# ai-forever/Kandinsky-2

Hardware: AMD Instinct MI355X
Metric: UNet denoise steps/sec @ 768x768 bs=1, 50 steps (higher is better)
Workload: dtype bf16; 1 GPU; Kandinsky-2.x text2img 768x768, decoder_steps=50, bs=1/GPU (CFG batch 2x4x96x96), 2.1-architecture UNet (1.23B) p_sampler step; parity pinned against the reference's modules; head=2.1, tile_configs_measured_in_this_process=0, images_per_gpu=1, parallelism=prompt-sharded x1, weights by one RCCL broadcast, world_size_observed=1, graph=True, chains=1, loop_graph=a 5-step loop replayed as ONE hipGraph (83 replay(s) = 415 timed steps)

## Files before the change

include/k22.h:

```cpp
#ifndef K22_H
#define K22_H
#include <stddef.h>
#include <stdint.h>
#ifdef __cplusplus
extern "C" {
#endif

#define K22_OK 0
#define K22_EINVAL (-1)
#define K22_EHIP (-2)
#define K22_ENOMEM (-3)

#define K22_BF16 0
#define K22_F32 1
#define K22_F16 2
#define K22_F16X3 3
#define K22_F16X2 4

int k22_version(void);
#define K22_BUILD_PACKED_FP32 1
#define K22_BUILD_DEBUG_VARIANTS 2
int k22_build_flags(void);
const char* k22_last_error(void);
int k22_set_option(const char* name, int value);
// ... 100 lines not shown
  int out_mode, res_f32, act, a_raw, want_stats;
  int SK0, SK1;
  int att_T, att_S, att_Tkp;
  int ldo, ldr;
  int has_frag;
  int algo, bm, bn, splitk, stages;
} K22IgemmProblem;
typedef struct K22IgemmOperands {
  const void *A0, *A1, *Wp, *bias, *residual;
  void *out, *partial;
  const void *S0, *S1, *Ws, *bias2;
  void *kall, *vtall;
  const void *Wfrag, *Wsfrag;
  float* stats;
  int stats_capacity_rows;
} K22IgemmOperands;
int k22_igemm_cfg_accepted(const K22IgemmProblem* pr);
int k22_igemm_cfg(const K22IgemmProblem* pr, const K22IgemmOperands* ops, int* rows_per_image, void* stream);
int k22_debug_conv_trace(const void* x_padded, const void* Wp, const float* bias, void* out, int B, int H, int W, int Cin, int Cout,
                         int Npad, unsigned long long* trace, void* stream);
int k22_conv3x3_gn(const void* x0, const void* x1, int C0, int C1, const float* gamma, const float* beta, const float* film, long film_ld,
                   float eps, int act, void* scratch, const void* Wp, const float* bias, const void* residual, void* out, void* partial,
                   int B, int H, int W, int Cout, int Npad, int splitk, int bm, int algo, int dtype, void* stream);
int k22_groupnorm(const void* x0, const void* x1, int C0, int C1, int B, int H, int W, const float* gamma,
                  const float* beta, const float* film, long film_ld, float eps, int act, int mode, int pad,
                  void* scratch, void* out, int dtype, void* stream);
size_t k22_groupnorm_scratch_bytes(int B, int C);
int k22_attention(const void* qkv, const void* ctxkv, void* kall, void* vtall, void* out, int B, int H, int T, int S,
                  int dtype, void* stream);
int k22_qkv_project(const void* x, const void* Wp, const float* bias, void* q_out, void* kall, void* vtall,
                    int B, int H, int T, int S, int K, int bm, int bn, int dtype, void* stream);
int k22_qkv_project_stream(const void* x, const void* Wp, const float* bias, void* q_out, void* kall, void* vtall, void* partial,
                           int B, int H, int T, int S, int K, int bm, int splitk, int dtype, void* stream);
int k22_linear_smallm(const float* x, const void* W, const float* bias, const float* add, float* out, int M, int N,
                      int K, int act_in, int act_out, int wdtype, void* stream);
int k22_conv3x3_direct(const float* x, const float* w, const float* bias, float* y, int B, int Cin, int Cout, int Hin, int Win,
                       int stride, int act, void* stream);

size_t k22_afrag_bytes(int M, int K);
int k22_afrag_pack(const void* A, long lda, void* out, int M, int K, int dtype, void* stream);
int k22_skinny_gemm(const void* Afrag, const void* Wfrag, const float* bias, void* out, float* partial, int M, int N, int Npad, int K,
                    int splitk, int epi, int act, int ldo, int mt, int nb, int dtype, void* stream);
int k22_finish_ln(const float* partial, int splitk, const float* bias, float* x, long ldx, const float* gain, const float* beta, void* yfrag,
                  int M, int N, float eps, int dtype, void* stream);
int k22_small_attention(const void* qkv, const float* qkv_partial, int nsplit, const float* qkv_bias, void* out, int out_frag, int B, int H, int T,
                        int causal, const float* key_valid, int kv_n, int dtype, void* stream);

typedef struct K22PriorConfig {
  int dtype;
  int text_ctx;
  int xf_width;
  int xf_layers;
  int xf_heads;
  int xf_final_ln;
  int clip_dim;
  int clip_xf_width;
} K22PriorConfig;
typedef struct K22Prior K22Prior;
int k22_prior_create(const K22PriorConfig* cfg, const K22Weight* weights, int n_weights, K22Prior** out);
void k22_prior_destroy(K22Prior* m);
int k22_prior_plan(K22Prior* m, int B, size_t* workspace_bytes);
int k22_prior_bind(K22Prior* m, void* workspace, size_t workspace_bytes);
int k22_prior_tuning_report(const K22Prior* m, char* buf, size_t cap);
int k22_prior_forward(K22Prior* m, const float* x, const float* timesteps, const float* text_emb, const float* text_enc,
                      const float* key_valid, float* out, void* stream);
int k22_prior_sampler_step(const float* x, const float* model_out, const float* noise, const float* scales, const float* table_row,
                           float clamp, float* x_out, int bs, int D, void* stream);
int k22_prior_ddim_step(const float* x, const float* model_out, const float* noise, const float* scales, const float* table_row,
                        float clamp, float* x_out, float* x0_out, int bs, int D, void* stream);
enum { K22_PRIOR_LOOP_ANCESTRAL = 0, K22_PRIOR_LOOP_DDIM = 1 };
int k22_prior_sample_loop(K22Prior* m, int kind, float* x, float* x_tmp, float* x0_out, const float* timesteps, const float* table,
                          const float* noise_seq, const float* scales, const float* text_emb, const float* text_enc,
                          const float* key_valid, float clamp, int n_steps, int use_graph, void* stream);

typedef struct K22MoVQConfig {
  int dtype;
  int ch;
  int n_levels;
  int ch_mult[8];
  int num_res_blocks;
  int attn_levels;
  int z_channels;
  int out_ch;
} K22MoVQConfig;
typedef struct K22MoVQ K22MoVQ;
int k22_movq_create(const K22MoVQConfig* cfg, const K22Weight* weights, int n_weights, K22MoVQ** out);
void k22_movq_destroy(K22MoVQ* m);
int k22_movq_plan(K22MoVQ* m, int B, int h, int w, size_t* workspace_bytes);
int k22_movq_bind(K22MoVQ* m, void* workspace, size_t workspace_bytes);
int k22_movq_decode(K22MoVQ* m, const float* z, float* out, unsigned char* out_u8, void* stream);
int k22_movq_plan_encoder(K22MoVQ* m, int B, int H, int W, size_t* workspace_bytes);
int k22_movq_encode(K22MoVQ* m, const float* image, float* latent, void* stream);
int k22_movq_num_ops(const K22MoVQ* m);

enum { K22_ENC_CLIP_TEXT = 0, K22_ENC_CLIP_VISION = 1, K22_ENC_XLMR = 2 };
typedef struct K22EncoderConfig {
  int dtype;
  int kind;
  int width;
  int layers;
  int heads;
  int n_ctx;
  int vocab;
  int out_dim;
  int image_size;
  int patch;
  int max_pos;
  int pad_id;
  float ln_eps;
  int mlp_dim;
  int hidden_act;
} K22EncoderConfig;
typedef struct K22Encoder K22Encoder;
int k22_encoder_create(const K22EncoderConfig* cfg, const K22Weight* weights, int n_weights, K22Encoder** out);
void k22_encoder_destroy(K22Encoder* m);
int k22_encoder_plan(K22Encoder* m, int B, size_t* workspace_bytes);
int k22_encoder_bind(K22Encoder* m, void* workspace, size_t workspace_bytes);
int k22_encoder_forward(K22Encoder* m, const int* tokens, const float* key_valid, const float* image, float* seq_out, float* pooled_out,
                        void* stream);

int k22_blend_noised(const float* x, const float* init, const float* noise, const float* mask, float sa, float sb, float* out,
                     int N, int C, int HW, int broadcast_first, void* stream);

int k22_spatialnorm_apply(const void* x, const float* coeff, const float* zq, const float* wy, const float* by, const float* wb, const float* bb,
                          void* out, int B, int H, int W, int C, int h0, int w0, int shift, int act, int pad, int dtype, void* stream);
int k22_upsample2_pad(const void* x, void* y, int B, int H, int W, int C, int dtype, void* stream);
int k22_pad_copy(const void* x, void* y, int B, int H, int W, int C, int dtype, void* stream);
int k22_subsample_odd(const void* x, void* y, int B, int H, int W, int C, int dtype, void* stream);
int k22_softmax_rows(void* x, long rows, int L, float scale, int dtype, void* stream);
int k22_movq_prepare(const float* z, const float* wpq, const float* bpq, float* zq, void* xin, int B, int h, int w, int Cpad, int dtype, void* stream);
int k22_movq_enc_prepare(const float* image, void* xin, int B, int H, int W, int Cpad, int dtype, void* stream);
int k22_movq_quant_conv(const float* h, const float* wq, const float* bq, float* out, int B, int HW, void* stream);
int k22_to_uint8_nhwc(const float* x, unsigned char* y, int B, int C, int H, int W, void* stream);
int k22_enc_layernorm(const float* x, long ldx, const float* gain, const float* beta, float* out_f32, long ld_out, void* out_t, int rows,
                      int D, float eps, int dtype, void* stream);
int k22_enc_embed(const int* tokens, const float* tok_emb, const float* pos_emb, const float* type_emb, float* x, int B, int n_ctx, int D,
                  int vocab, int xlmr, int pad_id, int max_pos, void* stream);
int k22_enc_gather_eot(const int* tokens, const float* x, float* out, int B, int n_ctx, int D, void* stream);
int k22_enc_masked_mean(const float* x, const float* mask, float* out, int B, int n_ctx, int D, void* stream);
int k22_enc_patchify(const float* image, void* out, int B, int S, int patch, int Kp, int dtype, void* stream);
int k22_enc_vision_assemble(const float* patch_out, const float* cls, const float* pos, float* x, int B, int P, int D, void* stream);
int k22_enc_mlp_act(const float* x, void* y, long n, int exact, int dtype, void* stream);
int k22_enc_attention_generic(const void* qkv, void* out, int B, int heads, int n, int hd, int dtype, void* stream);
int k22_prior_layernorm(const float* x, long ldx, const float* gain, const float* beta, void* y, int rows, int D, int to_f32, int dtype,
                        void* stream);
int k22_prior_finish_input(float* inp, const float* pos, const float* prd, int B, int n_ctx, int D, void* stream);
int k22_attention_masked(const void* qkv, const void* ctxkv, void* kall, void* vtall, void* out, int B, int H, int T, int S, int causal,
                         const float* key_valid, int kv_n, int out_x3, int dtype, void* stream);
int k22_gn_stats(const void* x0, const void* x1, int C0, int C1, int B, int HW, float* partial, int* nsplit_out, int dtype, void* stream);
int k22_gn_coeff(const float* st0, int rpi0, int C0, const float* st1, int rpi1, int C1, int B, int HW, const float* gamma, const float* beta,
                 const float* film, long film_ld, float eps, float* coeff, void* stream);
int k22_gn_apply(const void* x0, const void* x1, int C0, int C1, int B, int H, int W, const float* coeff, int act, int mode, int pad, void* out,
                 int dtype, void* stream);

#ifdef __cplusplus
}
#endif
#endif
```

kandinsky-2_amd/_lib.py:

```python
from __future__ import annotations

import ctypes as C
import os

_HERE = os.path.dirname(os.path.abspath(__file__))
LIB_PATH = os.environ.get("K22_LIB_PATH") or os.path.join(_HERE, "libk22hip.so")
TILE_TABLE_PATH = os.path.join(_HERE, "tiles_gfx950.txt")

K22_BF16, K22_F32, K22_F16, K22_F16X3, K22_F16X2 = 0, 1, 2, 3, 4
K22_LOOP_DDIM, K22_LOOP_PLMS = 0, 1
K22_PRIOR_LOOP_ANCESTRAL, K22_PRIOR_LOOP_DDIM = 0, 1
F16X3 = "f16x3"
F16X2 = "f16x2"
SPLIT_DTYPES = (F16X3, F16X2)
X3_WSCALE = 256.0


def dtype_code(backend_dtype) -> int:
    import torch
    try:
        return {torch.bfloat16: K22_BF16, torch.float32: K22_F32, torch.float16: K22_F16, F16X3: K22_F16X3, F16X2: K22_F16X2}[backend_dtype]
    except KeyError:
        raise ValueError('backend_dtype must be torch.bfloat16, torch.float16, torch.float32 "f16x3" or "f16x2"') from None
ACT_NONE, ACT_SILU, ACT_GELU = 0, 1, 2
OUT_ROWMAJOR, OUT_ROWMAJOR_F32, OUT_NCHW_F32, OUT_QKV = 0, 1, 2, 3


class K22UNetConfig(C.Structure):
    _fields_ = [
        ("dtype", C.c_int), ("in_channels", C.c_int), ("model_channels", C.c_int), ("out_channels", C.c_int),
        ("num_res_blocks", C.c_int), ("n_levels", C.c_int), ("channel_mult", C.c_int * 8),
        ("n_attention_ds", C.c_int), ("attention_ds", C.c_int * 8), ("num_head_channels", C.c_int),
        ("ctx_dim", C.c_int), ("ctx_len", C.c_int), ("n_image_embs", C.c_int), ("text_dim1", C.c_int),
        ("text_dim2", C.c_int), ("image_dim", C.c_int), ("head_type", C.c_int), ("hint_channels", C.c_int),
    ]


class K22IgemmProblem(C.Structure):
    _fields_ = [(n, C.c_int) for n in (
        "dtype", "taps", "M", "N", "Kc", "K0", "H", "W", "out_mode", "res_f32", "act", "a_raw", "want_stats", "SK0", "SK1",
        "att_T", "att_S", "att_Tkp", "ldo", "ldr", "has_frag", "algo", "bm", "bn", "splitk", "stages")]


class K22IgemmOperands(C.Structure):
    _fields_ = [(n, C.c_void_p) for n in (
        "A0", "A1", "Wp", "bias", "residual", "out", "partial", "S0", "S1", "Ws", "bias2", "kall", "vtall", "Wfrag", "Wsfrag",
        "stats")] + [("stats_capacity_rows", C.c_int)]


class K22MoVQConfig(C.Structure):
    _fields_ = [("dtype", C.c_int), ("ch", C.c_int), ("n_levels", C.c_int), ("ch_mult", C.c_int * 8),
                ("num_res_blocks", C.c_int), ("attn_levels", C.c_int), ("z_channels", C.c_int), ("out_ch", C.c_int)]


class K22PriorConfig(C.Structure):
    _fields_ = [("dtype", C.c_int), ("text_ctx", C.c_int), ("xf_width", C.c_int), ("xf_layers", C.c_int), ("xf_heads", C.c_int),
                ("xf_final_ln", C.c_int), ("clip_dim", C.c_int), ("clip_xf_width", C.c_int)]


class K22EncoderConfig(C.Structure):
    _fields_ = [("dtype", C.c_int), ("kind", C.c_int), ("width", C.c_int), ("layers", C.c_int), ("heads", C.c_int), ("n_ctx", C.c_int),
                ("vocab", C.c_int), ("out_dim", C.c_int), ("image_size", C.c_int), ("patch", C.c_int), ("max_pos", C.c_int),
                ("pad_id", C.c_int), ("ln_eps", C.c_float), ("mlp_dim", C.c_int), ("hidden_act", C.c_int)]


class K22Weight(C.Structure):
    _fields_ = [("name", C.c_char_p), ("ptr", C.c_void_p)]


_P, _I, _L, _F, _D, _Z = C.c_void_p, C.c_int, C.c_long, C.c_float, C.c_double, C.c_size_t

SIGNATURES = {
    "k22_version": (_I, []),
    "k22_build_flags": (_I, []),
    "k22_last_error": (C.c_char_p, []),
    "k22_set_option": (_I, [C.c_char_p, _I]),
    "k22_comm_broadcast_weights": (_I, [_P, _Z, _I, _P, _P]),
    "k22_tile_table_load": (_I, [C.c_char_p]),
    "k22_tile_table_save": (_I, [C.c_char_p]),
    "k22_tile_table_size": (_I, []),
    "k22_tile_table_measured": (_I, []),
    "k22_tile_table_clear": (None, []),
    "k22_unet_create": (_I, [C.POINTER(K22UNetConfig), C.POINTER(K22Weight), _I, C.POINTER(_P)]),
    "k22_unet_destroy": (None, [_P]),
    "k22_unet_plan": (_I, [_P, _I, _I, _I, C.POINTER(_Z)]),
    "k22_unet_bind": (_I, [_P, _P, _Z]),
    "k22_unet_set_condition": (_I, [_P, _P, _P, _P, _P]),
    "k22_unet_set_hint": (_I, [_P, _P, _P]),
    "k22_unet_forward": (_I, [_P, _P, _P, _P, _P, _P, _I, _P]),
    "k22_unet_sample_loop": (_I, [_P, _P, _P, _P, _P, _P, _P, _P, _P, _P, C.POINTER(_I), _I, _F, _F, _F, _I, _D, _P, _I, _P]),
    "k22_unet_ddim_loop": (_I, [_P, _I, _P, _P, _P, _P, _P, _P, _P, _P, _P, _I, _F, _I, _P]),
    "k22_unet_num_ops": (_I, [_P]),
    "k22_unet_set_autotune": (_I, [_P, _I]),
    "k22_unet_tuning_report": (_I, [_P, C.c_char_p, _Z]),
    "k22_unet_profile": (_I, [_P, _I, C.POINTER(_D), C.POINTER(_D), C.POINTER(_D), C.POINTER(_I), _P]),
    "k22_afrag_bytes": (_Z, [_I, _I]),
    "k22_afrag_pack": (_I, [_P, _L, _P, _I, _I, _I, _P]),
    "k22_skinny_gemm": (_I, [_P, _P, _P, _P, _P, _I, _I, _I, _I, _I, _I, _I, _I, _I, _I, _I, _P]),
    "k22_finish_ln": (_I, [_P, _I, _P, _P, _L, _P, _P, _P, _I, _I, _F, _I, _P]),
    "k22_small_attention": (_I, [_P, _P, _I, _P, _P, _I, _I, _I, _I, _I, _P, _I, _I, _P]),
    "k22_prior_create": (_I, [C.POINTER(K22PriorConfig), C.POINTER(K22Weight), _I, C.POINTER(_P)]),
    "k22_prior_destroy": (None, [_P]),
    "k22_prior_plan": (_I, [_P, _I, C.POINTER(_Z)]),
    "k22_prior_bind": (_I, [_P, _P, _Z]),
    "k22_prior_tuning_report": (_I, [_P, C.c_char_p, _Z]),
    "k22_prior_forward": (_I, [_P, _P, _P, _P, _P, _P, _P, _P]),
    "k22_prior_sampler_step": (_I, [_P, _P, _P, _P, _P, _F, _P, _I, _I, _P]),
    "k22_prior_ddim_step": (_I, [_P, _P, _P, _P, _P, _F, _P, _P, _I, _I, _P]),
    "k22_prior_sample_loop": (_I, [_P, _I, _P, _P, _P, _P, _P, _P, _P, _P, _P, _P, _F, _I, _I, _P]),
    "k22_encoder_create": (_I, [C.POINTER(K22EncoderConfig), C.POINTER(K22Weight), _I, C.POINTER(_P)]),
    "k22_encoder_destroy": (None, [_P]),
    "k22_encoder_plan": (_I, [_P, _I, C.POINTER(_Z)]),
    "k22_encoder_bind": (_I, [_P, _P, _Z]),
    "k22_encoder_forward": (_I, [_P, _P, _P, _P, _P, _P, _P]),
    "k22_movq_create": (_I, [C.POINTER(K22MoVQConfig), C.POINTER(K22Weight), _I, C.POINTER(_P)]),
    "k22_movq_destroy": (None, [_P]),
    "k22_movq_plan": (_I, [_P, _I, _I, _I, C.POINTER(_Z)]),
    "k22_movq_bind": (_I, [_P, _P, _Z]),
    "k22_movq_decode": (_I, [_P, _P, _P, _P, _P]),
    "k22_movq_plan_encoder": (_I, [_P, _I, _I, _I, C.POINTER(_Z)]),
    "k22_movq_encode": (_I, [_P, _P, _P, _P]),
    "k22_movq_num_ops": (_I, [_P]),
    "k22_ddim_step": (_I, [_P, _P, _P, _P, _F, _I, _P, _P, _I, _I, _P]),
    "k22_blend_noised": (_I, [_P, _P, _P, _P, _F, _F, _P, _I, _I, _I, _I, _P]),
    "k22_prepare_mask": (_I, [_P, _P, _I, _I, _I, _P]),
    "k22_plms_step": (_I, [_P, _P, _P, _P, _P, _I, _P, _F, _I, _P, _P, _P, _I, _I, _P]),
    "k22_sampler_scratch_bytes": (_Z, [_I, _I]),
    "k22_sampler_step": (_I, [_P, _P, _P, _P, _P, _P, _I, _F, _I, _F, _F, _I, _D, _P, _P, _P, _I, _I, _P]),
    "k22_gemm": (_I, [_P, _P, _P, _P, _P, _P, _P, _I, _I, _I, _I, _I, _L, _L, _I, _I, _I, _I, _I, _I, _I, _I, _P]),
    "k22_x3_pack": (_I, [_P, _P, _L, _F, _P]),
    "k22_conv3x3": (_I, [_P, _P, _P, _P, _P, _P, _I, _I, _I, _I, _I, _I, _I, _I, _I, _I, _I, _I, _P]),
    "k22_conv3x3_skip": (_I, [_P, _P, _P, _P, _P, _I, _I, _P, _P, _P, _P, _I, _I, _I, _I, _I, _I, _I, _I, _I, _P]),
    "k22_gemm_gnstats": (_I, [_P, _P, _P, _P, _P, _P, _I, _I, _I, _I, _I, _I, _I, _I, _P, _I, C.POINTER(_I), _I, _P]),
    "k22_conv3x3_gnstats": (_I, [_P, _P, _P, _P, _P, _P, _I, _I, _I, _I, _I, _I, _I, _I, _I, _P, _I, C.POINTER(_I), _I, _P]),
    "k22_igemm_cfg_accepted": (_I, [C.POINTER(K22IgemmProblem)]),
    "k22_igemm_cfg": (_I, [C.POINTER(K22IgemmProblem), C.POINTER(K22IgemmOperands), C.POINTER(_I), _P]),
    "k22_conv3x3_gn": (_I, [_P, _P, _I, _I, _P, _P, _P, _L, _F, _I, _P, _P, _P, _P, _P, _P, _I, _I, _I, _I, _I, _I, _I, _I, _I, _P]),
    "k22_debug_conv_trace": (_I, [_P, _P, _P, _P, _I, _I, _I, _I, _I, _I, _P, _P]),
    "k22_groupnorm": (_I, [_P, _P, _I, _I, _I, _I, _I, _P, _P, _P, _L, _F, _I, _I, _I, _P, _P, _I, _P]),
    "k22_groupnorm_scratch_bytes": (_Z, [_I, _I]),
    "k22_attention": (_I, [_P, _P, _P, _P, _P, _I, _I, _I, _I, _I, _P]),
    "k22_qkv_project": (_I, [_P, _P, _P, _P, _P, _P, _I, _I, _I, _I, _I, _I, _I, _I, _P]),
    "k22_qkv_project_stream": (_I, [_P, _P, _P, _P, _P, _P, _P, _I, _I, _I, _I, _I, _I, _I, _I, _P]),
    "k22_linear_smallm": (_I, [_P, _P, _P, _P, _P, _I, _I, _I, _I, _I, _I, _P]),
    "k22_conv3x3_direct": (_I, [_P, _P, _P, _P, _I, _I, _I, _I, _I, _I, _I, _P]),
    "k22_debug_counter": (_L, [C.c_char_p]),
    "k22_stream_frag_bytes": (C.c_size_t, [_I, _I, _I, _I]),
    "k22_stream_repack": (_I, [_P, _P, _I, _I, _I, _I, _P]),
    "k22_debug_set_stream_frag": (_I, [_P, _P]),
    "k22_debug_set_stream_scratch": (_I, [_P, C.c_size_t]),
    "k22_spatialnorm_apply": (_I, [_P, _P, _P, _P, _P, _P, _P, _P, _I, _I, _I, _I, _I, _I, _I, _I, _I, _I, _P]),
    "k22_upsample2_pad": (_I, [_P, _P, _I, _I, _I, _I, _I, _P]),
    "k22_pad_copy": (_I, [_P, _P, _I, _I, _I, _I, _I, _P]),
    "k22_subsample_odd": (_I, [_P, _P, _I, _I, _I, _I, _I, _P]),
    "k22_softmax_rows": (_I, [_P, _L, _I, _F, _I, _P]),
    "k22_movq_prepare": (_I, [_P, _P, _P, _P, _P, _I, _I, _I, _I, _I, _P]),
    "k22_movq_enc_prepare": (_I, [_P, _P, _I, _I, _I, _I, _I, _P]),
    "k22_movq_quant_conv": (_I, [_P, _P, _P, _P, _I, _I, _P]),
    "k22_to_uint8_nhwc": (_I, [_P, _P, _I, _I, _I, _I, _P]),
    "k22_enc_layernorm": (_I, [_P, _L, _P, _P, _P, _L, _P, _I, _I, _F, _I, _P]),
    "k22_enc_embed": (_I, [_P, _P, _P, _P, _P, _I, _I, _I, _I, _I, _I, _I, _P]),
    "k22_enc_gather_eot": (_I, [_P, _P, _P, _I, _I, _I, _P]),
    "k22_enc_masked_mean": (_I, [_P, _P, _P, _I, _I, _I, _P]),
    "k22_enc_patchify": (_I, [_P, _P, _I, _I, _I, _I, _I, _P]),
    "k22_enc_vision_assemble": (_I, [_P, _P, _P, _P, _I, _I, _I, _P]),
    "k22_enc_mlp_act": (_I, [_P, _P, _L, _I, _I, _P]),
    "k22_enc_attention_generic": (_I, [_P, _P, _I, _I, _I, _I, _I, _P]),
    "k22_prior_layernorm": (_I, [_P, _L, _P, _P, _P, _I, _I, _I, _I, _P]),
    "k22_prior_finish_input": (_I, [_P, _P, _P, _I, _I, _I, _P]),
    "k22_attention_masked": (_I, [_P, _P, _P, _P, _P, _I, _I, _I, _I, _I, _P, _I, _I, _I, _P]),
    "k22_gn_stats": (_I, [_P, _P, _I, _I, _I, _I, _P, C.POINTER(_I), _I, _P]),
    "k22_gn_coeff": (_I, [_P, _I, _I, _P, _I, _I, _I, _I, _P, _P, _P, _L, _F, _P, _P]),
    "k22_gn_apply": (_I, [_P, _P, _I, _I, _I, _I, _I, _P, _I, _I, _I, _P, _I, _P]),
}

_lib = None


def lib() -> C.CDLL:
    global _lib
    if _lib is None:
        if not os.path.exists(LIB_PATH):
            raise RuntimeError(
                f"{LIB_PATH} is missing: the HIP extension is the only compute path (no CPU fallback). "
                "Build it with `python -c 'import __graft_entry__ as g; g.build()'`.")
        l = C.CDLL(LIB_PATH)
        for name, (res, args) in SIGNATURES.items():
            fn = getattr(l, name)
            fn.restype = res
            fn.argtypes = args
        _lib = l
        tbl = os.environ.get("K22_TILE_TABLE", TILE_TABLE_PATH)
        if tbl != "0" and os.path.exists(tbl):
            if l.k22_tile_table_load(tbl.encode()) < 0:
                raise RuntimeError(f"k22: cannot read the tile table {tbl}")
    return _lib


def check(rc: int) -> None:
    if rc != 0:
        msg = lib().k22_last_error()
        raise RuntimeError(f"k22 error {rc}: {msg.decode() if msg else ''}")


def ptr(t) -> int:
    if t is None:
        return None
    assert t.is_contiguous(), "k22: tensors crossing the C ABI must be contiguous"
    return t.data_ptr()


def current_stream() -> int:
    import torch
    return torch.cuda.current_stream().cuda_stream
```

kandinsky-2_amd/csrc/capi.hip:

```cpp
#include "kernels.h"
#include "elementwise.h"
#include "../../include/k22.h"
#include "tuning.h"
#include "skinny.h"
#include <dlfcn.h>
#include <stdio.h>
#include <string.h>

static thread_local char g_err[512] = "";

int k22_set_error(int code, const char* msg) {
  snprintf(g_err, sizeof(g_err), "%s", msg ? msg : "");
  return code;
}
int k22_set_error_hip(hipError_t e, const char* file, int line) {
  snprintf(g_err, sizeof(g_err), "HIP error %d (%s) at %s:%d", (int)e, hipGetErrorString(e), file, line);
  return K22_EHIP;
}

extern "C" {

int k22_version(void) { return 100; }
int k22_build_flags(void) {
  int f = 0;
#ifndef K22_NOPK
  f |= K22_BUILD_PACKED_FP32;
#endif
#if defined(K22_DEBUG_VARIANTS) || defined(K22_STREAM_DEBUG) || defined(K22_SKINNY_DEBUG)
  f |= K22_BUILD_DEBUG_VARIANTS;
#endif
  return f;
}

int k22_set_option(const char* name, int value) {
  if (name && !strcmp(name, "igemm_stages")) { igemm_set_default_stages(value); return K22_OK; }
  if (name && !strcmp(name, "igemm_xcd_remap")) { igemm_set_xcd_remap(value); return K22_OK; }
  if (name && !strcmp(name, "conv_algo")) { igemm_set_conv_algo(value); return K22_OK; }
  if (name && !strcmp(name, "gemm_algo")) { igemm_set_gemm_algo(value); return K22_OK; }
  if (name && !strcmp(name, "att_pipe")) { attention_set_pipe(value); return K22_OK; }
  return k22_set_error(K22_EINVAL, "k22_set_option: unknown option");
}
const char* k22_last_error(void) { return g_err; }

#ifdef K22_STREAM_DEBUG
static unsigned long long* g_dbg_trace = nullptr;
extern "C" int k22_debug_set_stream_trace(unsigned long long* t) { g_dbg_trace = t; return K22_OK; }
#define K22_DBG_TRACE(p) (p).st_trace = g_dbg_trace
#else
#define K22_DBG_TRACE(p) (void)0
#endif
static const void* g_dbg_wfrag = nullptr;
static const void* g_dbg_wsfrag = nullptr;
static void* g_dbg_scratch = nullptr;
static size_t g_dbg_scratch_bytes = 0;
static int dbg_frag(IgemmParams& p, int dtype, hipStream_t st) {
  K22_DBG_TRACE(p);
  p.Wfrag = g_dbg_wfrag; p.Wsfrag = g_dbg_wsfrag;
  if (g_dbg_wfrag || !g_dbg_scratch || dtype == K22_F32 || (p.taps != 1 && p.taps != 9) || p.Kc % 64 || p.Npad % 64) return K22_OK;
  const size_t n1 = stream_frag_bytes(p.Npad, p.taps, p.Kc, dtype);
  const bool skip = p.S0 != nullptr && p.Ws != nullptr && (p.SK0 + p.SK1) % 64 == 0;
  const size_t n2 = skip ? stream_frag_bytes(p.Npad, 1, p.SK0 + p.SK1, dtype) : 0;
  if (n1 + n2 > g_dbg_scratch_bytes) return k22_set_error(K22_ENOMEM, "debug stream scratch too small");
  if (int rc = launch_stream_repack(p.Wp, g_dbg_scratch, p.Npad, p.taps, p.Kc, dtype, st)) return rc;
  p.Wfrag = g_dbg_scratch;
  if (skip) {
    void* w2 = static_cast<char*>(g_dbg_scratch) + n1;
    if (int rc = launch_stream_repack(p.Ws, w2, p.Npad, 1, p.SK0 + p.SK1, dtype, st)) return rc;
    p.Wsfrag = w2;
  }
  return K22_OK;
}
#define K22_DBG_FRAG(p) do { if (int rc_ = dbg_frag((p), dtype, reinterpret_cast<hipStream_t>(stream))) return rc_; } while (0)
int k22_debug_set_stream_frag(const void* wfrag, const void* wsfrag) { g_dbg_wfrag = wfrag; g_dbg_wsfrag = wsfrag; return K22_OK; }
int k22_debug_set_stream_scratch(void* scratch, size_t bytes) { g_dbg_scratch = scratch; g_dbg_scratch_bytes = scratch ? bytes : 0; return K22_OK; }
size_t k22_stream_frag_bytes(int Npad, int taps, int Kc, int dtype) { return stream_frag_bytes(Npad, taps, Kc, dtype); }
int k22_stream_repack(const void* W, void* out, int Npad, int taps, int Kc, int dtype, void* stream) {
  return launch_stream_repack(W, out, Npad, taps, Kc, dtype, reinterpret_cast<hipStream_t>(stream));
}

long k22_debug_counter(const char* name) {
  if (name && !strcmp(name, "stream_launches")) return stream_launch_count();
  if (name && !strcmp(name, "loop_captures")) return loop_capture_count();
  if (name && !strcmp(name, "loop_launches")) return loop_launch_count();
  return -1;
}

int k22_comm_broadcast_weights(void* arena, size_t bytes, int root, void* nccl_comm, void* stream) {
  if (!arena || !nccl_comm) return k22_set_error(K22_EINVAL, "k22_comm_broadcast_weights: null arena / communicator");
  typedef int (*bcast_fn)(const void*, void*, size_t, int , int, void*, hipStream_t);
  static bcast_fn fn = nullptr;
  if (!fn) {
    void* sym = dlsym(RTLD_DEFAULT, "ncclBroadcast");
    if (!sym) {
      void* h = dlopen("librccl.so.1", RTLD_NOW | RTLD_GLOBAL);
      if (!h) h = dlopen("librccl.so", RTLD_NOW | RTLD_GLOBAL);
      if (h) sym = dlsym(h, "ncclBroadcast");
    }
    if (!sym) return k22_set_error(K22_EINVAL, "k22_comm_broadcast_weights: RCCL (ncclBroadcast) is not loadable in this process");
    fn = reinterpret_cast<bcast_fn>(sym);
  }
  const size_t piece = (size_t)1 << 30;
  char* base = reinterpret_cast<char*>(arena);
  for (size_t off = 0; off < bytes; off += piece) {
    const size_t n = bytes - off < piece ? bytes - off : piece;
    const int rc = fn(base + off, base + off, n,  1, root, nccl_comm, reinterpret_cast<hipStream_t>(stream));
    if (rc != 0) { char msg[96]; snprintf(msg, sizeof msg, "k22_comm_broadcast_weights: ncclBroadcast returned %d", rc); return k22_set_error(K22_EHIP, msg); }
  }
  return K22_OK;
}

int k22_tile_table_load(const char* path) {
  if (!path) return k22_set_error(K22_EINVAL, "k22_tile_table_load: null path");
  const int n = tile_table_load_file(path);
  if (n < 0) return k22_set_error(K22_EINVAL, "k22_tile_table_load: cannot read the file");
  return n;
}
int k22_tile_table_save(const char* path) {
  if (!path) return k22_set_error(K22_EINVAL, "k22_tile_table_save: null path");
  const int n = tile_table_save_file(path);
  if (n < 0) return k22_set_error(K22_EINVAL, "k22_tile_table_save: cannot write the file");
  return n;
}
int k22_tile_table_size(void) {
  TileTable& tt = tile_table();
  std::lock_guard<std::mutex> lk(tt.mu);
  return (int)tt.m.size();
}
int k22_tile_table_measured(void) {
  TileTable& tt = tile_table();
  std::lock_guard<std::mutex> lk(tt.mu);
  return (int)tt.measured;
}
void k22_tile_table_clear(void) {
  TileTable& tt = tile_table();
  std::lock_guard<std::mutex> lk(tt.mu);
  tt.m.clear();
  tt.measured = 0;
}

int k22_gemm(const void* A0, const void* A1, const void* Wp, const float* bias, const void* residual, void* out,
             void* partial, int M, int N, int Npad, int K0, int K1, long lda0, long lda1, int ldo, int ldr,
             int out_f32, int act, int splitk, int bm, int bn, int dtype, void* stream) {
  IgemmParams p = igemm_gemm_problem(M, N, K0, K1, out_f32 ? IG_OUT_ROWMAJOR_F32 : IG_OUT_ROWMAJOR, act);
  p.A0 = A0; p.A1 = A1; p.Wp = Wp; p.bias = bias; p.residual = residual; p.out = out;
  p.partial = reinterpret_cast<float*>(partial);
  p.Npad = Npad; p.lda0 = lda0; p.lda1 = lda1; p.ldo = ldo; p.ldr = ldr;
  p.splitk = splitk; p.force_bm = bm; p.force_bn = bn;
  p.a_raw = k22_is_split(dtype) ? 1 : 0;
  if (p.splitk == 0) p.splitk = partial ? igemm_choose_splitk(p, dtype) : 1;
  K22_DBG_FRAG(p);
  return launch_igemm(p, dtype, reinterpret_cast<hipStream_t>(stream));
}

int k22_x3_pack(const float* src, void* dst, long n, float scale, void* stream) {
  if (!src || !dst || n < 0) return k22_set_error(K22_EINVAL, "x3_pack: null argument");
  return launch_x3_pack(src, dst, n, scale, reinterpret_cast<hipStream_t>(stream));
}

int k22_conv3x3(const void* x_padded, const void* Wp, const float* bias, const void* residual, void* out,
                void* partial, int B, int H, int W, int Cin, int Cout, int Npad, int out_mode, int act, int splitk,
                int bm, int bn, int dtype, void* stream) {
  IgemmParams p = igemm_conv3_problem(B, H, W, Cin, Cout, out_mode, act);
  p.A0 = x_padded; p.Wp = Wp; p.bias = bias; p.residual = residual; p.out = out;
  p.partial = reinterpret_cast<float*>(partial);
  p.Npad = Npad; p.splitk = splitk; p.force_bm = bm; p.force_bn = bn;
  if (p.splitk == 0) p.splitk = partial ? igemm_choose_splitk(p, dtype) : 1;
  K22_DBG_FRAG(p);
  return launch_igemm(p, dtype, reinterpret_cast<hipStream_t>(stream));
}

int k22_conv3x3_gnstats(const void* x_padded, const void* Wp, const float* bias, const void* residual, void* out,
                        void* partial, int B, int H, int W, int Cin, int Cout, int Npad, int splitk, int bm, int bn,
                        float* stats, int stats_capacity_rows, int* rows_per_image, int dtype, void* stream) {
  IgemmParams p = igemm_conv3_problem(B, H, W, Cin, Cout);
  p.A0 = x_padded; p.Wp = Wp; p.bias = bias; p.residual = residual; p.out = out;
  p.partial = reinterpret_cast<float*>(partial);
  p.Npad = Npad; p.splitk = splitk; p.force_bm = bm; p.force_bn = bn;
  if (p.splitk == 0) p.splitk = partial ? igemm_choose_splitk(p, dtype) : 1;
  const int rpi = igemm_stats_rows_per_image(p, dtype);
  if (rows_per_image) *rows_per_image = rpi;
  if (rpi <= 0) return k22_set_error(K22_EINVAL, "conv3x3_gnstats: this configuration cannot produce GroupNorm partial sums");
  if (rpi * B > stats_capacity_rows) return k22_set_error(K22_ENOMEM, "conv3x3_gnstats: stats buffer too small");
  p.stats = stats;
  K22_DBG_FRAG(p);
  return launch_igemm(p, dtype, reinterpret_cast<hipStream_t>(stream));
}

int k22_gemm_gnstats(const void* A, const void* Wp, const float* bias, const void* residual, void* out, void* partial,
                     int B, int H, int W, int N, int Npad, int K, int splitk, int bm, float* stats,
                     int stats_capacity_rows, int* rows_per_image, int dtype, void* stream) {
  IgemmParams p = igemm_gemm_problem(B * H * W, N, K, 0);
  p.A0 = A; p.Wp = Wp; p.bias = bias; p.residual = residual; p.out = out; p.partial = reinterpret_cast<float*>(partial);
  p.Npad = Npad; p.H = H; p.W = W;
  p.splitk = splitk > 0 ? splitk : 1;
  p.force_bm = bm; p.algo = (bm == 160 || bm == 288) ? IG_ALGO_STREAM : IG_ALGO_GEMM8;
  p.a_raw = k22_is_split(dtype) ? 1 : 0;
  const int rpi = igemm_stats_rows_per_image(p, dtype);
  if (rows_per_image) *rows_per_image = rpi;
  if (rpi <= 0) return k22_set_error(K22_EINVAL, "gemm_gnstats: this configuration cannot produce GroupNorm partial sums");
  if (rpi * B > stats_capacity_rows) return k22_set_error(K22_ENOMEM, "gemm_gnstats: stats buffer too small");
  p.stats = stats;
  K22_DBG_FRAG(p);
  return launch_igemm(p, dtype, reinterpret_cast<hipStream_t>(stream));
}

int k22_conv3x3_skip(const void* x_padded, const void* Wp, const float* bias, const void* skip0, const void* skip1,
                     int SK0, int SK1, const void* Ws, const float* bias_s, void* out, void* partial, int B, int H, int W,
                     int Cin, int Cout, int Npad, int splitk, int bm, int dtype, void* stream) {
  IgemmParams p = igemm_conv3_problem(B, H, W, Cin, Cout);
  p.A0 = x_padded; p.Wp = Wp; p.bias = bias; p.out = out; p.partial = reinterpret_cast<float*>(partial);
  p.Npad = Npad; p.splitk = splitk; p.force_bm = bm;
  p.S0 = skip0; p.S1 = skip1; p.SK0 = SK0; p.SK1 = SK1; p.Ws = Ws; p.bias2 = bias_s;
  if (p.splitk == 0) p.splitk = partial ? igemm_choose_splitk(p, dtype) : 1;
  K22_DBG_FRAG(p);
  return launch_igemm(p, dtype, reinterpret_cast<hipStream_t>(stream));
}

static int igemm_problem_tuned(const K22IgemmProblem& d, Tuned& t) {
  if (d.dtype < K22_BF16 || d.dtype > K22_F16X2) return k22_set_error(K22_EINVAL, "igemm_cfg: bad dtype");
  if ((d.taps != 1 && d.taps != 9) || d.M <= 0 || d.N <= 0 || d.Kc <= 0 || d.K0 <= 0 || d.K0 > d.Kc)
    return k22_set_error(K22_EINVAL, "igemm_cfg: bad problem (taps 1 / 9, M, N > 0, 0 < K0 <= Kc)");
  if (d.out_mode < IG_OUT_ROWMAJOR || d.out_mode > IG_OUT_QKV || d.SK0 < 0 || d.SK1 < 0 || (d.SK1 > 0 && d.SK0 == 0))
    return k22_set_error(K22_EINVAL, "igemm_cfg: bad output mode / skip widths");
  if (d.taps == 9 && (d.H <= 0 || d.W <= 0 || d.M % (d.H * d.W))) return k22_set_error(K22_EINVAL, "igemm_cfg: a convolution needs M = B * H * W");
  const void* mark = reinterpret_cast<const void*>(1);
  IgemmParams& p = t.p;
  if (d.taps == 9) {
    p = igemm_conv3_problem(d.M / (d.H * d.W), d.H, d.W, d.Kc, d.N, d.out_mode, d.act);
    p.K0 = d.K0;
  } else {
    p = igemm_gemm_problem(d.M, d.N, d.K0, d.Kc - d.K0, d.out_mode, d.act);
    p.H = d.H; p.W = d.W;
  }
  p.ldo = d.ldo > 0 ? d.ldo : (d.out_mode == IG_OUT_QKV ? d.N / 3 : d.N);
  p.ldr = d.ldr > 0 ? d.ldr : (d.res_f32 ? p.ldo : d.N);
  p.res_f32 = d.res_f32 ? 1 : 0; p.a_raw = d.a_raw ? 1 : 0;
// ... 163 lines not shown
  FinishLnParams q = {};
  q.partial = partial; q.splitk = splitk; q.bias = bias; q.x = x; q.ldx = ldx; q.g = gain; q.b = beta; q.yfrag = yfrag; q.M = M; q.N = N;
  q.MA = (M + 31) / 32; q.eps = eps;
  return launch_finish_ln(q, dtype, reinterpret_cast<hipStream_t>(stream));
}
int k22_small_attention(const void* qkv, const float* qkv_partial, int nsplit, const float* qkv_bias, void* out, int out_frag, int B, int H, int T,
                        int causal, const float* key_valid, int kv_n, int dtype, void* stream) {
  SmallAttnParams ap = {};
  ap.qkv = qkv; ap.part = qkv_partial; ap.nsplit = nsplit; ap.bias = qkv_bias; ap.ldq = 3 * H * 64; ap.out = out; ap.ldo = H * 64; ap.out_frag = out_frag; ap.MA = (B * T + 31) / 32;
  ap.B = B; ap.H = H; ap.T = T; ap.scale = 0.125f; ap.causal = causal; ap.key_valid = key_valid; ap.kv_ld = kv_n; ap.kv_n = kv_n;
  return launch_small_attention(ap, dtype, reinterpret_cast<hipStream_t>(stream));
}

int k22_linear_smallm(const float* x, const void* W, const float* bias, const float* add, float* out, int M, int N,
                      int K, int act_in, int act_out, int wdtype, void* stream) {
  LinearSmallParams lp = {};
  lp.x = x; lp.ldx = K; lp.W = W; lp.bias = bias; lp.add = add; lp.ld_add = N; lp.out = out; lp.ldo = N;
  lp.M = M; lp.N = N; lp.K = K; lp.act_in = act_in; lp.act_out = act_out;
  return launch_linear_smallm(lp, wdtype, reinterpret_cast<hipStream_t>(stream));
}

int k22_conv3x3_direct(const float* x, const float* w, const float* bias, float* y, int B, int Cin, int Cout, int Hin, int Win,
                       int stride, int act, void* stream) {
  if (!x || !w || !bias || !y) return k22_set_error(K22_EINVAL, "conv3x3_direct: null argument");
  if (B < 1 || Cin < 1 || Cout < 1 || Hin < 1 || Win < 1) return k22_set_error(K22_EINVAL, "conv3x3_direct: empty shape");
  if (act != K22_ACT_NONE && act != K22_ACT_SILU) return k22_set_error(K22_EINVAL, "conv3x3_direct: act must be 0 (none) or 1 (SiLU)");
  ConvDirectParams p = {};
  p.x = x; p.w = w; p.bias = bias; p.y = y;
  p.B = B; p.Cin = Cin; p.Cout = Cout; p.Hin = Hin; p.Win = Win; p.stride = stride; p.act = act;
  return launch_conv3x3_direct(p, reinterpret_cast<hipStream_t>(stream));
}

int k22_ddim_step(const float* x, const float* model_out, const float* noise, const float* table_row, float guidance, int use_cfg,
                  float* x_out, float* x0_out, int N, int HW, void* stream) {
  if (!x || !model_out || !table_row || !x_out) return k22_set_error(K22_EINVAL, "ddim_step: null argument");
  return launch_ddim_step(x, model_out, noise, table_row, guidance, use_cfg, x_out, x0_out, N, HW, reinterpret_cast<hipStream_t>(stream));
}

int k22_prepare_mask(const float* mask, float* out, int C, int H, int W, void* stream) {
  if (!mask || !out) return k22_set_error(K22_EINVAL, "prepare_mask: null argument");
  return launch_prepare_mask(mask, out, C, H, W, reinterpret_cast<hipStream_t>(stream));
}

int k22_plms_step(const float* x, const float* model_out, const float* eps_hist1, const float* eps_hist2, const float* eps_hist3, int order,
                  const float* table_row, float guidance, int use_cfg, float* x_out, float* eps_out, float* x0_out, int N, int HW, void* stream) {
  if (!x || !model_out || !table_row || !x_out) return k22_set_error(K22_EINVAL, "plms_step: null argument");
  return launch_plms_step(x, model_out, eps_hist1, eps_hist2, eps_hist3, order, table_row, guidance, use_cfg, x_out, eps_out, x0_out, N, HW,
                          reinterpret_cast<hipStream_t>(stream));
}

size_t k22_sampler_scratch_bytes(int N, int HW) { return (size_t)N * 4 * HW * sizeof(float) + 256; }

int k22_sampler_step(const float* x, const float* model_out, const float* noise, const float* init_img,
                     const float* mask, const float* table, int step_index, float guidance, int use_cfg,
                     float clamp_lo, float clamp_hi, int pct_index, double pct_gamma, void* scratch,
                     float* x_out, float* x0_out, int N, int HW, void* stream) {
  SamplerParams p = {};
  p.x = x; p.model_out = model_out; p.noise = noise; p.init_img = init_img; p.mask = mask; p.table = table;
  p.step = nullptr; p.step_host = step_index; p.guidance = guidance; p.clamp_lo = clamp_lo; p.clamp_hi = clamp_hi;
  p.use_cfg = use_cfg; p.n_lo = pct_index; p.gamma = pct_gamma;
  p.s_buf = reinterpret_cast<float*>(scratch);
  p.x0_buf = reinterpret_cast<float*>(scratch) + 64;
  p.x_out = x_out; p.x0_out = x0_out; p.N = N; p.HW = HW;
  if (pct_index >= 4 * HW) return k22_set_error(K22_EINVAL, "sampler: percentile index out of range");
  return launch_sampler_step(p, reinterpret_cast<hipStream_t>(stream));
}

static bool aux_dtype_ok(int dt) { return dt == K22_BF16 || dt == K22_F16 || dt == K22_F32; }

int k22_spatialnorm_apply(const void* x, const float* coeff, const float* zq, const float* wy, const float* by, const float* wb, const float* bb,
                          void* out, int B, int H, int W, int C, int h0, int w0, int shift, int act, int pad, int dtype, void* stream) {
  if (!x || !coeff || !zq || !wy || !by || !wb || !bb || !out || B < 1 || H < 1 || W < 1 || C < 1 || h0 < 1 || w0 < 1 || shift < 0 || shift > 12 || (H & ((1 << shift) - 1)) ||
      (pad != 0 && pad != 1) || (act != K22_ACT_NONE && act != K22_ACT_SILU) || !aux_dtype_ok(dtype))
    return k22_set_error(K22_EINVAL, "spatialnorm_apply: bad argument");
  SpatialNormParams p = {};
  p.x = x; p.coeff = coeff; p.zq = zq; p.wy = wy; p.by = by; p.wb = wb; p.bb = bb; p.out = out;
  p.B = B; p.H = H; p.W = W; p.C = C; p.h0 = h0; p.w0 = w0; p.shift = shift; p.act = act; p.pad = pad;
  return launch_spatialnorm_apply(p, dtype, reinterpret_cast<hipStream_t>(stream));
}
#define K22_AUX_NHWC(NAME_)                                                                                                     \
  int k22_##NAME_(const void* x, void* y, int B, int H, int W, int C, int dtype, void* stream) {                                \
    if (!x || !y || B < 1 || B > 65535 || H < 1 || W < 1 || C < 1 || !aux_dtype_ok(dtype)) return k22_set_error(K22_EINVAL, #NAME_ ": bad argument"); \
    return launch_##NAME_(x, y, B, H, W, C, dtype, reinterpret_cast<hipStream_t>(stream));                                      \
  }
K22_AUX_NHWC(upsample2_pad)
K22_AUX_NHWC(pad_copy)
K22_AUX_NHWC(subsample_odd)
#undef K22_AUX_NHWC
int k22_softmax_rows(void* x, long rows, int L, float scale, int dtype, void* stream) {
  if (!x || L < 1 || !aux_dtype_ok(dtype)) return k22_set_error(K22_EINVAL, "softmax_rows: bad argument");
  return launch_softmax_rows(x, rows, L, scale, dtype, reinterpret_cast<hipStream_t>(stream));
}
int k22_movq_prepare(const float* z, const float* wpq, const float* bpq, float* zq, void* xin, int B, int h, int w, int Cpad, int dtype, void* stream) {
  if (!z || !wpq || !bpq || !zq || !xin || B < 1 || h < 1 || w < 1 || Cpad < 4 || !aux_dtype_ok(dtype)) return k22_set_error(K22_EINVAL, "movq_prepare: bad argument");
  return launch_movq_prepare(z, wpq, bpq, zq, xin, B, h, w, Cpad, dtype, reinterpret_cast<hipStream_t>(stream));
}
int k22_movq_enc_prepare(const float* image, void* xin, int B, int H, int W, int Cpad, int dtype, void* stream) {
  if (!image || !xin || B < 1 || H < 1 || W < 1 || Cpad < 3 || !aux_dtype_ok(dtype)) return k22_set_error(K22_EINVAL, "movq_enc_prepare: bad argument");
  return launch_movq_enc_prepare(image, xin, B, H, W, Cpad, dtype, reinterpret_cast<hipStream_t>(stream));
}
int k22_movq_quant_conv(const float* h, const float* wq, const float* bq, float* out, int B, int HW, void* stream) {
  if (!h || !wq || !bq || !out || B < 1 || HW < 1) return k22_set_error(K22_EINVAL, "movq_quant_conv: bad argument");
  return launch_movq_quant_conv(h, wq, bq, out, B, HW, reinterpret_cast<hipStream_t>(stream));
}
int k22_to_uint8_nhwc(const float* x, unsigned char* y, int B, int C, int H, int W, void* stream) {
  if (!x || !y || B < 1 || C < 1 || H < 1 || W < 1) return k22_set_error(K22_EINVAL, "to_uint8_nhwc: bad argument");
  return launch_to_uint8_nhwc(x, y, B, C, H, W, reinterpret_cast<hipStream_t>(stream));
}
int k22_attention_masked(const void* qkv, const void* ctxkv, void* kall, void* vtall, void* out, int B, int H, int T, int S, int causal,
                         const float* key_valid, int kv_n, int out_x3, int dtype, void* stream) {
  if (!qkv || !kall || !vtall || !out || B < 1 || H < 1 || T < 1 || S < 0 || kv_n < 0 || (S > 0 && !ctxkv) || !(aux_dtype_ok(dtype) || k22_is_split(dtype)))
    return k22_set_error(K22_EINVAL, "attention_masked: bad argument");
  if (causal && S != 0) return k22_set_error(K22_EINVAL, "attention_masked: causal needs S == 0 (key index against query index)");
  if (kv_n > S + T) return k22_set_error(K22_EINVAL, "attention_masked: kv_n > S + T");
  if (out_x3 && !k22_is_split(dtype)) return k22_set_error(K22_EINVAL, "attention_masked: out_x3 needs a split dtype");
  return attention_seq(qkv, ctxkv, kall, vtall, out, B, H, T, S, causal, key_valid, kv_n, out_x3, dtype, reinterpret_cast<hipStream_t>(stream));
}

int k22_gn_stats(const void* x0, const void* x1, int C0, int C1, int B, int HW, float* partial, int* nsplit_out, int dtype, void* stream) {
  if (nsplit_out) *nsplit_out = 0;
  if (!x0 || !partial || C0 < 1 || C1 < 0 || (C1 > 0 && !x1) || B < 1 || B > 65535 || HW < 1 || !(aux_dtype_ok(dtype) || k22_is_split(dtype)))
    return k22_set_error(K22_EINVAL, "gn_stats: bad argument");
  GnStatsParams sp = {};
  sp.x0 = x0; sp.x1 = C1 > 0 ? x1 : nullptr; sp.C0 = C0; sp.C1 = C1; sp.HW = HW; sp.B = B; sp.groups = 32; sp.nsplit = gn_nsplit(B, HW); sp.partial = partial;
  if (nsplit_out) *nsplit_out = sp.nsplit;
  return launch_gn_stats(sp, k22_storage_dtype(dtype), reinterpret_cast<hipStream_t>(stream));
}
int k22_gn_coeff(const float* st0, int rpi0, int C0, const float* st1, int rpi1, int C1, int B, int HW, const float* gamma, const float* beta,
                 const float* film, long film_ld, float eps, float* coeff, void* stream) {
  if (!gamma || !beta || !coeff) return k22_set_error(K22_EINVAL, "gn_coeff: gamma, beta and coeff are required");
  if (!st0 || C0 < 1 || C1 < 0 || B < 1 || B > 65535 || HW < 1) return k22_set_error(K22_EINVAL, "gn_coeff: bad argument");
  if (rpi0 <= 0 || (C1 > 0 && rpi1 <= 0)) return k22_set_error(K22_EINVAL, "gn_coeff: rows per image of a used source must be positive");
  if (C1 > 0 && !st1) return k22_set_error(K22_EINVAL, "gn_coeff: second source without partial sums");
  const int C = C0 + C1;
  if (C % 32 != 0) return k22_set_error(K22_EINVAL, "gn_coeff: 32 groups need C % 32 == 0");
  if (film && film_ld < 2L * C) return k22_set_error(K22_EINVAL, "gn_coeff: film_ld < 2 C");
  GnCoeffParams cp = {};
  cp.src[0].st = st0; cp.src[0].rpi = rpi0; cp.src[0].C = C0;
  if (C1 > 0) { cp.src[1].st = st1; cp.src[1].rpi = rpi1; cp.src[1].C = C1; }
  cp.HW = HW; cp.C = C; cp.groups = 32; cp.eps = eps; cp.gamma = gamma; cp.beta = beta; cp.film = film; cp.film_ld = film_ld; cp.coeff = coeff;
  return launch_gn_coeff(cp, B, reinterpret_cast<hipStream_t>(stream));
}
int k22_gn_apply(const void* x0, const void* x1, int C0, int C1, int B, int H, int W, const float* coeff, int act, int mode, int pad, void* out,
                 int dtype, void* stream) {
  if (!x0 || !coeff || !out || C0 < 1 || C1 < 0 || (C1 > 0 && !x1) || B < 1 || H < 1 || W < 1 || mode < 0 || mode > 2 || (mode == 1 && (H < 2 || W < 2)) ||
      (pad != 0 && pad != 1) || (act != K22_ACT_NONE && act != K22_ACT_SILU) || !(aux_dtype_ok(dtype) || k22_is_split(dtype)))
    return k22_set_error(K22_EINVAL, "gn_apply: bad argument");
  GnApplyParams ap = {};
  ap.x0 = x0; ap.x1 = C1 > 0 ? x1 : nullptr; ap.C0 = C0; ap.C1 = C1; ap.B = B; ap.H = H; ap.W = W; ap.mode = mode; ap.pad = pad; ap.act = act;
  ap.coeff = coeff; ap.out = out; ap.out_x3 = k22_is_split(dtype) ? 1 : 0;
  return launch_gn_apply(ap, k22_storage_dtype(dtype), reinterpret_cast<hipStream_t>(stream));
}

}

__global__ __launch_bounds__(256) void lds_sentinel_kernel(int words, int spins, unsigned* rec) {
  extern __shared__ unsigned sent_lds[];
  for (int i = threadIdx.x; i < words; i += 256) sent_lds[i] = 0xA5000000u | (unsigned)i;
  __syncthreads();
  for (int s = 0; s < spins; ++s) {
    for (int i = threadIdx.x; i < words; i += 256) {
      const unsigned v = reinterpret_cast<volatile unsigned*>(sent_lds)[i];
      if (v != (0xA5000000u | (unsigned)i)) {
        const unsigned k = atomicAdd(rec, 1u);
        if (k < 255u) { rec[1 + 4 * k] = blockIdx.x; rec[2 + 4 * k] = 4u * i; rec[3 + 4 * k] = v; rec[4 + 4 * k] = (unsigned)s; }
        sent_lds[i] = 0xA5000000u | (unsigned)i;
      }
    }
    __builtin_amdgcn_s_sleep(8);
  }
}
extern "C" int k22_debug_lds_sentinel(int bytes, int workgroups, int spins, unsigned* rec, void* stream) {
  if (bytes <= 0 || bytes > 64 * 1024 || (bytes & 3) || !rec) return k22_set_error(K22_EINVAL, "lds_sentinel: bytes in 4..65536, multiple of 4");
  hipLaunchKernelGGL(lds_sentinel_kernel, dim3(workgroups), dim3(256), (size_t)bytes, reinterpret_cast<hipStream_t>(stream), bytes / 4, spins, rec);
  K22_CHECK_LAUNCH();
  return K22_OK;
}
```

kandinsky-2_amd/csrc/elementwise.h:

```cpp
#pragma once
#include "common.h"

struct GnStatsParams {
  const void* x0; const void* x1;
  int C0, C1, HW, B, groups, nsplit;
  float* partial;
};
struct GnSrc { const float* st; int rpi, C; };
struct GnCoeffParams {
  GnSrc src[2];
  int HW, C, groups; float eps;
  const float* gamma; const float* beta;
  const float* film; int64_t film_ld;
  float* coeff;
};
struct GnApplyParams {
  const void* x0; const void* x1; int C0, C1;
  int B, H, W;
  int mode;
  int pad;
  int act;
  const float* coeff;
  void* out;
  int out_x3;
};
struct ConvInParams {
  const float* x; const float* img; const float* mask;
  const float* w; const float* bias;
  void* out;
  int B, H, W, Cin, Cout;
  int img_premul;
};
struct ConvDirectParams {
  const float* x; const float* w; const float* bias; float* y;
  int B, Cin, Cout, Hin, Win, stride, act;
};
int launch_conv3x3_direct(const ConvDirectParams& p, hipStream_t s);
struct LinearSmallParams {
  const float* x; int64_t ldx;
  const void* W;
  const float* bias;
  const float* add; int64_t ld_add;
  int add_mod;
  float* out; int64_t ldo;
  int M, N, K, act_in, act_out;
  int rows_per_wave;
};
struct KvPackParams {
  const void* qkv; const void* ctxkv; void* kall; void* vtall;
  int B, H, T, S, Tkp;
};
struct AttentionParams {
  const void* q; int64_t ldq;
  const void* kall; const void* vtall;
  void* out; int64_t ldo;
  int B, H, T, Tk, Tkp;
  float scale;
  int causal;
  const float* key_valid;
  int kv_ld, kv_n;
  int out_x3;
};
struct SmallAttnParams {
  const void* qkv; int64_t ldq;
  const float* part; int nsplit; const float* bias;
  void* out; int64_t ldo;
  int out_frag, MA;
  int B, H, T;
  float scale;
  int causal;
  const float* key_valid; int kv_ld, kv_n;
};
struct SamplerParams {
  const float* x;
  const float* model_out;
  const float* noise;
  const float* init_img;
  const float* mask;
  const float* table;
  const int* step;
  int step_host;
  float guidance, clamp_lo, clamp_hi;
  int use_cfg;
  int n_lo; double gamma;
  float* x0_buf;
  float* s_buf;
  float* x_out;
  float* x0_out;
  int N, HW;
};

int launch_x3_pack(const float* in, void* out, int64_t n, float scale, hipStream_t s);
int gn_nsplit(int B, int HW);
int launch_gn_stats(const GnStatsParams& p, int dtype, hipStream_t s);
int launch_gn_coeff(const GnCoeffParams& p, int B, hipStream_t s);
inline int launch_gn_stats_coeff(const void* x0, const void* x1, int C0, int C1, int B, int HW, float eps, const float* gamma, const float* beta,
                                 const float* film, int64_t film_ld, float* partial, float* coeff, int dtype, hipStream_t s) {
  const int nsplit = gn_nsplit(B, HW), C = C0 + C1;
  GnStatsParams sp = {};
  sp.x0 = x0; sp.x1 = x1; sp.C0 = C0; sp.C1 = C1; sp.HW = HW; sp.B = B; sp.groups = 32; sp.nsplit = nsplit; sp.partial = partial;
  const int rc = launch_gn_stats(sp, dtype, s);
  if (rc) return rc;
  GnCoeffParams cp = {};
  cp.src[0].st = partial; cp.src[0].rpi = nsplit; cp.src[0].C = C;
  cp.HW = HW; cp.C = C; cp.groups = 32; cp.eps = eps; cp.gamma = gamma; cp.beta = beta; cp.film = film; cp.film_ld = film_ld; cp.coeff = coeff;
  return launch_gn_coeff(cp, B, s);
}
int launch_gn_apply(const GnApplyParams& p, int dtype, hipStream_t s);
int launch_resample(const void* x, void* y, int B, int H, int W, int C, int mode, int dtype, hipStream_t s);
int launch_conv_in(const ConvInParams& p, int dtype, hipStream_t s);
int launch_timestep_embedding(const float* t, const float* freqs, float* out, int B, int half, hipStream_t s);
int launch_linear_smallm(const LinearSmallParams& p, int wdtype, hipStream_t s);
int launch_layernorm_f32(const float* x, const float* g, const float* b, float* y, int rows, int D, float eps, hipStream_t s);
int launch_cast_rows(const float* x, void* y, int rows, int cols, int64_t ldx, int64_t ldy, int dtype, hipStream_t s);
int launch_kv_pack(const KvPackParams& p, int dtype, hipStream_t s);
int launch_attention(const AttentionParams& p, int dtype, hipStream_t s);
int launch_small_attention(const SmallAttnParams& p, int dtype, hipStream_t s);
int launch_sampler_step(const SamplerParams& p, hipStream_t s);
int launch_plms_step(const float* x, const float* model_out, const float* h1, const float* h2, const float* h3, int order, const float* tab,
                     float guidance, int use_cfg, float* x_out, float* e_store, float* x0_out, int N, int HW, hipStream_t s);
int launch_prepare_mask(const float* old_mask, float* out, int C, int H, int W, hipStream_t s);
int launch_ddim_step(const float* x, const float* model_out, const float* noise, const float* tab, float guidance, int use_cfg,
                     float* x_out, float* x0_out, int N, int HW, hipStream_t s);

struct SpatialNormParams {
  const void* x;
  const float* coeff;
  const float* zq;
  const float* wy; const float* by;
  const float* wb; const float* bb;
  void* out;
  int B, H, W, C, h0, w0, shift, act, pad;
};
int launch_spatialnorm_apply(const SpatialNormParams& p, int dtype, hipStream_t s);
int launch_upsample2_pad(const void* x, void* y, int B, int H, int W, int C, int dtype, hipStream_t s);
int launch_softmax_rows(void* x, int64_t rows, int L, float scale, int dtype, hipStream_t s);
int launch_movq_prepare(const float* z, const float* wpq, const float* bpq, float* zq, void* xin, int B, int h, int w,
                        int Cpad, int dtype, hipStream_t s);
int launch_movq_enc_prepare(const float* img, void* xin, int B, int H, int W, int Cpad, int dtype, hipStream_t s);
int launch_pad_copy(const void* x, void* y, int B, int H, int W, int C, int dtype, hipStream_t s);
int launch_subsample_odd(const void* x, void* y, int B, int H, int W, int C, int dtype, hipStream_t s);
int launch_movq_quant_conv(const float* h, const float* wq, const float* bq, float* out, int B, int HW, hipStream_t s);
int launch_to_uint8_nhwc(const float* x, unsigned char* y, int B, int C, int H, int W, hipStream_t s);
```

kandinsky-2_amd/csrc/elementwise.hip:

```cpp
#include "kernels.h"
#include "elementwise.h"

__device__ __forceinline__ void load4(const bf16_t* p, float* f) {
  const uint2 r = *reinterpret_cast<const uint2*>(p);
  f[0] = __uint_as_float(r.x << 16); f[1] = __uint_as_float(r.x & 0xffff0000u);
  f[2] = __uint_as_float(r.y << 16); f[3] = __uint_as_float(r.y & 0xffff0000u);
}
__device__ __forceinline__ void load4(const f16_t* p, float* f) {
  const uint2 r = *reinterpret_cast<const uint2*>(p);
  unpack2_f16(r.x, f[0], f[1]); unpack2_f16(r.y, f[2], f[3]);
}
__device__ __forceinline__ void load4(const float* p, float* f) {
  const float4 r = *reinterpret_cast<const float4*>(p);
  f[0] = r.x; f[1] = r.y; f[2] = r.z; f[3] = r.w;
}

template <typename T>
__global__ __launch_bounds__(256) void gn_stats_kernel(GnStatsParams p) {
  __shared__ float red[1024 * 2 * 2];
  const int tid = threadIdx.x, b = blockIdx.y, s = blockIdx.x;
  const int C = p.C0 + p.C1, VP = C / 4;
  const int per = (p.HW + p.nsplit - 1) / p.nsplit;
  const int pix0 = s * per, pix1 = min(p.HW, pix0 + per);
  const T* x0 = reinterpret_cast<const T*>(p.x0) + (int64_t)b * p.HW * p.C0;
  const T* x1 = p.x1 ? reinterpret_cast<const T*>(p.x1) + (int64_t)b * p.HW * p.C1 : nullptr;
  int PL, pl;
  if (VP >= 256) { PL = 1; pl = 0; } else { PL = 256 / VP; pl = tid / VP; }
  float sum[3][4], sq[3][4];
  int vj[3];
#pragma unroll
  for (int j = 0; j < 3; ++j) {
    int v = (VP >= 256) ? tid + 256 * j : ((j == 0 && pl < PL) ? tid - pl * VP : VP);
    vj[j] = v < VP ? v : -1;
#pragma unroll
    for (int k = 0; k < 4; ++k) { sum[j][k] = 0.f; sq[j][k] = 0.f; }
  }
#pragma unroll
  for (int j = 0; j < 3; ++j) {
    if (vj[j] >= 0) {
      const int c = vj[j] * 4;
      const T* src = c < p.C0 ? x0 + c : x1 + (c - p.C0);
      const int64_t ld = c < p.C0 ? p.C0 : p.C1;
      int pix = pix0 + pl;
      for (; pix + 7 * PL < pix1; pix += 8 * PL) {
        float f[8][4];
#pragma unroll
        for (int u = 0; u < 8; ++u) load4(src + (int64_t)(pix + u * PL) * ld, f[u]);
#pragma unroll
        for (int k = 0; k < 4; ++k) {
          sum[j][k] += ((f[0][k] + f[1][k]) + (f[2][k] + f[3][k])) + ((f[4][k] + f[5][k]) + (f[6][k] + f[7][k]));
          sq[j][k] += ((f[0][k] * f[0][k] + f[1][k] * f[1][k]) + (f[2][k] * f[2][k] + f[3][k] * f[3][k])) +
                      ((f[4][k] * f[4][k] + f[5][k] * f[5][k]) + (f[6][k] * f[6][k] + f[7][k] * f[7][k]));
        }
      }
      for (; pix < pix1; pix += PL) {
        float f[4];
        load4(src + (int64_t)pix * ld, f);
#pragma unroll
        for (int k = 0; k < 4; ++k) { sum[j][k] += f[k]; sq[j][k] += f[k] * f[k]; }
      }
    }
  }
  float* out = p.partial + ((int64_t)b * p.nsplit + s) * C * 2;
  if (PL == 1) {
#pragma unroll
    for (int j = 0; j < 3; ++j)
      if (vj[j] >= 0) {
        float* o = out + (int64_t)vj[j] * 8;
        *reinterpret_cast<float4*>(o) = make_float4(sum[j][0], sq[j][0], sum[j][1], sq[j][1]);
        *reinterpret_cast<float4*>(o + 4) = make_float4(sum[j][2], sq[j][2], sum[j][3], sq[j][3]);
      }
    return;
  }
  if (vj[0] >= 0) {
    float* o = red + ((int64_t)pl * C + vj[0] * 4) * 2;
    *reinterpret_cast<float4*>(o) = make_float4(sum[0][0], sq[0][0], sum[0][1], sq[0][1]);
    *reinterpret_cast<float4*>(o + 4) = make_float4(sum[0][2], sq[0][2], sum[0][3], sq[0][3]);
  }
  __syncthreads();
  for (int i = tid; i < C * 2; i += 256) {
    float a = 0.f;
    for (int q = 0; q < PL; ++q) a += red[(int64_t)q * C * 2 + i];
    out[i] = a;
  }
}

__global__ __launch_bounds__(256) void gn_coeff_kernel(GnCoeffParams p) {
  __shared__ double red[4][2];
  __shared__ float ms[2];
  const int tid = threadIdx.x, lane = tid & 63, wave = tid >> 6, g = blockIdx.x, b = blockIdx.y;
  const int cg = p.C / p.groups;
  float pg = 0.f, pb = 0.f, psc = 1.f, psh = 0.f;
  if (tid < cg) {
    const int c = g * cg + tid;
    pg = p.gamma[c]; pb = p.beta[c];
    if (p.film != nullptr) {
      psc = 1.f + p.film[(int64_t)b * p.film_ld + c];
      psh = p.film[(int64_t)b * p.film_ld + p.C + c];
    }
  }
  double s = 0.0, q = 0.0;
  int off = 0;
#pragma unroll
  for (int k = 0; k < 2; ++k) {
    const GnSrc sr = p.src[k];
    if (sr.C > 0) {
      const int c_lo = max(g * cg, off), c_hi = min((g + 1) * cg, off + sr.C);
      const int nc = c_hi - c_lo;
      if (nc > 0) {
        const float* base = sr.st + ((int64_t)b * sr.rpi * sr.C + (c_lo - off)) * 2;
        const int items = sr.rpi * nc;
        int i = tid;
        for (; i + 768 < items; i += 1024) {
          float2 v[4];
#pragma unroll
          for (int u = 0; u < 4; ++u) {
            const int ii = i + 256 * u, r = ii / nc, cc = ii - r * nc;
            v[u] = *reinterpret_cast<const float2*>(base + ((int64_t)r * sr.C + cc) * 2);
          }
          s += ((double)v[0].x + (double)v[1].x) + ((double)v[2].x + (double)v[3].x);
          q += ((double)v[0].y + (double)v[1].y) + ((double)v[2].y + (double)v[3].y);
        }
        for (; i < items; i += 256) {
          const int r = i / nc, cc = i - r * nc;
          const float2 v = *reinterpret_cast<const float2*>(base + ((int64_t)r * sr.C + cc) * 2);
          s += (double)v.x;
          q += (double)v.y;
        }
      }
    }
    off += sr.C;
  }
#pragma unroll
  for (int o = 32; o > 0; o >>= 1) {
    s += __shfl_xor(s, o, 64);
    q += __shfl_xor(q, o, 64);
  }
  if (lane == 0) { red[wave][0] = s; red[wave][1] = q; }
  __syncthreads();
  if (tid == 0) {
    const double st = (red[0][0] + red[1][0]) + (red[2][0] + red[3][0]);
    const double qt = (red[0][1] + red[1][1]) + (red[2][1] + red[3][1]);
    const double n = (double)p.HW * (double)cg;
    const double mean = st / n;
    double var = qt / n - mean * mean;
    if (var < 0.0) var = 0.0;
    ms[0] = (float)mean;
    ms[1] = (float)(1.0 / sqrt(var + (double)p.eps));
  }
  __syncthreads();
  const float mean_f = ms[0], rstd_f = ms[1];
  if (tid < cg) {
    const int c = g * cg + tid;
    float A = rstd_f * pg;
    float Bc = pb - mean_f * A;
    if (p.film != nullptr) {
      A *= psc;
      Bc = Bc * psc + psh;
    }
    *reinterpret_cast<float2*>(p.coeff + ((int64_t)b * p.C + c) * 2) = make_float2(A, Bc);
  }
}

template <typename T>
__global__ __launch_bounds__(256) void gn_apply_kernel(GnApplyParams p) {
  constexpr int EPV = Vec16<T>::N;
  const bool fast = p.out_x3 != 0;
  const int C = p.C0 + p.C1, CV = C / EPV;
  const int Ho = p.mode == 1 ? p.H / 2 : (p.mode == 2 ? p.H * 2 : p.H);
  const int Wo = p.mode == 1 ? p.W / 2 : (p.mode == 2 ? p.W * 2 : p.W);
  const int pad = p.pad, Hp = Ho + 2 * pad, Wp = Wo + 2 * pad;
  const int idx = blockIdx.x * 256 + threadIdx.x;
  if (idx >= Wp * CV) return;
  const int xp = idx / CV, cv = idx - xp * CV;
  const int xo = xp - pad, yo = (int)blockIdx.y - pad, b = blockIdx.z;
  T* out = reinterpret_cast<T*>(p.out) + (((int64_t)b * Hp + blockIdx.y) * Wp + xp) * C + cv * EPV;
  Vec16<T> o;
  if (xo < 0 || yo < 0 || xo >= Wo || yo >= Ho) {
#pragma unroll
    for (int k = 0; k < EPV / 2; ++k) o.set2(k, 0.f, 0.f);
  } else {
    const int c = cv * EPV;
    const T* src; int cs, ld;
    if (c < p.C0) { src = reinterpret_cast<const T*>(p.x0); cs = c; ld = p.C0; }
    else { src = reinterpret_cast<const T*>(p.x1); cs = c - p.C0; ld = p.C1; }
    float A[EPV], Bc[EPV];
    const float* cf = p.coeff + ((int64_t)b * C + c) * 2;
#pragma unroll
    for (int k = 0; k < EPV; k += 2) {
      const float4 q = *reinterpret_cast<const float4*>(cf + 2 * k);
      A[k] = q.x; Bc[k] = q.y; A[k + 1] = q.z; Bc[k + 1] = q.w;
    }
    float r[EPV];
    if (p.mode == 1) {
      Vec16<T> v[4];
#pragma unroll
      for (int dy = 0; dy < 2; ++dy)
#pragma unroll
        for (int dx = 0; dx < 2; ++dx)
          v[dy * 2 + dx].raw = *reinterpret_cast<const decltype(v[0].raw)*>(src + ((int64_t)(b * p.H + 2 * yo + dy) * p.W + 2 * xo + dx) * ld + cs);
#pragma unroll
      for (int k = 0; k < EPV; ++k) {
        float acc = 0.f;
#pragma unroll
        for (int q = 0; q < 4; ++q) acc += fast ? apply_act_sel<true>(v[q].get(k) * A[k] + Bc[k], p.act) : apply_act_sel<false>(v[q].get(k) * A[k] + Bc[k], p.act);
        r[k] = acc * 0.25f;
      }
    } else {
      const int yi = p.mode == 2 ? yo >> 1 : yo, xi = p.mode == 2 ? xo >> 1 : xo;
      Vec16<T> v;
      v.raw = *reinterpret_cast<const decltype(v.raw)*>(src + ((int64_t)(b * p.H + yi) * p.W + xi) * ld + cs);
#pragma unroll
      for (int k = 0; k < EPV; ++k) r[k] = fast ? apply_act_sel<true>(v.get(k) * A[k] + Bc[k], p.act) : apply_act_sel<false>(v.get(k) * A[k] + Bc[k], p.act);
    }
#pragma unroll
    for (int k = 0; k < EPV / 2; ++k) o.set2(k, r[2 * k], r[2 * k + 1]);
  }
  if constexpr (sizeof(T) == 4) {
    if (p.out_x3) { x3_store4(out, x3_split4(o.raw)); return; }
  }
  *reinterpret_cast<decltype(o.raw)*>(out) = o.raw;
}

template <typename T>
__global__ __launch_bounds__(256) void resample_kernel(const void* xin, void* yout, int B, int H, int W, int C, int mode) {
  constexpr int EPV = Vec16<T>::N;
  const int CV = C / EPV;
  const int Ho = mode == 1 ? H / 2 : H * 2, Wo = mode == 1 ? W / 2 : W * 2;
  const int64_t total = (int64_t)B * Ho * Wo * CV;
  const T* x = reinterpret_cast<const T*>(xin);
  T* y = reinterpret_cast<T*>(yout);
  for (int64_t i = (int64_t)blockIdx.x * 256 + threadIdx.x; i < total; i += (int64_t)gridDim.x * 256) {
    const int cv = (int)(i % CV);
    int64_t t = i / CV;
    const int xo = (int)(t % Wo); t /= Wo;
    const int yo = (int)(t % Ho);
    const int b = (int)(t / Ho);
    Vec16<T> o;
    if (mode == 1) {
      float r[EPV];
#pragma unroll
      for (int k = 0; k < EPV; ++k) r[k] = 0.f;
#pragma unroll
      for (int dy = 0; dy < 2; ++dy)
#pragma unroll
        for (int dx = 0; dx < 2; ++dx) {
          Vec16<T> v;
          v.raw = *reinterpret_cast<const decltype(v.raw)*>(x + ((int64_t)(b * H + 2 * yo + dy) * W + 2 * xo + dx) * C + cv * EPV);
#pragma unroll
          for (int k = 0; k < EPV; ++k) r[k] += v.get(k);
        }
#pragma unroll
      for (int k = 0; k < EPV / 2; ++k) o.set2(k, r[2 * k] * 0.25f, r[2 * k + 1] * 0.25f);
    } else {
      o.raw = *reinterpret_cast<const decltype(o.raw)*>(x + ((int64_t)(b * H + (yo >> 1)) * W + (xo >> 1)) * C + cv * EPV);
    }
    *reinterpret_cast<decltype(o.raw)*>(y + i * EPV) = o.raw;
  }
}

constexpr int CONV_IN_PT = 8;
template <typename T, int CIN>
__global__ __launch_bounds__(128) void conv_in_kernel(ConvInParams p) {
  constexpr int PT = CONV_IN_PT, PW = PT + 2;
  __shared__ float patch[CIN][3][PW];
  const int tid = threadIdx.x;
  const int xt = blockIdx.x, y = blockIdx.y, b = blockIdx.z;
  const int x0 = xt * PT;
  const int hw = p.H * p.W;
  for (int i = tid; i < CIN * 3 * PW; i += 128) {
    const int c = i / (3 * PW), r = (i / PW) % 3, xx = i % PW;
    const int yy = y + r - 1, xs = x0 + xx - 1;
    float v = 0.f;
    if (yy >= 0 && yy < p.H && xs >= 0 && xs < p.W) {
      const int64_t o = (int64_t)yy * p.W + xs;
      if (c < 4) v = p.x[((int64_t)b * 4 + c) * hw + o];
      else if (c < 8) v = p.img[((int64_t)b * 4 + (c - 4)) * hw + o] * (p.img_premul ? 1.f : p.mask[(int64_t)b * hw + o]);
      else v = p.mask[(int64_t)b * hw + o];
    }
    patch[c][r][xx] = v;
  }
  __syncthreads();
  T* out = reinterpret_cast<T*>(p.out);
  for (int n = tid; n < p.Cout; n += 128) {
    float w[CIN * 9];
#pragma unroll
    for (int k = 0; k < CIN * 9; ++k) w[k] = p.w[(int64_t)k * p.Cout + n];
    const float bias = p.bias[n];
    for (int px = 0; px < PT && x0 + px < p.W; ++px) {
      float acc = bias;
#pragma unroll
      for (int c = 0; c < CIN; ++c)
#pragma unroll
        for (int r = 0; r < 3; ++r)
#pragma unroll
          for (int q = 0; q < 3; ++q) acc += w[c * 9 + r * 3 + q] * patch[c][r][px + q];
      out[((int64_t)(b * p.H + y) * p.W + x0 + px) * p.Cout + n] = from_f32<T>(acc);
    }
  }
}

template <int OCB>
__global__ __launch_bounds__(256) void conv3x3_direct_kernel(ConvDirectParams p) {
  const int Ho = (p.Hin - 1) / p.stride + 1, Wo = (p.Win - 1) / p.stride + 1;
  const int pix = blockIdx.x * 256 + threadIdx.x;
  const int oc0 = blockIdx.y * OCB, b = blockIdx.z;
  if (pix >= Ho * Wo) return;
  const int yo = pix / Wo, xo = pix - yo * Wo;
  const int yi = yo * p.stride - 1, xi = xo * p.stride - 1;
  float acc[OCB];
#pragma unroll
  for (int o = 0; o < OCB; ++o) acc[o] = (oc0 + o < p.Cout) ? p.bias[oc0 + o] : 0.f;
  const int64_t plane = (int64_t)p.Hin * p.Win;
  for (int c = 0; c < p.Cin; ++c) {
    const float* xp = p.x + ((int64_t)b * p.Cin + c) * plane;
    float v[9];
#pragma unroll
    for (int r = 0; r < 3; ++r)
#pragma unroll
      for (int q = 0; q < 3; ++q) {
        const int yy = yi + r, xx = xi + q;
        v[r * 3 + q] = (yy >= 0 && yy < p.Hin && xx >= 0 && xx < p.Win) ? xp[(int64_t)yy * p.Win + xx] : 0.f;
      }
#pragma unroll
    for (int o = 0; o < OCB; ++o) {
      if (oc0 + o < p.Cout) {
        const float* wp = p.w + ((int64_t)(oc0 + o) * p.Cin + c) * 9;
#pragma unroll
        for (int k = 0; k < 9; ++k) acc[o] += wp[k] * v[k];
      }
    }
  }
#pragma unroll
  for (int o = 0; o < OCB; ++o)
    if (oc0 + o < p.Cout) p.y[(((int64_t)b * p.Cout + oc0 + o) * Ho + yo) * Wo + xo] = apply_act(acc[o], p.act);
}

__global__ void timestep_embedding_kernel(const float* t, const float* freqs, float* out, int B, int half) {
  const int i = blockIdx.x * blockDim.x + threadIdx.x;
  if (i >= B * half) return;
  const int b = i / half, k = i - b * half;
  const float a = t[b] * freqs[k];
  out[(int64_t)b * 2 * half + k] = cosf(a);
  out[(int64_t)b * 2 * half + half + k] = sinf(a);
}

template <typename TW, int MT>
__global__ __launch_bounds__(256) void linear_smallm_kernel(LinearSmallParams p) {
  constexpr int EPC = 16 / sizeof(TW);
  extern __shared__ __attribute__((aligned(16))) char smem_lin[];
  float* xs = reinterpret_cast<float*>(smem_lin);
  const int tid = threadIdx.x, lane = tid & 63, wave = tid >> 6;
  for (int i = tid; i < MT * p.K; i += 256) {
    const int m = i / p.K, k = i - m * p.K;
    float xv = m < p.M ? p.x[(int64_t)m * p.ldx + k] : 0.f;
    if (p.act_in == K22_ACT_SILU) xv = silu_f(xv);
    xs[i] = xv;
  }
  __syncthreads();
  const int per_wave = p.rows_per_wave;
  const int n_begin = (blockIdx.x * 4 + wave) * per_wave;
  for (int r = 0; r < per_wave; ++r) {
    const int n = n_begin + r;
    if (n >= p.N) return;
    const TW* w = reinterpret_cast<const TW*>(p.W) + (int64_t)n * p.K;
    float acc[MT];
#pragma unroll
    for (int m = 0; m < MT; ++m) acc[m] = 0.f;
    for (int k = lane * EPC; k < p.K; k += 64 * EPC) {
      Vec16<TW> wv;
      wv.raw = *reinterpret_cast<const decltype(wv.raw)*>(w + k);
#pragma unroll
      for (int m = 0; m < MT; ++m) {
        const float* xr = xs + m * p.K + k;
#pragma unroll
        for (int e = 0; e < EPC; e += 4) {
          const float4 xv = *reinterpret_cast<const float4*>(xr + e);
          acc[m] += xv.x * wv.get(e) + xv.y * wv.get(e + 1) + xv.z * wv.get(e + 2) + xv.w * wv.get(e + 3);
        }
      }
    }
#pragma unroll
    for (int m = 0; m < MT; ++m) {
      float v = wave_sum(acc[m]);
      if (lane == 0 && m < p.M) {
        if (p.bias) v += p.bias[n];
        v = apply_act(v, p.act_out);
        if (p.add) v += p.add[(int64_t)(p.add_mod > 0 ? m % p.add_mod : m) * p.ld_add + n];
        p.out[(int64_t)m * p.ldo + n] = v;
      }
    }
  }
}

__global__ __launch_bounds__(256) void layernorm_f32_kernel(const float* x, const float* g, const float* bta, float* y, int D, float eps) {
  __shared__ float red[8];
  const int row = blockIdx.x, tid = threadIdx.x;
  const float* xr = x + (int64_t)row * D;
  float s = 0.f;
  for (int i = tid; i < D; i += 256) s += xr[i];
  s = wave_sum(s);
  if ((tid & 63) == 0) red[tid >> 6] = s;
  __syncthreads();
  const float mean = (red[0] + red[1] + red[2] + red[3]) / D;
  float q = 0.f;
  for (int i = tid; i < D; i += 256) { const float d = xr[i] - mean; q += d * d; }
  q = wave_sum(q);
  if ((tid & 63) == 0) red[4 + (tid >> 6)] = q;
  __syncthreads();
  const float rstd = rsqrtf((red[4] + red[5] + red[6] + red[7]) / D + eps);
  for (int i = tid; i < D; i += 256) y[(int64_t)row * D + i] = (xr[i] - mean) * rstd * g[i] + bta[i];
}

template <typename T>
__global__ void cast_rows_kernel(const float* x, void* yout, int rows, int cols, int64_t ldx, int64_t ldy) {
  T* y = reinterpret_cast<T*>(yout);
  const int64_t total = (int64_t)rows * cols;
  for (int64_t i = (int64_t)blockIdx.x * blockDim.x + threadIdx.x; i < total; i += (int64_t)gridDim.x * blockDim.x) {
    const int r = (int)(i / cols), c = (int)(i - (int64_t)r * cols);
    y[r * ldy + c] = from_f32<T>(x[r * ldx + c]);
  }
}

template <typename T>
__global__ __launch_bounds__(256) void kv_pack_kernel(KvPackParams p) {
  __shared__ T vt[64][66];
  const int tid = threadIdx.x, jt = blockIdx.x, h = blockIdx.y, b = blockIdx.z;
  const int C = p.H * 64, Tk = p.S + p.T;
  const T* qkv = reinterpret_cast<const T*>(p.qkv);
  const T* ckv = reinterpret_cast<const T*>(p.ctxkv);
  T* Kall = reinterpret_cast<T*>(p.kall) + ((int64_t)(b * p.H + h) * p.Tkp) * 64;
  T* VTall = reinterpret_cast<T*>(p.vtall) + ((int64_t)(b * p.H + h) * 64) * p.Tkp;
  for (int i = tid; i < 64 * 64; i += 256) {
    const int jj = i >> 6, d = i & 63;
    const int j = jt * 64 + jj;
    T kv = from_f32<T>(0.f), vv = from_f32<T>(0.f);
    if (j < p.S) {
      const T* r = ckv + (int64_t)(b * p.S + j) * 2 * C + h * 64 + d;
      kv = r[0]; vv = r[C];
    } else if (j < Tk) {
      const T* r = qkv + (int64_t)(b * p.T + (j - p.S)) * 3 * C + C + h * 64 + d;
      kv = r[0]; vv = r[C];
    }
    Kall[(int64_t)j * 64 + d] = kv;
    vt[d][jj] = vv;
  }
  __syncthreads();
  for (int i = tid; i < 64 * 64; i += 256) {
    const int d = i >> 6, jj = i & 63;
    VTall[(int64_t)d * p.Tkp + jt * 64 + jj] = vt[d][jj];
  }
}

__global__ __launch_bounds__(256) void x3_pack_kernel(const float4* __restrict__ in, u32x4_t* __restrict__ out, int64_t n4, float scale) {
  for (int64_t i = (int64_t)blockIdx.x * 256 + threadIdx.x; i < n4; i += (int64_t)gridDim.x * 256) {
    const float4 v = in[i];
    x3_store4(out + i, x3_split4(v.x * scale, v.y * scale, v.z * scale, v.w * scale));
  }
}
int launch_x3_pack(const float* in, void* out, int64_t n, float scale, hipStream_t s) {
  if (n % 8 || (uintptr_t)in % 16 || (uintptr_t)out % 32) return k22_set_error(K22_EINVAL, "x3_pack: n % 8 == 0, 16-byte aligned input, 32-byte aligned output (groups of eight)");
  const int64_t n4 = n / 4;
  int nb = (int)((n4 + 255) / 256);
  if (nb > 4096) nb = 4096;
  if (nb < 1) return K22_OK;
  hipLaunchKernelGGL(x3_pack_kernel, dim3(nb), dim3(256), 0, s, reinterpret_cast<const float4*>(in), reinterpret_cast<u32x4_t*>(out), n4, scale);
  K22_CHECK_LAUNCH();
  return K22_OK;
}

static inline int grid_for(int64_t total, int threads, int cap) {
  int64_t nb = (total + threads - 1) / threads;
  if (nb > cap) nb = cap;
  if (nb < 1) nb = 1;
  return (int)nb;
}

int gn_nsplit(int B, int HW) {
  int ns = 512 / (B > 0 ? B : 1);
  if (ns > 128) ns = 128;
  while (ns > 1 && HW / ns < 32) ns >>= 1;
  return ns < 1 ? 1 : ns;
}

int launch_gn_stats(const GnStatsParams& p, int dtype, hipStream_t s) {
  const int C = p.C0 + p.C1;
  if (p.groups != 32 || C % 128 != 0 || p.C0 % 4 != 0) return k22_set_error(K22_EINVAL, "gn_stats: need 32 groups, C % 128 == 0");
  if (C / 4 > 768) return k22_set_error(K22_EINVAL, "gn_stats: C too large (max 3072)");
  if (C / 4 < 256 && (256 / (C / 4)) * C > 2048) return k22_set_error(K22_EINVAL, "gn_stats: internal LDS bound");
  dim3 grid(p.nsplit, p.B);
  if (dtype == K22_BF16) hipLaunchKernelGGL(gn_stats_kernel<bf16_t>, grid, dim3(256), 0, s, p);
  else if (dtype == K22_F16) hipLaunchKernelGGL(gn_stats_kernel<f16_t>, grid, dim3(256), 0, s, p);
  else hipLaunchKernelGGL(gn_stats_kernel<float>, grid, dim3(256), 0, s, p);
  K22_CHECK_LAUNCH();
  return K22_OK;
}
int launch_gn_coeff(const GnCoeffParams& p, int B, hipStream_t s) {
  if (p.C / p.groups > 256) return k22_set_error(K22_EINVAL, "gn_coeff: more than 256 channels per group");
  hipLaunchKernelGGL(gn_coeff_kernel, dim3(p.groups, B), dim3(256), 0, s, p);
  K22_CHECK_LAUNCH();
  return K22_OK;
}
int launch_gn_apply(const GnApplyParams& p, int dtype, hipStream_t s) {
  const int C = p.C0 + p.C1;
  const int epv = dtype == K22_F32 ? 4 : 8;
  if (C % epv || p.C0 % epv) return k22_set_error(K22_EINVAL, "gn_apply: channel alignment");
  if (p.out_x3 && dtype != K22_F32) return k22_set_error(K22_EINVAL, "gn_apply: x3-chunk output is an option of the fp32 launch");
  const int Ho = p.mode == 1 ? p.H / 2 : (p.mode == 2 ? p.H * 2 : p.H);
  const int Wo = p.mode == 1 ? p.W / 2 : (p.mode == 2 ? p.W * 2 : p.W);
  const int Hp = Ho + 2 * p.pad, Wp = Wo + 2 * p.pad;
  if (Hp > 65535 || p.B > 65535) return k22_set_error(K22_EINVAL, "gn_apply: tensor too large");
  dim3 grid((Wp * (C / epv) + 255) / 256, Hp, p.B);
  if (dtype == K22_BF16) hipLaunchKernelGGL(gn_apply_kernel<bf16_t>, grid, dim3(256), 0, s, p);
  else if (dtype == K22_F16) hipLaunchKernelGGL(gn_apply_kernel<f16_t>, grid, dim3(256), 0, s, p);
  else hipLaunchKernelGGL(gn_apply_kernel<float>, grid, dim3(256), 0, s, p);
  K22_CHECK_LAUNCH();
  return K22_OK;
}
int launch_resample(const void* x, void* y, int B, int H, int W, int C, int mode, int dtype, hipStream_t s) {
  const int epv = dtype == K22_F32 ? 4 : 8;
  const int Ho = mode == 1 ? H / 2 : H * 2, Wo = mode == 1 ? W / 2 : W * 2;
  const int nb = grid_for((int64_t)B * Ho * Wo * (C / epv), 256, 8192);
  if (dtype == K22_BF16) hipLaunchKernelGGL(resample_kernel<bf16_t>, dim3(nb), dim3(256), 0, s, x, y, B, H, W, C, mode);
  else if (dtype == K22_F16) hipLaunchKernelGGL(resample_kernel<f16_t>, dim3(nb), dim3(256), 0, s, x, y, B, H, W, C, mode);
  else hipLaunchKernelGGL(resample_kernel<float>, dim3(nb), dim3(256), 0, s, x, y, B, H, W, C, mode);
  K22_CHECK_LAUNCH();
  return K22_OK;
}
int launch_conv_in(const ConvInParams& p, int dtype, hipStream_t s) {
  dim3 grid((p.W + CONV_IN_PT - 1) / CONV_IN_PT, p.H, p.B);
  if (p.Cin == 4) {
    if (dtype == K22_BF16) hipLaunchKernelGGL((conv_in_kernel<bf16_t, 4>), grid, dim3(128), 0, s, p);
    else if (dtype == K22_F16) hipLaunchKernelGGL((conv_in_kernel<f16_t, 4>), grid, dim3(128), 0, s, p);
    else hipLaunchKernelGGL((conv_in_kernel<float, 4>), grid, dim3(128), 0, s, p);
  } else if (p.Cin == 9) {
    if (dtype == K22_BF16) hipLaunchKernelGGL((conv_in_kernel<bf16_t, 9>), grid, dim3(128), 0, s, p);
    else if (dtype == K22_F16) hipLaunchKernelGGL((conv_in_kernel<f16_t, 9>), grid, dim3(128), 0, s, p);
    else hipLaunchKernelGGL((conv_in_kernel<float, 9>), grid, dim3(128), 0, s, p);
  } else if (p.Cin == 8) {
    if (dtype == K22_BF16) hipLaunchKernelGGL((conv_in_kernel<bf16_t, 8>), grid, dim3(128), 0, s, p);
    else if (dtype == K22_F16) hipLaunchKernelGGL((conv_in_kernel<f16_t, 8>), grid, dim3(128), 0, s, p);
    else hipLaunchKernelGGL((conv_in_kernel<float, 8>), grid, dim3(128), 0, s, p);
  } else {
    return k22_set_error(K22_EINVAL, "conv_in: in_channels must be 4, 8 or 9");
  }
  K22_CHECK_LAUNCH();
  return K22_OK;
}
int launch_conv3x3_direct(const ConvDirectParams& p, hipStream_t s) {
  if (p.stride != 1 && p.stride != 2) return k22_set_error(K22_EINVAL, "conv3x3_direct: stride must be 1 or 2");
  const int Ho = (p.Hin - 1) / p.stride + 1, Wo = (p.Win - 1) / p.stride + 1;
  constexpr int OCB = 8;
  dim3 grid((Ho * Wo + 255) / 256, (p.Cout + OCB - 1) / OCB, p.B);
  hipLaunchKernelGGL((conv3x3_direct_kernel<OCB>), grid, dim3(256), 0, s, p);
  K22_CHECK_LAUNCH();
  return K22_OK;
}
int launch_timestep_embedding(const float* t, const float* freqs, float* out, int B, int half, hipStream_t s) {
  hipLaunchKernelGGL(timestep_embedding_kernel, dim3((B * half + 255) / 256), dim3(256), 0, s, t, freqs, out, B, half);
  K22_CHECK_LAUNCH();
  return K22_OK;
}
template <typename TW>
static void launch_linear_m(const LinearSmallParams& p, int Mt, dim3 grid, size_t smem, hipStream_t s) {
  switch (Mt) {
    case 1: hipLaunchKernelGGL((linear_smallm_kernel<TW, 1>), grid, dim3(256), smem, s, p); break;
    case 2: hipLaunchKernelGGL((linear_smallm_kernel<TW, 2>), grid, dim3(256), smem, s, p); break;
    case 4: hipLaunchKernelGGL((linear_smallm_kernel<TW, 4>), grid, dim3(256), smem, s, p); break;
    default: hipLaunchKernelGGL((linear_smallm_kernel<TW, 8>), grid, dim3(256), smem, s, p); break;
  }
}
int launch_linear_smallm(const LinearSmallParams& p0, int wdtype, hipStream_t s) {
  if (p0.M > 8 || p0.M < 1) return k22_set_error(K22_EINVAL, "linear_smallm: M must be in 1..8");
  const int epc = wdtype == K22_F32 ? 4 : 8;
  if (p0.K % epc) return k22_set_error(K22_EINVAL, "linear_smallm: K alignment");
  const int Mt = p0.M <= 2 ? p0.M : (p0.M <= 4 ? 4 : 8);
  const size_t smem = (size_t)Mt * p0.K * 4;
  if (smem > 64 * 1024) return k22_set_error(K22_EINVAL, "linear_smallm: M*K too large for the LDS stage");
  LinearSmallParams p = p0;
  int rpw = 1;
  while (rpw < 8 && (p.N + 8 * rpw - 1) / (8 * rpw) >= 1024) rpw *= 2;
  p.rows_per_wave = rpw;
  dim3 grid((p.N + 4 * rpw - 1) / (4 * rpw));
  if (wdtype == K22_BF16) launch_linear_m<bf16_t>(p, Mt, grid, smem, s);
  else if (wdtype == K22_F16) launch_linear_m<f16_t>(p, Mt, grid, smem, s);
  else launch_linear_m<float>(p, Mt, grid, smem, s);
  K22_CHECK_LAUNCH();
  return K22_OK;
}
int launch_layernorm_f32(const float* x, const float* g, const float* b, float* y, int rows, int D, float eps, hipStream_t s) {
  hipLaunchKernelGGL(layernorm_f32_kernel, dim3(rows), dim3(256), 0, s, x, g, b, y, D, eps);
  K22_CHECK_LAUNCH();
  return K22_OK;
}
int launch_cast_rows(const float* x, void* y, int rows, int cols, int64_t ldx, int64_t ldy, int dtype, hipStream_t s) {
  const int nb = grid_for((int64_t)rows * cols, 256, 4096);
  if (dtype == K22_BF16) hipLaunchKernelGGL(cast_rows_kernel<bf16_t>, dim3(nb), dim3(256), 0, s, x, y, rows, cols, ldx, ldy);
  else if (dtype == K22_F16) hipLaunchKernelGGL(cast_rows_kernel<f16_t>, dim3(nb), dim3(256), 0, s, x, y, rows, cols, ldx, ldy);
  else hipLaunchKernelGGL(cast_rows_kernel<float>, dim3(nb), dim3(256), 0, s, x, y, rows, cols, ldx, ldy);
  K22_CHECK_LAUNCH();
  return K22_OK;
}
int launch_kv_pack(const KvPackParams& p, int dtype, hipStream_t s) {
  if (p.Tkp % 64) return k22_set_error(K22_EINVAL, "kv_pack: Tkp % 64");
  dim3 grid(p.Tkp / 64, p.H, p.B);
  if (dtype == K22_BF16) hipLaunchKernelGGL(kv_pack_kernel<bf16_t>, grid, dim3(256), 0, s, p);
  else if (dtype == K22_F16) hipLaunchKernelGGL(kv_pack_kernel<f16_t>, grid, dim3(256), 0, s, p);
  else hipLaunchKernelGGL(kv_pack_kernel<float>, grid, dim3(256), 0, s, p);
  K22_CHECK_LAUNCH();
  return K22_OK;
}
```

kandinsky-2_amd/csrc/engine.hip:

```cpp
#include "kernels.h"
#include "elementwise.h"
#include "../../include/k22.h"
#include "tuning.h"
#include "plan.h"

#include <atomic>
#include <deque>
#include <functional>
#include <map>
#include <memory>
#include <string>
#include <tuple>
#include <unordered_map>
#include <vector>
#include <stdio.h>
#include <stdlib.h>
#include <string.h>

int launch_step_advance(int* step, int delta, hipStream_t s);

static std::atomic<long> g_loop_captures{0}, g_loop_launches{0};
long loop_capture_count() { return g_loop_captures.load(); }
long loop_launch_count() { return g_loop_launches.load(); }
void loop_count_capture() { g_loop_captures.fetch_add(1); }
void loop_count_launch() { g_loop_launches.fetch_add(1); }
enum : unsigned long long { K22_LOOP_KIND_P = 0, K22_LOOP_KIND_DDIM = 1, K22_LOOP_KIND_PLMS = 2 };

namespace {

enum OpKind { OP_CONV3 = 0, OP_GEMM = 1, OP_GN = 2, OP_ATTN = 3, OP_MISC = 4, OP_NKINDS = 5 };

struct Op {
  std::function<int(hipStream_t)> fn;
  int kind = OP_MISC;
  double flops = 0.0;
  double flops2 = 0.0;
  double bytes = 0.0;
  int kernels = 1;
  Op() {}
  template <typename F> Op(F f, int k = OP_MISC, double fl = 0.0, double by = 0.0, int nk = 1) : fn(f), kind(k), flops(fl), bytes(by), kernels(nk) {}
  int operator()(hipStream_t st) const { return fn(st); }
};
typedef std::vector<Op> OpList;

struct Act {
  Slot* s0 = nullptr; int C0 = 0;
  Slot* s1 = nullptr; int C1 = 0;
  int H = 0, W = 0;
  const Tuned* p0 = nullptr; Slot* st0 = nullptr;
  const Tuned* p1 = nullptr; Slot* st1 = nullptr;
  int C() const { return C0 + C1; }
};

}

struct K22UNet : GraphPlan {
  K22UNetConfig cfg;
  int sdt;

  int B = 0, H = 0, W = 0;
  OpList ops;
  OpList cond_ops;
  OpList hint_ops;
  bool hint_set = false;
  int fuse_skip = 1;
  int fuse_gn = 0;
  struct GnLink { const Tuned* consumer = nullptr; };
  std::deque<GnLink> gn_links;
  int stream_frag = 1;
  struct FragJob { const void* W; Slot* slot; int Npad, taps, Kc; };
  std::vector<FragJob> frag_jobs;
  bool frag_done = false;
  int repack_frags(hipStream_t st) {
    for (auto& j : frag_jobs) {
      int rc = launch_stream_repack(j.W, ptr(j.slot), j.Npad, j.taps, j.Kc, dtype, st);
      if (rc) return rc;
    }
    frag_done = true;
    return K22_OK;
  }
  bool cond_set = false;
  GraphCache loop;
  std::vector<unsigned long long> loop_key;

  Slot *s_xin, *s_img, *s_mask, *s_t, *s_out;
  Slot *s_temb, *s_e1, *s_emb, *s_film, *s_xfproj, *s_ctx;
  Slot *s_full, *s_pool, *s_imgemb, *s_tmpf, *s_tmpf2, *s_fullT;
  Slot *s_part, *s_coeff, *s_P1, *s_U1, *s_P2, *s_S, *s_N, *s_QKV, *s_KALL, *s_VT, *s_ATT, *s_splitk, *s_flush;
  Slot *s_U1st;
  Slot *s_ctxf = nullptr, *s_hint = nullptr, *s_hintin = nullptr, *s_hbuf[2] = {nullptr, nullptr};
  Slot* s_h[3];
  Slot* s_hst[3];
  std::vector<Slot*> s_ctxkv;
  int n_attn = 0;
  int64_t film_total = 0;
  float* film_all = nullptr;
  size_t film_all_bytes = 0;
  int hoist_time = 1;
  const float* film_cur = nullptr;
  const float* film_base() const { return film_cur ? film_cur : ptr<float>(s_film); }
  struct TimeW { const float* freqs; const float* w0; const float* b0; const float* w2; const float* b2; const void* we; const float* be; int mc, ted, dt; } tw = {};
  int time_rows(const float* t, float* temb, float* e1, float* emb, float* film, int rows, hipStream_t st) {
    int rc = launch_timestep_embedding(t, tw.freqs, temb, rows, tw.mc / 2, st);
    if (rc) return rc;
    LinearSmallParams lp = {};
    lp.x = temb; lp.ldx = tw.mc; lp.W = tw.w0; lp.bias = tw.b0; lp.out = e1; lp.ldo = tw.ted;
    lp.M = rows; lp.N = tw.ted; lp.K = tw.mc; lp.act_in = K22_ACT_NONE; lp.act_out = K22_ACT_SILU;
    rc = launch_linear_smallm(lp, K22_F32, st);
    if (rc) return rc;
    lp.x = e1; lp.ldx = tw.ted; lp.W = tw.w2; lp.bias = tw.b2; lp.add = ptr<float>(s_xfproj); lp.ld_add = tw.ted; lp.add_mod = B;
    lp.out = emb; lp.K = tw.ted; lp.act_out = K22_ACT_NONE;
    rc = launch_linear_smallm(lp, K22_F32, st);
    if (rc) return rc;
    LinearSmallParams le = {};
    le.x = emb; le.ldx = tw.ted; le.W = tw.we; le.bias = tw.be; le.out = film; le.ldo = film_total;
    le.M = rows; le.N = (int)film_total; le.K = tw.ted; le.act_in = K22_ACT_SILU; le.act_out = K22_ACT_NONE;
    return launch_linear_smallm(le, tw.dt, st);
  }

  float* model_out() { return ptr<float>(s_out); }
  int exec(hipStream_t st) { return run_ops(st); }
  int exec_eager(hipStream_t st) { return run_eager(st, [this](hipStream_t s) { return exec(s); }); }
  int prepare_run(hipStream_t st) {
    if (!frag_done) { int rc = repack_frags(st); if (rc) return rc; }
    return tune_once(s_flush, st);
  }

  ~K22UNet() {
    if (film_all) (void)hipFree(film_all);
  }

  struct LoopRows {
    bool hoist = false;
    float *film = nullptr, *temb = nullptr, *e1 = nullptr, *emb = nullptr;
  };
  int loop_begin(int n_calls, hipStream_t st, LoopRows* lr) {
    if (int rc = prepare_run(st)) return rc;
    lr->hoist = B <= 8 && hoist_time;
    if (!lr->hoist) return K22_OK;
    const int64_t rows_all = (int64_t)n_calls * B;
    const size_t need = (size_t)rows_all * (size_t)(film_total + tw.mc + 2 * tw.ted) * sizeof(float);
    if (need > film_all_bytes) {
      loop.drop();
      if (film_all) { (void)hipStreamSynchronize(st); (void)hipFree(film_all); film_all = nullptr; film_all_bytes = 0; }
      const hipError_t e = hipMalloc(reinterpret_cast<void**>(&film_all), need);
      if (e != hipSuccess) { film_all = nullptr; return k22_set_error_hip(e, __FILE__, __LINE__); }
      film_all_bytes = need;
    }
    lr->film = film_all;
    lr->temb = lr->film + rows_all * film_total;
    lr->e1 = lr->temb + rows_all * tw.mc;
    lr->emb = lr->e1 + rows_all * tw.ted;
    return K22_OK;
  }
  int loop_prologue(const LoopRows& lr, const float* timesteps, int n_calls, const float* inpaint_image, const float* inpaint_mask, hipStream_t s) {
    if (lr.hoist) {
      const int spl = 8 / B;
      for (int k0 = 0; k0 < n_calls; k0 += spl) {
        const int rows = (n_calls - k0 < spl ? n_calls - k0 : spl) * B;
        const int64_t r0 = (int64_t)k0 * B;
        const int rc = time_rows(timesteps + r0, lr.temb + r0 * tw.mc, lr.e1 + r0 * tw.ted, lr.emb + r0 * tw.ted, lr.film + r0 * film_total, rows, s);
        if (rc) return rc;
      }
    }
    if (cfg.in_channels == 9) {
      const size_t pb = (size_t)B, hw = (size_t)H * W;
      if (int rc = copy_d2d(ptr(s_img), inpaint_image, pb * 4 * hw * 4, s)) return rc;
      if (int rc = copy_d2d(ptr(s_mask), inpaint_mask, pb * hw * 4, s)) return rc;
    }
    return K22_OK;
  }
  int loop_model(const LoopRows& lr, const float* cur, const float* timesteps, int call, hipStream_t s) {
    const size_t half = (size_t)(B / 2) * 4 * H * W * sizeof(float);
    if (int rc = copy_d2d(ptr(s_xin), cur, half, s)) return rc;
    if (int rc = copy_d2d(ptr(s_xin) + half, cur, half, s)) return rc;
    if (lr.hoist) {
      film_cur = lr.film + (int64_t)call * B * film_total;
    } else {
      if (int rc = copy_d2d(ptr(s_t), timesteps + (size_t)call * B, (size_t)B * 4, s)) return rc;
    }
    return exec(s);
  }
  template <typename F> int loop_run(const std::vector<unsigned long long>& key, const float* timesteps, const float* inpaint_image,
                                     const float* inpaint_mask, int use_graph, hipStream_t st, F body) {
    auto run_loop = [&](hipStream_t s) -> int { const int rc = body(s); film_cur = nullptr; return rc; };
    if (!use_graph) {
      const int rc = run_loop(st);
      if (rc == K22_OK) loop_count_launch();
      return rc;
    }
    if (!loop || key != loop_key) {
      if (!warmed) {
        const size_t pb = (size_t)B, hw = (size_t)H * W;
        hipError_t e = hipMemsetAsync(ptr(s_xin), 0, pb * 4 * hw * 4, st);
        if (e != hipSuccess) return k22_set_error_hip(e, __FILE__, __LINE__);
        if (int rc = copy_d2d(ptr(s_t), timesteps, pb * 4, st)) return rc;
        if (cfg.in_channels == 9) {
          if (int rc = copy_d2d(ptr(s_img), inpaint_image, pb * 4 * hw * 4, st)) return rc;
          if (int rc = copy_d2d(ptr(s_mask), inpaint_mask, pb * hw * 4, st)) return rc;
        }
        if (int rc = exec_eager(st)) return rc;
        e = hipStreamSynchronize(st);
        if (e != hipSuccess) return k22_set_error_hip(e, __FILE__, __LINE__);
      }
      if (int rc = loop.capture(cap, run_loop)) return rc;
      loop_key = key;
      loop_count_capture();
    }
    const int rc = loop.launch(st);
    if (rc == K22_OK) loop_count_launch();
    return rc;
  }

  int run_ops_range(hipStream_t st, size_t lo, size_t hi) {
    for (size_t i = lo; i < hi && i < ops.size(); ++i) { int rc = ops[i](st); if (rc) return rc; }
    return K22_OK;
  }
  int run_ops(hipStream_t st) { return run_ops_range(st, 0, ops.size()); }

  void op_gn(OpList& L, const Act& in, const std::string& pfx, int64_t film_off,
             int act, int mode, int pad, Slot* dst, const GnLink* link = nullptr) {
    const int Bn = B, C = in.C(), HW = in.H * in.W;
    const int nsplit = gn_nsplit(Bn, HW);
    const bool fused = in.st0 != nullptr && (in.s1 == nullptr || in.st1 != nullptr);
    if (!fused) need(s_part, (size_t)Bn * nsplit * C * 2 * sizeof(float));
    need(s_coeff, (size_t)Bn * C * 2 * sizeof(float));
    const int Ho = mode == 1 ? in.H / 2 : (mode == 2 ? in.H * 2 : in.H);
    const int Wo = mode == 1 ? in.W / 2 : (mode == 2 ? in.W * 2 : in.W);
    need(dst, (size_t)Bn * (Ho + 2 * pad) * (Wo + 2 * pad) * C * esz);
    const float* gamma = Wf(pfx + ".weight");
    const float* beta = Wf(pfx + ".bias");
    const Act a = in;
    const int dt = sdt;
    const int x3 = k22_is_split(dtype) ? 1 : 0;
    const double gn_bytes = (double)Bn * HW * C * esz * (fused ? 1.0 : 2.0) + (double)Bn * (Ho + 2 * pad) * (Wo + 2 * pad) * C * esz;
    L.push_back(Op([=](hipStream_t st) {
      const void* x0 = ptr(a.s0);
      const void* x1 = a.s1 ? ptr(a.s1) : nullptr;
      GnCoeffParams cp = {};
      if (fused) {
        cp.src[0].st = ptr<float>(a.st0); cp.src[0].rpi = a.p0->rpi; cp.src[0].C = a.C0;
        if (a.s1) { cp.src[1].st = ptr<float>(a.st1); cp.src[1].rpi = a.p1->rpi; cp.src[1].C = a.C1; }
        if (cp.src[0].rpi <= 0 || (a.s1 && cp.src[1].rpi <= 0)) return k22_set_error(K22_EINVAL, "unet: producer delivered no GroupNorm partial sums");
      } else {
        GnStatsParams sp;
        sp.x0 = x0; sp.x1 = x1; sp.C0 = a.C0; sp.C1 = a.C1;
        sp.HW = HW; sp.B = Bn; sp.groups = 32; sp.nsplit = nsplit; sp.partial = ptr<float>(s_part);
        int rc = launch_gn_stats(sp, dt, st);
        if (rc) return rc;
        cp.src[0].st = ptr<float>(s_part); cp.src[0].rpi = nsplit; cp.src[0].C = C;
      }
      cp.HW = HW; cp.C = C; cp.groups = 32; cp.eps = 1e-5f;
      cp.gamma = gamma; cp.beta = beta;
      cp.film = film_off >= 0 ? film_base() + film_off : nullptr; cp.film_ld = film_total;
      cp.coeff = ptr<float>(s_coeff);
      GnApplyParams ap = {};
      ap.x0 = x0; ap.x1 = x1; ap.C0 = a.C0; ap.C1 = a.C1; ap.B = Bn; ap.H = a.H; ap.W = a.W;
      ap.mode = mode; ap.pad = pad; ap.act = act; ap.coeff = ptr<float>(s_coeff); ap.out = ptr(dst); ap.out_x3 = x3;
      int rc = launch_gn_coeff(cp, Bn, st);
      if (rc) return rc;
      if (link != nullptr && link->consumer != nullptr && conv3_algo_fuses_gn(link->consumer->cfg.algo)) return K22_OK;
      return launch_gn_apply(ap, dt, st);
    }, OP_GN, 0.0, gn_bytes, fused ? 2 : 3));
  }

  static void apply_cfg(IgemmParams& q, const Cfg& c) { tuned_apply_cfg(q, c); }
  int op_dt(const Tuned& t) const { return t.dt >= 0 ? t.dt : dtype; }
  void make_candidates(Tuned& t) { tuned_make_candidates(t, op_dt(t)); }
  void default_cfg(Tuned& t) { tuned_default_cfg(t, op_dt(t)); }
  void finish_cfg(Tuned& t) { tuned_finish_cfg(t, op_dt(t)); }
  size_t max_splitk_bytes(const Tuned& t) const { return tuned_max_splitk_bytes(t, op_dt(t), autotune != 0); }
  int max_rpi(const Tuned& t) const { return tuned_max_rpi(t, op_dt(t), autotune != 0); }

  int x2_plan = 0;
  enum ConvRole { CONV_IN = 0, CONV_OUT = 1, CONV_HEAD = 2 };
  int conv_dt(int role, int Hc) const {
    if (dtype != K22_F16X2) return dtype;
    if (role == CONV_HEAD) return K22_F16X3;
    if (Hc >= H) return (x2_plan >> role) & 1 ? K22_F16X2 : K22_F16X3;
    return K22_F16X2;
  }
  int gemm_dt(bool qkv) const { return dtype == K22_F16X2 ? (qkv ? K22_F16X2 : K22_F16X3) : dtype; }

  Tuned* op_conv(OpList& L, int role, Slot* src, int Hc, int Wc, int Cin, int Cout,
                 const std::string& pfx, const Act* residual, Slot* dst, int out_mode, Slot* stats = nullptr,
                 const Act* skip_in = nullptr, const std::string& skip_pfx = std::string(), const Act* gn_in = nullptr, int gn_act = K22_ACT_NONE) {
    tuned.emplace_back();
    Tuned* t = &tuned.back();
    t->dt = conv_dt(role, Hc);
    IgemmParams& p = t->p;
    p = igemm_conv3_problem(B, Hc, Wc, Cin, Cout, out_mode);
    p.Wp = W_(pfx + ".weight"); p.bias = Wf(pfx + ".bias");
    Act sk;
    if (skip_in) {
      sk = *skip_in;
      p.S0 = reinterpret_cast<const void*>(1); p.S1 = sk.s1 ? reinterpret_cast<const void*>(1) : nullptr;
      p.SK0 = sk.C0; p.SK1 = sk.C1;
      p.Ws = W_(skip_pfx + ".weight"); p.bias2 = Wf(skip_pfx + ".bias");
    }
    t->want_stats = stats != nullptr;
    Slot *wf = nullptr, *wsf = nullptr;
    if (stream_frag && k22_esz(dtype) == 2 && p.M <= 1152 && (stream_supported(p, dtype, 5) || stream_supported(p, dtype, 9))) {
      wf = new_slot();
      need(wf, stream_frag_bytes(p.Npad, 9, Cin, dtype));
      frag_jobs.push_back({p.Wp, wf, p.Npad, 9, Cin});
      p.Wfrag = reinterpret_cast<const void*>(1);
      if (skip_in) {
        wsf = new_slot();
        need(wsf, stream_frag_bytes(p.Npad, 1, p.SK0 + p.SK1, dtype));
        frag_jobs.push_back({p.Ws, wsf, p.Npad, 1, p.SK0 + p.SK1});
        p.Wsfrag = reinterpret_cast<const void*>(1);
      }
    }
    make_candidates(*t);
    default_cfg(*t);
    if (wf && t->cfg.algo != IG_ALGO_STREAM && (t->from_table || !autotune)) {
      wf->bytes = 0; wf = nullptr;
      if (wsf) { wsf->bytes = 0; wsf = nullptr; frag_jobs.pop_back(); }
      frag_jobs.pop_back();
      p.Wfrag = nullptr; p.Wsfrag = nullptr;
      make_candidates(*t);
      default_cfg(*t);
    }
    need(s_splitk, max_splitk_bytes(*t));
    if (t->want_stats) need(stats, (size_t)B * max_rpi(*t) * Cout * 2 * sizeof(float));
    need(dst, out_mode == IG_OUT_ROWMAJOR ? (size_t)p.M * Cout * esz : (size_t)p.M * Cout * sizeof(float));
    Slot* rs = residual ? residual->s0 : nullptr;
    const int dt = t->dt;
    const bool gnf = gn_in != nullptr && fuse_gn;
    Act ga;
    if (gnf) ga = *gn_in;
    t->run = [=](hipStream_t st) {
      IgemmParams q = t->p;
      apply_cfg(q, t->cfg);
      q.A0 = ptr(src); q.residual = rs ? ptr(rs) : nullptr; q.out = ptr(dst); q.partial = ptr<float>(s_splitk);
      if (gnf && conv3_algo_fuses_gn(t->cfg.algo)) {
        q.gn_coeff = ptr<float>(s_coeff); q.gn_x0 = ptr(ga.s0); q.gn_x1 = ga.s1 ? ptr(ga.s1) : nullptr; q.gn_C0 = ga.C0; q.gn_act = gn_act;
      }
      q.stats = t->want_stats ? ptr<float>(stats) : nullptr;
      if (q.S0) { q.S0 = ptr(sk.s0); q.S1 = sk.s1 ? ptr(sk.s1) : nullptr; }
      q.Wfrag = wf ? ptr(wf) : nullptr; q.Wsfrag = wsf ? ptr(wsf) : nullptr;
      return launch_igemm(q, dt, st);
    };
    const double fl = 2.0 * p.M * (double)p.N * 9.0 * p.Kc;
    L.push_back(Op([=](hipStream_t st) { return t->run(st); }, OP_CONV3, fl, 0.0, 1));
    if (skip_in) L.back().flops2 = 2.0 * p.M * (double)p.N * (p.SK0 + p.SK1);
    return t;
  }

  Tuned* op_gemm(OpList& L, const Act& in, int M, int N, const std::string& pfx,
                 const Act* residual, Slot* dst, int ldo = 0, int out_mode = IG_OUT_ROWMAJOR, Slot* stats = nullptr, bool a_raw = false) {
    tuned.emplace_back();
    Tuned* t = &tuned.back();
    t->dt = gemm_dt(out_mode == IG_OUT_QKV);
    IgemmParams& p = t->p;
    p = igemm_gemm_problem(M, N, in.C0, in.C1, out_mode);
    if (ldo) p.ldo = ldo;
    if (in.H > 0 && in.W > 0 && M % (in.H * in.W) == 0 && M / (in.H * in.W) == B) { p.H = in.H; p.W = in.W; }
    if (out_mode == IG_OUT_QKV) p.att_T = in.H * in.W;
    p.Wp = W_(pfx + ".weight"); p.bias = Wf(pfx + ".bias");
    p.a_raw = (a_raw && k22_is_split(dtype)) ? 1 : 0;
    t->want_stats = stats != nullptr && p.H > 0;
    make_candidates(*t);
    if (t->want_stats && t->cands.empty()) { t->want_stats = false; make_candidates(*t); }
    default_cfg(*t);
    need(s_splitk, max_splitk_bytes(*t));
    if (t->want_stats) need(stats, (size_t)B * max_rpi(*t) * N * 2 * sizeof(float));
    need(dst, (size_t)M * p.ldo * esz);
    const Act a = in;
    Slot* rs = residual ? residual->s0 : nullptr;
    const int dt = t->dt;
    t->run = [=](hipStream_t st) {
      IgemmParams q = t->p;
      apply_cfg(q, t->cfg);
      q.A0 = ptr(a.s0); q.A1 = a.s1 ? ptr(a.s1) : nullptr;
      q.residual = rs ? ptr(rs) : nullptr; q.out = ptr(dst); q.partial = ptr<float>(s_splitk);
      if (t->aux0) { q.kall = ptr(reinterpret_cast<Slot*>(t->aux0)); q.vtall = ptr(reinterpret_cast<Slot*>(t->aux1)); }
      q.stats = t->want_stats ? ptr<float>(stats) : nullptr;
      return launch_igemm(q, dt, st);
    };
    L.push_back(Op([=](hipStream_t st) { return t->run(st); }, OP_GEMM, 2.0 * p.M * (double)p.N * p.Kc, 0.0, 1));
    return t;
  }

  Act resblock(const std::string& pfx, const Act& in, int Cout, int updown, int64_t& film_cursor, Slot* dst, Slot* dst_stats) {
    const int Cin = in.C();
    const int Ho = updown == 1 ? in.H / 2 : (updown == 2 ? in.H * 2 : in.H);
    const int Wo = updown == 1 ? in.W / 2 : (updown == 2 ? in.W * 2 : in.W);
    GnLink* l1 = nullptr;
    if (fuse_gn && updown == 0) { gn_links.emplace_back(); l1 = &gn_links.back(); }
    op_gn(ops, in, pfx + ".in_layers.0", -1, K22_ACT_SILU, updown, 1, s_P1, l1);
    Tuned* t1 = op_conv(ops, CONV_IN, s_P1, Ho, Wo, Cin, Cout, pfx + ".in_layers.2", nullptr, s_U1, IG_OUT_ROWMAJOR, s_U1st, nullptr, std::string(),
                        l1 ? &in : nullptr, K22_ACT_SILU);
    if (l1) l1->consumer = t1;
    Act u1; u1.s0 = s_U1; u1.C0 = Cout; u1.H = Ho; u1.W = Wo;
    if (t1->want_stats) { u1.p0 = t1; u1.st0 = s_U1st; }
    const int64_t film_off = film_cursor;
    film_cursor += 2 * Cout;
    GnLink* l2 = nullptr;
    if (fuse_gn) { gn_links.emplace_back(); l2 = &gn_links.back(); }
    op_gn(ops, u1, pfx + ".out_layers.0", film_off, K22_ACT_SILU, 0, 1, s_P2, l2);
    Act skip;
    skip.H = Ho; skip.W = Wo; skip.C0 = Cout;
    if (updown) {
      if (Cin != Cout || in.s1) { if (err.empty()) err = "updown ResBlock with channel change is not supported"; }
      need(s_S, (size_t)B * Ho * Wo * Cin * esz);
      const Act a = in; const int Bn = B, dt = sdt;
      ops.push_back([=](hipStream_t st) { return launch_resample(ptr(a.s0), ptr(s_S), Bn, a.H, a.W, Cin, updown, dt, st); });
      skip.s0 = s_S;
    } else if (Cin != Cout) {
      IgemmParams probe = igemm_conv3_problem(B, Ho, Wo, Cout, Cout);
      probe.S0 = reinterpret_cast<const void*>(1); probe.S1 = in.s1 ? reinterpret_cast<const void*>(1) : nullptr;
      probe.SK0 = in.C0; probe.SK1 = in.C1; probe.Ws = reinterpret_cast<const void*>(1);
      if (fuse_skip && Cout >= 128 && (conv3_halo_supported(probe, dtype, 256) || conv3_halo_supported(probe, dtype, 128))) {
        Tuned* t2 = op_conv(ops, CONV_OUT, s_P2, Ho, Wo, Cout, Cout, pfx + ".out_layers.3", nullptr, dst, IG_OUT_ROWMAJOR, dst_stats,
                            &in, pfx + ".skip_connection", l2 ? &u1 : nullptr, K22_ACT_SILU);
        if (l2) l2->consumer = t2;
        Act out; out.s0 = dst; out.C0 = Cout; out.H = Ho; out.W = Wo;
        if (t2->want_stats) { out.p0 = t2; out.st0 = dst_stats; }
        return out;
      }
      op_gemm(ops, in, B * Ho * Wo, Cout, pfx + ".skip_connection", nullptr, s_S, 0, IG_OUT_ROWMAJOR, nullptr, true);
      skip.s0 = s_S;
    } else {
      if (in.s1) { if (err.empty()) err = "identity skip over a concat input"; }
      skip.s0 = in.s0;
    }
    Tuned* t2 = op_conv(ops, CONV_OUT, s_P2, Ho, Wo, Cout, Cout, pfx + ".out_layers.3", &skip, dst, IG_OUT_ROWMAJOR, dst_stats, nullptr, std::string(),
                        l2 ? &u1 : nullptr, K22_ACT_SILU);
    if (l2) l2->consumer = t2;
    Act out; out.s0 = dst; out.C0 = Cout; out.H = Ho; out.W = Wo;
    if (t2->want_stats) { out.p0 = t2; out.st0 = dst_stats; }
    return out;
  }

  Act attnblock(const std::string& pfx, const Act& in, Slot* dst, Slot* dst_stats = nullptr) {
    const int C = in.C0, T = in.H * in.W, Hh = C / 64, S = cfg.ctx_len;
    const int Tk = S + T, Tkp = (Tk + 63) / 64 * 64;
    n_attn++;
    op_gn(ops, in, pfx + ".norm", -1, K22_ACT_NONE, 0, 0, s_N);
    Act n; n.s0 = s_N; n.C0 = C; n.H = in.H; n.W = in.W;
    Slot* kall = new_slot((size_t)B * Hh * Tkp * 64 * esz);
    Slot* vtall = new_slot((size_t)B * Hh * Tkp * 64 * esz);
    Slot* ckv = new_slot((size_t)B * S * 2 * C * esz);
    s_ctxkv.push_back(ckv);
    const int Bn = B, dt = dtype, sd = sdt;
    {
      Act c; c.s0 = s_ctx; c.C0 = cfg.ctx_dim; c.H = 1; c.W = S;
      op_gemm(cond_ops, c, B * S, 2 * C, pfx + ".encoder_kv", nullptr, ckv, 0, IG_OUT_ROWMAJOR, nullptr, true);
      cond_ops.push_back(Op([=](hipStream_t st) {
        KvPackParams kp;
        kp.qkv = nullptr; kp.ctxkv = ptr(ckv); kp.kall = ptr(kall); kp.vtall = ptr(vtall);
        kp.B = Bn; kp.H = Hh; kp.T = 0; kp.S = S; kp.Tkp = Tkp;
        return launch_kv_pack(kp, sd, st);
      }));
    }
    need(s_QKV, (size_t)B * T * C * esz);
    {
      Tuned* t = op_gemm(ops, n, B * T, 3 * C, pfx + ".qkv", nullptr, s_QKV, C, IG_OUT_QKV);
      t->p.att_T = T; t->p.att_S = S; t->p.att_Tkp = Tkp;
      t->aux0 = kall; t->aux1 = vtall;
    }
    need(s_ATT, (size_t)B * T * C * esz);
    ops.push_back(Op([=](hipStream_t st) {
      AttentionParams ap = {};
      ap.q = ptr(s_QKV); ap.ldq = C; ap.kall = ptr(kall); ap.vtall = ptr(vtall); ap.out = ptr(s_ATT); ap.ldo = C;
      ap.B = Bn; ap.H = Hh; ap.T = T; ap.Tk = Tk; ap.Tkp = Tkp; ap.scale = 0.125f;
      ap.out_x3 = k22_is_split(dt) ? 1 : 0;
      return launch_attention(ap, dt, st);
    }, OP_ATTN, 4.0 * Bn * Hh * (double)T * Tk * 64.0, 0.0, 1));
    Act a; a.s0 = s_ATT; a.C0 = C; a.H = in.H; a.W = in.W;
    Tuned* tp = op_gemm(ops, a, B * T, C, pfx + ".proj_out", &in, dst, 0, IG_OUT_ROWMAJOR, dst_stats);
    Act out; out.s0 = dst; out.C0 = C; out.H = in.H; out.W = in.W;
    if (tp->want_stats) { out.p0 = tp; out.st0 = dst_stats; }
    return out;
  }

  bool has_attn(int ds) const {
    for (int i = 0; i < cfg.n_attention_ds; ++i) if (cfg.attention_ds[i] == ds) return true;
    return false;
  }

  int plan(int nB, int nH, int nW) {
    const int n_down = cfg.n_levels - 1;
    if (nB < 1 || nH < 1 || nW < 1) return k22_set_error(K22_EINVAL, "unet: B, H, W must be positive");
    if (nH % (1 << n_down) || nW % (1 << n_down)) return k22_set_error(K22_EINVAL, "unet: H, W must be divisible by 2^(levels-1)");
    if (nB > 8) return k22_set_error(K22_EINVAL, "unet: batch (2*bs) must be <= 8 per engine call");
    begin_plan();
    B = nB; H = nH; W = nW;
    gn_links.clear();
    ops.clear(); cond_ops.clear(); hint_ops.clear(); s_ctxkv.clear(); frag_jobs.clear(); frag_done = false; n_attn = 0;
    cond_set = false; hint_set = false;
    loop.drop();
    const int mc = cfg.model_channels, ted = 4 * mc;

    film_total = 0;
    {
      int ch = mc * cfg.channel_mult[0];
      for (int l = 0; l < cfg.n_levels; ++l) {
        for (int i = 0; i < cfg.num_res_blocks; ++i) { ch = mc * cfg.channel_mult[l]; film_total += 2 * ch; }
        if (l != cfg.n_levels - 1) film_total += 2 * ch;
      }
      film_total += 2 * 2 * ch;
      for (int l = cfg.n_levels - 1; l >= 0; --l)
        for (int i = 0; i <= cfg.num_res_blocks; ++i) {
          ch = mc * cfg.channel_mult[l];
          film_total += 2 * ch;
          if (l && i == cfg.num_res_blocks) film_total += 2 * ch;
        }
    }

    s_xin = new_slot((size_t)B * 4 * H * W * 4); s_img = new_slot((size_t)B * 4 * H * W * 4);
    s_mask = new_slot((size_t)B * H * W * 4); s_t = new_slot((size_t)B * 4 + 64);
    s_out = new_slot((size_t)B * cfg.out_channels * H * W * 4);
    s_temb = new_slot((size_t)B * mc * 4); s_e1 = new_slot((size_t)B * ted * 4); s_emb = new_slot((size_t)B * ted * 4);
    s_film = new_slot((size_t)B * film_total * 4); s_xfproj = new_slot((size_t)B * ted * 4);
    s_ctx = new_slot((size_t)B * cfg.ctx_len * cfg.ctx_dim * esz);
    const int ntext_p = cfg.ctx_len - cfg.n_image_embs;
    s_full = new_slot((size_t)B * (ntext_p > 0 ? ntext_p : 1) * cfg.text_dim1 * 4); s_pool = new_slot((size_t)B * cfg.text_dim2 * 4);
    s_imgemb = new_slot((size_t)B * cfg.image_dim * 4);
    s_tmpf = new_slot((size_t)B * cfg.n_image_embs * cfg.ctx_dim * 4 + (size_t)B * ted * 4);
    s_tmpf2 = new_slot((size_t)B * ted * 4);
    s_fullT = new_slot((size_t)B * (ntext_p > 0 ? ntext_p : 1) * cfg.text_dim1 * esz);
    s_ctxf = new_slot(cfg.head_type == 1 ? (size_t)B * cfg.ctx_len * cfg.ctx_dim * 4 : 0);
    if (cfg.hint_channels) {
      s_hint = new_slot((size_t)B * 4 * H * W * 4);
      s_hintin = new_slot((size_t)B * cfg.hint_channels * 64 * H * W * 4);
      for (int i = 0; i < 2; ++i) s_hbuf[i] = new_slot((size_t)B * 16 * 64 * H * W * 4);
    }
    s_part = new_slot(); s_coeff = new_slot(); s_P1 = new_slot(); s_U1 = new_slot(); s_P2 = new_slot(); s_S = new_slot();
    s_N = new_slot(); s_QKV = new_slot(); s_KALL = new_slot(); s_VT = new_slot(); s_ATT = new_slot();
    s_splitk = new_slot(256);
    s_U1st = new_slot();
    s_flush = new_slot(autotune ? ((size_t)320 << 20) : 0);
    for (int i = 0; i < 3; ++i) { s_h[i] = new_slot(); s_hst[i] = new_slot(); }
    int hrot = 0, hcur = 0;
    auto next_h = [&]() { hcur = hrot; hrot = (hrot + 1) % 3; return s_h[hcur]; };
    auto cur_hst = [&]() { return s_hst[hcur]; };

    if (cfg.head_type == 1) build_cond_ops_22(); else build_cond_ops();
    if (cfg.hint_channels) build_hint_ops();

    {
      tw.freqs = Wf("time_freqs");
      tw.w0 = Wf("time_embed.0.weight"); tw.b0 = Wf("time_embed.0.bias");
      tw.w2 = Wf("time_embed.2.weight"); tw.b2 = Wf("time_embed.2.bias");
      tw.we = W_("emb_layers.weight"); tw.be = Wf("emb_layers.bias");
      tw.mc = mc; tw.ted = ted; tw.dt = sdt;
      const int Bn = B;
      ops.push_back([=](hipStream_t st) {
        if (film_cur) return (int)K22_OK;
        return time_rows(ptr<float>(s_t), ptr<float>(s_temb), ptr<float>(s_e1), ptr<float>(s_emb), ptr<float>(s_film), Bn, st);
      });
    }

    int64_t film_cursor = 0;
    std::vector<Act> hs;
    int ch = mc * cfg.channel_mult[0];
    {
      Slot* d = new_slot((size_t)B * H * W * ch * esz);
      ConvInParams cp = {};
      cp.w = Wf("input_blocks.0.0.weight"); cp.bias = Wf("input_blocks.0.0.bias");
      cp.B = B; cp.H = H; cp.W = W; cp.Cin = cfg.in_channels; cp.Cout = ch;
      const int dt = sdt; const bool inpaint = cfg.in_channels == 9, hinted = cfg.in_channels == 8;
      const int premul = (hinted || cfg.head_type == 1) ? 1 : 0;
      ops.push_back([=](hipStream_t st) {
        ConvInParams q = cp;
        q.x = ptr<float>(s_xin); q.img = inpaint ? ptr<float>(s_img) : (hinted ? ptr<float>(s_hint) : nullptr);
        q.mask = inpaint ? ptr<float>(s_mask) : nullptr; q.img_premul = premul;
        q.out = ptr(d);
        return launch_conv_in(q, dt, st);
      });
      Act a; a.s0 = d; a.C0 = ch; a.H = H; a.W = W;
      hs.push_back(a);
    }
    Act h = hs.back();
    int ds = 1, blk = 1;
    for (int l = 0; l < cfg.n_levels; ++l) {
      for (int i = 0; i < cfg.num_res_blocks; ++i) {
        const int co = mc * cfg.channel_mult[l];
        const std::string pfx = "input_blocks." + std::to_string(blk);
        Slot* d = new_slot();
        if (has_attn(ds)) {
          Slot* rd = next_h();
          Act r = resblock(pfx + ".0", h, co, 0, film_cursor, rd, cur_hst());
          h = attnblock(pfx + ".1", r, d, new_slot());
        } else {
          h = resblock(pfx + ".0", h, co, 0, film_cursor, d, new_slot());
        }
        ch = co; hs.push_back(h); ++blk;
      }
      if (l != cfg.n_levels - 1) {
        const std::string pfx = "input_blocks." + std::to_string(blk);
        Slot* d = new_slot();
        h = resblock(pfx + ".0", h, ch, 1, film_cursor, d, new_slot());
        hs.push_back(h); ++blk; ds *= 2;
      }
    }
    {
      Slot* d0 = next_h(); Slot* st0 = cur_hst();
      Act r = resblock("middle_block.0", h, ch, 0, film_cursor, d0, st0);
      Slot* da = next_h(); Slot* sta = cur_hst();
      Act a = attnblock("middle_block.1", r, da, sta);
      Slot* d2 = next_h(); Slot* st2 = cur_hst();
      h = resblock("middle_block.2", a, ch, 0, film_cursor, d2, st2);
    }
    blk = 0;
    for (int l = cfg.n_levels - 1; l >= 0; --l) {
      for (int i = 0; i <= cfg.num_res_blocks; ++i) {
        const Act skip = hs.back(); hs.pop_back();
        Act cat; cat.s0 = h.s0; cat.C0 = h.C0; cat.s1 = skip.s0; cat.C1 = skip.C0; cat.H = h.H; cat.W = h.W;
        cat.p0 = h.p0; cat.st0 = h.st0; cat.p1 = skip.p0; cat.st1 = skip.st0;
        if (skip.H != h.H || skip.W != h.W) return k22_set_error(K22_EINVAL, "unet: skip shape mismatch");
        const int co = mc * cfg.channel_mult[l];
        const std::string pfx = "output_blocks." + std::to_string(blk);
        { Slot* d = next_h(); Slot* dst_st = cur_hst(); h = resblock(pfx + ".0", cat, co, 0, film_cursor, d, dst_st); }
        int sub = 1;
        if (has_attn(ds)) { Slot* da = next_h(); Slot* sta = cur_hst(); h = attnblock(pfx + "." + std::to_string(sub), h, da, sta); ++sub; }
        if (l && i == cfg.num_res_blocks) {
          { Slot* d = next_h(); Slot* dst_st = cur_hst(); h = resblock(pfx + "." + std::to_string(sub), h, co, 2, film_cursor, d, dst_st); }
          ds /= 2;
        }
        ch = co; ++blk;
      }
    }
    if (film_cursor != film_total) return k22_set_error(K22_EINVAL, "unet: internal FiLM width mismatch");
    op_gn(ops, h, "out.0", -1, K22_ACT_SILU, 0, 1, s_P1);
    op_conv(ops, CONV_HEAD, s_P1, H, W, ch, cfg.out_channels, "out.2", nullptr, s_out, IG_OUT_NCHW_F32);

    return finish_plan();
  }

  void build_cond_ops_22() {
    const int mc = cfg.model_channels, ted = 4 * mc, Bn = B, dt = sdt;
    const int cd = cfg.ctx_dim, S = cfg.ctx_len, di = cfg.image_dim;
    const float* w_cp = Wf("head22.ctx_proj.weight"); const float* b_cp = Wf("head22.ctx_proj.bias");
    const float* g_cn = Wf("head22.ctx_norm.weight"); const float* b_cn = Wf("head22.ctx_norm.bias");
    const float* w_ep = Wf("head22.emb_proj.weight"); const float* b_ep = Wf("head22.emb_proj.bias");
    const float* g_en = Wf("head22.emb_norm.weight"); const float* b_en = Wf("head22.emb_norm.bias");
    cond_ops.push_back([=](hipStream_t st) {
      float* proj = ptr<float>(s_tmpf);
      float* embp = ptr<float>(s_tmpf) + (size_t)Bn * S * cd;
      LinearSmallParams lp = {};
      lp.x = ptr<float>(s_imgemb); lp.ldx = di; lp.W = w_cp; lp.bias = b_cp; lp.out = proj; lp.ldo = S * cd;
      lp.M = Bn; lp.N = S * cd; lp.K = di;
      int rc = launch_linear_smallm(lp, K22_F32, st);
      if (rc) return rc;
      rc = launch_layernorm_f32(proj, g_cn, b_cn, ptr<float>(s_ctxf), Bn * S, cd, 1e-5f, st);
      if (rc) return rc;
      rc = launch_cast_rows(ptr<float>(s_ctxf), ptr(s_ctx), Bn * S, cd, cd, cd, dt, st);
      if (rc) return rc;
      lp.W = w_ep; lp.bias = b_ep; lp.out = embp; lp.ldo = ted; lp.N = ted;
      rc = launch_linear_smallm(lp, K22_F32, st);
      if (rc) return rc;
      return launch_layernorm_f32(embp, g_en, b_en, ptr<float>(s_xfproj), Bn, ted, 1e-5f, st);
    });
  }

  void build_hint_ops() {
    static const int chans[9] = {0, 16, 16, 32, 32, 96, 96, 256, 4};
    static const int strides[8] = {1, 1, 2, 1, 2, 1, 2, 1};
    int hin = 8 * H, win = 8 * W, cin = cfg.hint_channels;
    for (int k = 0; k < 8; ++k) {
      const float* w = Wf("hint." + std::to_string(k) + ".weight");
      const float* b = Wf("hint." + std::to_string(k) + ".bias");
      const int cout = chans[k + 1], stride = strides[k], Bn = B, ci = cin, hi = hin, wi = win;
      Slot* src = k == 0 ? s_hintin : s_hbuf[(k - 1) & 1];
      Slot* dst = k == 7 ? s_hint : s_hbuf[k & 1];
      hint_ops.push_back([=](hipStream_t st) {
        ConvDirectParams q = {};
        q.x = ptr<float>(src); q.w = w; q.bias = b; q.y = ptr<float>(dst);
        q.B = Bn; q.Cin = ci; q.Cout = cout; q.Hin = hi; q.Win = wi; q.stride = stride; q.act = k == 7 ? K22_ACT_NONE : K22_ACT_SILU;
        return launch_conv3x3_direct(q, st);
      });
      cin = cout;
      if (stride == 2) { hin = (hin - 1) / 2 + 1; win = (win - 1) / 2 + 1; }
    }
  }

  void build_cond_ops() {
    const int mc = cfg.model_channels, ted = 4 * mc, Bn = B, dt = sdt;
    const int nie = cfg.n_image_embs, cd = cfg.ctx_dim, S = cfg.ctx_len, ntext = S - nie;
    const float* w_cs = Wf("clip_to_seq.weight"); const float* b_cs = Wf("clip_to_seq.bias");
    const float* w_pn = Wf("proj_n.weight"); const float* b_pn = Wf("proj_n.bias");
    const float* g_ln = Wf("ln_model_n.weight"); const float* b_ln = Wf("ln_model_n.bias");
    const float* w_il = Wf("img_layer.weight"); const float* b_il = Wf("img_layer.bias");
    const int d1 = cfg.text_dim1, d2 = cfg.text_dim2, di = cfg.image_dim;
    cond_ops.push_back([=](hipStream_t st) {
      float* clipseq = ptr<float>(s_tmpf);
      float* proj = ptr<float>(s_tmpf) + (size_t)Bn * nie * cd;
      LinearSmallParams lp = {};
      lp.x = ptr<float>(s_imgemb); lp.ldx = di; lp.W = w_cs; lp.bias = b_cs; lp.out = clipseq; lp.ldo = nie * cd;
      lp.M = Bn; lp.N = nie * cd; lp.K = di;
      int rc = launch_linear_smallm(lp, K22_F32, st);
      if (rc) return rc;
      for (int b = 0; b < Bn; ++b) {
        rc = launch_cast_rows(clipseq + (size_t)b * nie * cd, ptr(s_ctx) + (size_t)b * S * cd * esz, nie, cd, cd, cd, dt, st);
        if (rc) return rc;
      }
      lp.x = ptr<float>(s_pool); lp.ldx = d2; lp.W = w_pn; lp.bias = b_pn; lp.out = proj; lp.ldo = ted; lp.N = ted; lp.K = d2;
      rc = launch_linear_smallm(lp, K22_F32, st);
      if (rc) return rc;
      rc = launch_layernorm_f32(proj, g_ln, b_ln, ptr<float>(s_tmpf2), Bn, ted, 1e-5f, st);
      if (rc) return rc;
      lp.x = ptr<float>(s_imgemb); lp.ldx = di; lp.W = w_il; lp.bias = b_il; lp.add = ptr<float>(s_tmpf2); lp.ld_add = ted;
      lp.out = ptr<float>(s_xfproj); lp.ldo = ted; lp.N = ted; lp.K = di;
      rc = launch_linear_smallm(lp, K22_F32, st);
      if (rc) return rc;
      return launch_cast_rows(ptr<float>(s_full), ptr(s_fullT), Bn * ntext, d1, d1, d1, dt, st);
    });
    {
      IgemmParams p = igemm_gemm_problem(ntext, cd, d1, 0);
      p.splitk = 1;
      p.a_raw = k22_is_split(dtype) ? 1 : 0;
      p.Wp = W_("to_model_dim_n.weight"); p.bias = Wf("to_model_dim_n.bias");
      const size_t es = esz;
      const int gdt = gemm_dt(false);
      cond_ops.push_back([=](hipStream_t st) {
        for (int b = 0; b < Bn; ++b) {
          IgemmParams q = p;
          q.A0 = ptr(s_fullT) + (size_t)b * ntext * d1 * es;
          q.out = ptr(s_ctx) + ((size_t)b * S + nie) * cd * es;
          int rc = launch_igemm(q, gdt, st);
          if (rc) return rc;
        }
        return K22_OK;
      });
    }
  }
};

extern "C" {

int k22_unet_create(const K22UNetConfig* cfg, const K22Weight* weights, int n_weights, K22UNet** out) {
  if (!cfg || !out) return k22_set_error(K22_EINVAL, "unet_create: null argument");
  if (!k22_dtype_ok(cfg->dtype) && !k22_is_split(cfg->dtype)) return k22_set_error(K22_EINVAL, "unet_create: dtype");
  if (cfg->num_head_channels != 64) return k22_set_error(K22_EINVAL, "unet_create: only num_head_channels == 64");
  if (cfg->model_channels % 128) return k22_set_error(K22_EINVAL, "unet_create: model_channels % 128");
  if (cfg->n_levels < 1 || cfg->n_levels > 8) return k22_set_error(K22_EINVAL, "unet_create: n_levels");
  if (cfg->in_channels != 4 && cfg->in_channels != 9 && cfg->in_channels != 8) return k22_set_error(K22_EINVAL, "unet_create: in_channels must be 4, 8 or 9");
  if (cfg->head_type != 0 && cfg->head_type != 1) return k22_set_error(K22_EINVAL, "unet_create: head_type must be 0 (2.1) or 1 (2.2)");
  if ((cfg->hint_channels != 0) != (cfg->in_channels == 8) || (cfg->hint_channels != 0 && cfg->hint_channels != 3))
    return k22_set_error(K22_EINVAL, "unet_create: hint_channels = 3 goes with in_channels = 8 (latent + hint latent), else 0");
  if (cfg->head_type == 1 && cfg->n_image_embs != cfg->ctx_len) return k22_set_error(K22_EINVAL, "unet_create: the 2.2 head has image tokens only (n_image_embs == ctx_len)");
  K22UNet* u = new K22UNet();
  u->cfg = *cfg; u->set_dtype(cfg->dtype); u->sdt = k22_storage_dtype(cfg->dtype);
  u->stream_frag = env_flag("K22_STREAM", 1);
  u->fuse_gn = env_flag("K22_FUSE_GN", 0);
  u->fuse_skip = env_flag("K22_FUSE_SKIP", 1);
  u->hoist_time = env_flag("K22_HOIST_TIME", 1);
  const char* xp = getenv("K22_X2_PLAN");
  u->x2_plan = xp ? (atoi(xp) & 3) : 0;
  u->set_weights(weights, n_weights);
  *out = u;
  return K22_OK;
}

void k22_unet_destroy(K22UNet* u) { delete u; }

int k22_unet_plan(K22UNet* u, int B, int H, int W, size_t* workspace_bytes) {
  if (!u || !workspace_bytes) return k22_set_error(K22_EINVAL, "unet_plan: null argument");
  int rc = u->plan(B, H, W);
  if (rc) return rc;
  *workspace_bytes = u->ws_bytes;
  return K22_OK;
}

int k22_unet_bind(K22UNet* u, void* workspace, size_t workspace_bytes) {
  if (!u) return k22_set_error(K22_EINVAL, "unet_bind: null argument");
  if (int rc = u->bind(workspace, workspace_bytes, "unet_bind")) return rc;
  u->cond_set = false; u->hint_set = false; u->frag_done = false;
  u->loop.drop();
  return K22_OK;
}

int k22_unet_set_condition(K22UNet* u, const float* full_emb, const float* pooled_emb, const float* image_emb, void* stream) {
  if (!u || !u->ws) return k22_set_error(K22_EINVAL, "unet_set_condition: bind a workspace first");
  hipStream_t st = reinterpret_cast<hipStream_t>(stream);
  const K22UNetConfig& c = u->cfg;
  const int ntext = c.ctx_len - c.n_image_embs;
  if (!image_emb) return k22_set_error(K22_EINVAL, "unet_set_condition: image_emb is required");
  if (c.head_type == 0 && (!full_emb || !pooled_emb)) return k22_set_error(K22_EINVAL, "unet_set_condition: the 2.1 head needs full_emb and pooled_emb");
  const size_t pb = (size_t)u->B;
  if (c.head_type == 0) {
    if (int rc = copy_d2d(u->ptr(u->s_full), full_emb, pb * ntext * c.text_dim1 * 4, st)) return rc;
    if (int rc = copy_d2d(u->ptr(u->s_pool), pooled_emb, pb * c.text_dim2 * 4, st)) return rc;
  }
  if (int rc = copy_d2d(u->ptr(u->s_imgemb), image_emb, pb * c.image_dim * 4, st)) return rc;
  for (auto& op : u->cond_ops) { int rc = op(st); if (rc) return rc; }
  u->cond_set = true;
  return K22_OK;
}

int k22_unet_set_hint(K22UNet* u, const float* hint, void* stream) {
  if (!u || !u->ws) return k22_set_error(K22_EINVAL, "unet_set_hint: bind a workspace first");
  if (!u->cfg.hint_channels) return k22_set_error(K22_EINVAL, "unet_set_hint: this UNet has no hint input (hint_channels == 0)");
  if (!hint) return k22_set_error(K22_EINVAL, "unet_set_hint: null hint");
  hipStream_t st = reinterpret_cast<hipStream_t>(stream);
  const size_t per = (size_t)u->B * u->cfg.hint_channels * 64 * u->H * u->W;
  if (int rc = copy_d2d(u->ptr(u->s_hintin), hint, per * 4, st)) return rc;
  for (auto& op : u->hint_ops) { int rc = op(st); if (rc) return rc; }
  u->hint_set = true;
  return K22_OK;
}

int k22_unet_forward(K22UNet* u, const float* x, const float* timesteps, const float* inpaint_image,
                     const float* inpaint_mask, float* out, int use_graph, void* stream) {
  if (!u || !u->ws) return k22_set_error(K22_EINVAL, "unet_forward: bind a workspace first");
  if (!u->cond_set) return k22_set_error(K22_EINVAL, "unet_forward: call k22_unet_set_condition first");
  if (u->cfg.in_channels == 9 && (!inpaint_image || !inpaint_mask)) return k22_set_error(K22_EINVAL, "unet_forward: inpainting UNet needs inpaint_image and inpaint_mask");
  if (u->cfg.hint_channels && !u->hint_set) return k22_set_error(K22_EINVAL, "unet_forward: call k22_unet_set_hint first");
  hipStream_t st = reinterpret_cast<hipStream_t>(stream);
  const size_t hw = (size_t)u->H * u->W;
  const size_t pb = (size_t)u->B;
  if (int rc = copy_d2d(u->ptr(u->s_xin), x, pb * 4 * hw * 4, st)) return rc;
  if (int rc = copy_d2d(u->ptr(u->s_t), timesteps, pb * 4, st)) return rc;
  if (u->cfg.in_channels == 9) {
    if (int rc = copy_d2d(u->ptr(u->s_img), inpaint_image, pb * 4 * hw * 4, st)) return rc;
    if (int rc = copy_d2d(u->ptr(u->s_mask), inpaint_mask, pb * hw * 4, st)) return rc;
  }
  { int rc = u->prepare_run(st); if (rc) return rc; }
  const int rc = use_graph ? u->replay(u->graph, st, [u](hipStream_t s) { return u->exec(s); }) : u->exec_eager(st);
  if (rc) return rc;
  return copy_d2d(out, u->ptr(u->s_out), pb * u->cfg.out_channels * hw * 4, st);
}

int k22_unet_sample_loop(K22UNet* u, float* x, float* x_tmp, const float* timesteps, const float* noise_seq, const float* init_img,
                         const float* mask, const float* inpaint_image, const float* inpaint_mask, const float* table,
                         const int* table_rows, int n_steps, float guidance, float clamp_lo, float clamp_hi, int pct_index,
                         double pct_gamma, void* scratch, int use_graph, void* stream) {
  if (!u || !u->ws) return k22_set_error(K22_EINVAL, "unet_sample_loop: bind a workspace first");
  if (!u->cond_set) return k22_set_error(K22_EINVAL, "unet_sample_loop: call k22_unet_set_condition first");
  if (!x || !x_tmp || !timesteps || !noise_seq || !table || !table_rows || !scratch || n_steps < 1)
    return k22_set_error(K22_EINVAL, "unet_sample_loop: null argument");
  if (u->B % 2) return k22_set_error(K22_EINVAL, "unet_sample_loop: the batch is the CFG batch [cond | uncond] (even)");
  if (u->cfg.out_channels != 8) return k22_set_error(K22_EINVAL, "unet_sample_loop: the UNet must predict eps and variance (8 channels)");
  if (u->cfg.in_channels == 9 && (!inpaint_image || !inpaint_mask)) return k22_set_error(K22_EINVAL, "unet_sample_loop: inpainting UNet needs inpaint_image and inpaint_mask");
  if (u->cfg.hint_channels && !u->hint_set) return k22_set_error(K22_EINVAL, "unet_sample_loop: call k22_unet_set_hint first");
  const int B = u->B, HW = u->H * u->W;
  if (pct_index >= 4 * HW) return k22_set_error(K22_EINVAL, "unet_sample_loop: percentile index out of range");
  hipStream_t st = reinterpret_cast<hipStream_t>(stream);
  K22UNet::LoopRows lr;
  if (int rc = u->loop_begin(n_steps, st, &lr)) return rc;
  auto body = [&](hipStream_t s) -> int {
    if (int rc = u->loop_prologue(lr, timesteps, n_steps, inpaint_image, inpaint_mask, s)) return rc;
    float* cur = x; float* nxt = x_tmp;
    for (int k = 0; k < n_steps; ++k) {
      int rc = u->loop_model(lr, cur, timesteps, k, s);
      if (rc) return rc;
      SamplerParams p = {};
      p.x = cur; p.model_out = u->model_out(); p.noise = noise_seq + (size_t)k * B * 4 * HW; p.init_img = init_img; p.mask = mask;
      p.table = table; p.step = nullptr; p.step_host = table_rows[k]; p.guidance = guidance; p.clamp_lo = clamp_lo; p.clamp_hi = clamp_hi;
      p.use_cfg = 1; p.n_lo = pct_index; p.gamma = pct_gamma;
      p.s_buf = reinterpret_cast<float*>(scratch); p.x0_buf = reinterpret_cast<float*>(scratch) + 64;
      p.x_out = nxt; p.x0_out = nullptr; p.N = B; p.HW = HW;
      rc = launch_sampler_step(p, s);
      if (rc) return rc;
      float* t_ = cur; cur = nxt; nxt = t_;
    }
    if (cur != x) return copy_d2d(x, cur, (size_t)B * 4 * HW * sizeof(float), s);
    return K22_OK;
  };
  std::vector<unsigned long long> key = {K22_LOOP_KIND_P, loop_key_ptr(x), loop_key_ptr(x_tmp), loop_key_ptr(timesteps), loop_key_ptr(noise_seq),
      loop_key_ptr(init_img), loop_key_ptr(mask), loop_key_ptr(inpaint_image), loop_key_ptr(inpaint_mask), loop_key_ptr(table), loop_key_ptr(scratch),
      (unsigned long long)n_steps, (unsigned long long)pct_index, (unsigned long long)(lr.hoist ? 1 : 0),
      loop_key_bits(guidance), loop_key_bits(clamp_lo), loop_key_bits(clamp_hi), loop_key_bits(pct_gamma)};
  for (int k = 0; k < n_steps; ++k) key.push_back((unsigned long long)table_rows[k]);
  return u->loop_run(key, timesteps, inpaint_image, inpaint_mask, use_graph, st, body);
}

int k22_unet_ddim_loop(K22UNet* u, int kind, float* x, float* x_tmp, float* x0_out, const float* timesteps, const float* table,
                       const float* noise_seq, const float* inpaint_image, const float* inpaint_mask, float* eps_hist, int n_steps,
                       float guidance, int use_graph, void* stream) {
  if (!u || !u->ws) return k22_set_error(K22_EINVAL, "unet_ddim_loop: bind a workspace first");
  if (kind != K22_LOOP_DDIM && kind != K22_LOOP_PLMS) return k22_set_error(K22_EINVAL, "unet_ddim_loop: kind must be K22_LOOP_DDIM or K22_LOOP_PLMS");
  if (!u->cond_set) return k22_set_error(K22_EINVAL, "unet_ddim_loop: call k22_unet_set_condition first");
  if (!x || !x_tmp || !timesteps || !table) return k22_set_error(K22_EINVAL, "unet_ddim_loop: null argument");
  if (n_steps < 1) return k22_set_error(K22_EINVAL, "unet_ddim_loop: n_steps must be >= 1");
  if (kind == K22_LOOP_PLMS && noise_seq) return k22_set_error(K22_EINVAL, "unet_ddim_loop: PLMS is eta = 0 (samplers.py:355-356): noise_seq must be NULL");
  if (kind == K22_LOOP_PLMS && !eps_hist) return k22_set_error(K22_EINVAL, "unet_ddim_loop: PLMS needs the eps-history workspace (4 x [B][4][HW] floats)");
  if (u->B % 2) return k22_set_error(K22_EINVAL, "unet_ddim_loop: the batch is the CFG batch [cond | uncond] (even)");
  if (u->cfg.out_channels != 8) return k22_set_error(K22_EINVAL, "unet_ddim_loop: the UNet must predict eps and variance (8 channels)");
  if (u->cfg.in_channels == 9 && (!inpaint_image || !inpaint_mask)) return k22_set_error(K22_EINVAL, "unet_ddim_loop: inpainting UNet needs inpaint_image and inpaint_mask");
  if (u->cfg.hint_channels && !u->hint_set) return k22_set_error(K22_EINVAL, "unet_ddim_loop: call k22_unet_set_hint first");
  const int B = u->B, HW = u->H * u->W;
  const int n_calls = kind == K22_LOOP_PLMS ? n_steps + 1 : n_steps;
  hipStream_t st = reinterpret_cast<hipStream_t>(stream);
  K22UNet::LoopRows lr;
  if (int rc = u->loop_begin(n_calls, st, &lr)) return rc;
  const size_t lat = (size_t)B * 4 * HW;
  auto body = [&](hipStream_t s) -> int {
    if (int rc = u->loop_prologue(lr, timesteps, n_calls, inpaint_image, inpaint_mask, s)) return rc;
    float* cur = x; float* nxt = x_tmp;
    float* old[3] = {nullptr, nullptr, nullptr};
    int n_old = 0, call = 0;
    for (int k = 0; k < n_steps; ++k) {
      const float* row = table + (size_t)k * 4;
      int rc = u->loop_model(lr, cur, timesteps, call++, s);
      if (rc) return rc;
      if (kind == K22_LOOP_DDIM) {
        rc = launch_ddim_step(cur, u->model_out(), noise_seq ? noise_seq + (size_t)k * lat : nullptr, row, guidance, 1, nxt, x0_out, B, HW, s);
        if (rc) return rc;
      } else {
        float* e_buf = nullptr;
        for (int j = 0; j < 4 && !e_buf; ++j) {
          float* c = eps_hist + (size_t)j * lat;
          if (c != old[0] && c != old[1] && c != old[2]) e_buf = c;
        }
        if (n_old == 0) {
          rc = launch_plms_step(cur, u->model_out(), nullptr, nullptr, nullptr, 0, row, guidance, 1, nxt, e_buf, nullptr, B, HW, s);
          if (rc) return rc;
          rc = u->loop_model(lr, nxt, timesteps, call++, s);
          if (rc) return rc;
          rc = launch_plms_step(cur, u->model_out(), e_buf, nullptr, nullptr, 4, row, guidance, 1, nxt, nullptr, x0_out, B, HW, s);
        } else {
          rc = launch_plms_step(cur, u->model_out(), old[0], old[1], old[2], n_old, row, guidance, 1, nxt, e_buf, x0_out, B, HW, s);
        }
        if (rc) return rc;
        old[2] = old[1]; old[1] = old[0]; old[0] = e_buf;
        if (n_old < 3) ++n_old;
      }
      float* t_ = cur; cur = nxt; nxt = t_;
    }
    if (cur != x) return copy_d2d(x, cur, lat * sizeof(float), s);
    return K22_OK;
  };
  const std::vector<unsigned long long> key = {kind == K22_LOOP_DDIM ? K22_LOOP_KIND_DDIM : K22_LOOP_KIND_PLMS, loop_key_ptr(x), loop_key_ptr(x_tmp),
      loop_key_ptr(x0_out), loop_key_ptr(timesteps), loop_key_ptr(table), loop_key_ptr(noise_seq), loop_key_ptr(inpaint_image), loop_key_ptr(inpaint_mask),
      loop_key_ptr(eps_hist), (unsigned long long)n_steps, (unsigned long long)(lr.hoist ? 1 : 0), loop_key_bits(guidance)};
  return u->loop_run(key, timesteps, inpaint_image, inpaint_mask, use_graph, st, body);
}

int k22_unet_num_ops(const K22UNet* u) {
  return u && u->planned ? (int)u->ops.size() : 0;
}

int k22_unet_set_autotune(K22UNet* u, int on) {
  if (!u) return k22_set_error(K22_EINVAL, "unet_set_autotune: null handle");
  if (u->planned && (on != 0) != (u->autotune != 0)) return k22_set_error(K22_EINVAL, "unet_set_autotune: call before k22_unet_plan");
  u->autotune = on ? 1 : 0;
  return K22_OK;
}

int k22_unet_tuning_report(const K22UNet* u, char* buf, size_t cap) {
  if (!u || !buf || cap == 0) return k22_set_error(K22_EINVAL, "unet_tuning_report: null argument");
  const std::string out = tuning_report_text(u->tuned);
  snprintf(buf, cap, "%s", out.c_str());
  return K22_OK;
}

int k22_unet_profile(K22UNet* u, int reps, double* ms, double* flops, double* bytes, int* launches, void* stream) {
  if (!u || !u->ws || !u->cond_set) return k22_set_error(K22_EINVAL, "unet_profile: run k22_unet_forward once first");
  if (reps < 1) reps = 1;
  hipStream_t st = reinterpret_cast<hipStream_t>(stream);
  for (int k = 0; k < OP_NKINDS; ++k) { ms[k] = 0.0; flops[k] = 0.0; bytes[k] = 0.0; launches[k] = 0; }
  int rc = K22_OK;
  {
    K22UNet* q = u;
    if (!q->frag_done) { int rc0 = q->repack_frags(st); if (rc0) return rc0; }
    const size_t n = q->ops.size();
    std::vector<hipEvent_t> ev(2 * n);
    for (auto& e : ev) { hipError_t r = hipEventCreate(&e); if (r != hipSuccess) return k22_set_error_hip(r, __FILE__, __LINE__); }
    for (size_t i = 0; i < n; ++i) {
      flops[q->ops[i].kind] += q->ops[i].flops + q->ops[i].flops2;
      bytes[q->ops[i].kind] += q->ops[i].bytes;
      launches[q->ops[i].kind] += q->ops[i].kernels;
    }
    for (int r = 0; r < reps && rc == K22_OK; ++r) {
      for (size_t i = 0; i < n; ++i) {
        (void)hipEventRecord(ev[2 * i], st);
        rc = q->ops[i](st);
        (void)hipEventRecord(ev[2 * i + 1], st);
        if (rc) break;
      }
      hipError_t e = hipStreamSynchronize(st);
      if (e != hipSuccess) { rc = k22_set_error_hip(e, __FILE__, __LINE__); break; }
      for (size_t i = 0; i < n; ++i) {
        float t = 0.f;
        (void)hipEventElapsedTime(&t, ev[2 * i], ev[2 * i + 1]);
        ms[q->ops[i].kind] += (double)t / reps;
      }
    }
    for (auto& e : ev) (void)hipEventDestroy(e);
  }
  return rc;
}

}
```

kandinsky-2_amd/csrc/kernels.h:

```cpp
#pragma once
#include "common.h"

#include <atomic>
#include <stdint.h>
#include <string.h>
#include <type_traits>

#define K22_OK 0
#define K22_EINVAL (-1)
#define K22_EHIP (-2)
#define K22_ENOMEM (-3)

struct LdsAttrGuard { std::atomic<unsigned long long> done{0}; };
inline int k22_ensure_lds_attr(LdsAttrGuard& g, const void* fn, int bytes, const char* file, int line) {
  int dev = 0;
  (void)hipGetDevice(&dev);
  const unsigned long long bit = 1ull << (dev & 63);
  if (g.done.load(std::memory_order_acquire) & bit) return K22_OK;
  const hipError_t e = hipFuncSetAttribute(fn, hipFuncAttributeMaxDynamicSharedMemorySize, bytes);
  if (e != hipSuccess) return k22_set_error_hip(e, file, line);
  g.done.fetch_or(bit, std::memory_order_release);
  return K22_OK;
}

enum IgemmOut { IG_OUT_ROWMAJOR = 0,
                IG_OUT_ROWMAJOR_F32 = 1,
                IG_OUT_NCHW_F32 = 2,
                IG_OUT_QKV = 3 };

struct IgemmParams {
  const void* A0;
  const void* A1;
  const void* Wp;
  const float* bias;
  const void* residual;
  void* out;
  float* partial;
  int M, N, Npad;
  int Kc;
  int K0;
  int taps;
  int H, W;
  long lda0, lda1;
  int ldo, ldr;
  int out_mode;
  int act;
  int splitk;
  int force_bm, force_bn;
  int stages = -1;
  int xcd_remap;
  int algo;
  const void* S0; const void* S1; const void* Ws; const float* bias2;
  int SK0, SK1;
  void* kall; void* vtall;
  int att_T, att_S, att_Tkp;
  unsigned long long* trace;
  int res_f32;
  float* stats;
  const void* Wfrag; const void* Wsfrag;
  int a_raw;
  const float* gn_coeff; const void* gn_x0; const void* gn_x1; int gn_C0, gn_act;
  unsigned long long* st_trace;
  int st_tm, st_rb, st_mtiles, st_buf;
};
static_assert(sizeof(IgemmParams) == 320 && std::is_trivially_copyable<IgemmParams>::value, "IgemmParams layout");

enum IgemmAlgo {
  IG_ALGO_AUTO = 0,
  IG_ALGO_GENERIC = 1,
  IG_ALGO_HALO = 2,
  IG_ALGO_HALO3 = 3,
  IG_ALGO_HALO_PIPE = 6,
  IG_ALGO_HALO_ASM = 7,
  IG_ALGO_DBG_NO_DMA = 8,
  IG_ALGO_DBG_NO_MFMA = 9,
  IG_ALGO_GEMM8 = 10,
  IG_ALGO_SPEC = 11,
  IG_ALGO_SPEC_PIPE = 12,
  IG_ALGO_DBG_SPEC_NO_DMA = 13,
  IG_ALGO_DBG_SPEC_NO_WAIT = 14,
  IG_ALGO_STREAM = 20
};
struct IgemmAlgoName { int algo; const char* name; };
constexpr IgemmAlgoName IGEMM_ALGO_NAMES[] = {{IG_ALGO_GENERIC, "gen"},   {IG_ALGO_HALO, "halo"},   {IG_ALGO_HALO3, "hal3"}, {IG_ALGO_HALO_PIPE, "hal6"},
                                              {IG_ALGO_HALO_ASM, "hal7"}, {IG_ALGO_GEMM8, "gem8"}, {IG_ALGO_SPEC, "spec"},  {IG_ALGO_SPEC_PIPE, "spcp"}};
inline const char* igemm_algo_name(int algo) {
  for (const IgemmAlgoName& a : IGEMM_ALGO_NAMES) if (a.algo == algo) return a.name;
  return "auto";
}
inline bool igemm_algo_is_halo(int a) { return a == IG_ALGO_HALO || a == IG_ALGO_HALO3 || (a >= IG_ALGO_HALO_PIPE && a <= IG_ALGO_DBG_NO_MFMA) || (a >= IG_ALGO_SPEC && a <= IG_ALGO_DBG_SPEC_NO_WAIT); }
inline bool igemm_algo_is_debug(int a) { return a == IG_ALGO_DBG_NO_DMA || a == IG_ALGO_DBG_NO_MFMA || a == IG_ALGO_DBG_SPEC_NO_DMA || a == IG_ALGO_DBG_SPEC_NO_WAIT; }

inline IgemmParams igemm_gemm_problem(int M, int N, int K0, int K1, int out_mode = IG_OUT_ROWMAJOR, int act = 0) {
  IgemmParams p = {};
  p.M = M; p.N = N; p.Npad = (N + 63) / 64 * 64; p.Kc = K0 + K1; p.K0 = K0; p.taps = 1;
  p.lda0 = K0; p.lda1 = K1; p.ldo = N; p.ldr = N; p.out_mode = out_mode; p.act = act;
  return p;
}
inline IgemmParams igemm_conv3_problem(int B, int H, int W, int Cin, int Cout, int out_mode = IG_OUT_ROWMAJOR, int act = 0) {
  IgemmParams p = {};
  p.M = B * H * W; p.N = Cout; p.Npad = (Cout + 63) / 64 * 64; p.Kc = Cin; p.K0 = Cin; p.taps = 9; p.H = H; p.W = W;
  p.ldo = Cout; p.ldr = Cout; p.out_mode = out_mode; p.act = act;
  return p;
}

enum IgemmFamily { IG_FAM_GENERIC, IG_FAM_HALO, IG_FAM_HALO3, IG_FAM_SPEC, IG_FAM_GEMM8, IG_FAM_GEMM8_SPEC, IG_FAM_STREAM };
enum IgemmFinish { IG_FINISH_NONE, IG_FINISH_FLAT, IG_FINISH_ROWS };
struct IgemmLaunch {
  int family;
  int algo;
  int bm, bn;
  int splitk;
  int depth;
  int pipe;
  int dbg;
  int a_raw;
  int xcd_remap;
  int finish;
  int stats_rows_per_image;
  unsigned grid, block;
  size_t lds;
};
struct IgemmOptions { int conv_algo = 0, gemm_algo = 0, stages = -1, xcd_remap = 1; };
int igemm_resolve(const IgemmParams& p, int dtype, IgemmLaunch* L);

template <typename K>
inline int launch_lds_kernel(K kernel, LdsAttrGuard& guard, unsigned grid, unsigned block, size_t smem, int attr_bytes, hipStream_t stream, const IgemmParams& params) {
  if (int rc = k22_ensure_lds_attr(guard, reinterpret_cast<const void*>(kernel), attr_bytes, __FILE__, __LINE__)) return rc;
  hipLaunchKernelGGL(kernel, dim3(grid), dim3(block), smem, stream, params);
  K22_CHECK_LAUNCH();
  return K22_OK;
}

struct IgemmStatsInfo { int rows_per_image; };
int igemm_stats_rows_per_image(const IgemmParams& p, int dtype);

int launch_igemm(const IgemmParams& p, int dtype, hipStream_t stream);

bool conv3_halo_supported(const IgemmParams& p, int dtype, int bm);
inline bool conv3_algo_fuses_gn(int algo) { return algo == IG_ALGO_SPEC || algo == IG_ALGO_SPEC_PIPE; }
int conv3_halo_tiles_per_image(const IgemmParams& p, int bm);
int conv3_halo_ring(const IgemmParams& p, int bm);
size_t conv3_halo_lds_bytes(const IgemmParams& p, int bm, int depth);
int launch_conv3_halo(const IgemmParams& p, int dtype, const IgemmLaunch& L, hipStream_t stream);
int launch_conv3_halo_spec(const IgemmParams& p, int dtype, const IgemmLaunch& L, hipStream_t stream);
int launch_conv3_halo_trace(const IgemmParams& p, int dtype, hipStream_t stream);
bool gemm8_supported(const IgemmParams& p, int dtype, int bm);
bool gemm8_spec_supported(int dtype);
int gemm8_tiles_per_image(const IgemmParams& p, int bm);
size_t gemm8_lds_bytes(int bm, int depth);
int launch_gemm8(const IgemmParams& p, int dtype, const IgemmLaunch& L, hipStream_t stream);
bool stream_supported(const IgemmParams& p, int dtype, int mb);
int stream_mtiles(const IgemmParams& p, int mb);
size_t stream_lds_bytes(const IgemmParams& p, int mb);
int launch_stream(const IgemmParams& p, int dtype, const IgemmLaunch& L, hipStream_t stream);
long stream_launch_count();
long loop_capture_count();
long loop_launch_count();
void loop_count_capture();
void loop_count_launch();
inline unsigned long long loop_key_ptr(const void* p) { return (unsigned long long)(uintptr_t)p; }
inline unsigned long long loop_key_bits(double v) { unsigned long long b; memcpy(&b, &v, 8); return b; }
size_t stream_frag_bytes(int Npad, int taps, int Kc, int dtype);
int launch_stream_repack(const void* W, void* out, int Npad, int taps, int Kc, int dtype, hipStream_t stream);
void igemm_set_gemm_algo(int v);
void igemm_set_conv_algo(int v);
void igemm_set_default_stages(int v);
void igemm_set_xcd_remap(int v);
void attention_set_pipe(int v);
int igemm_choose_splitk(const IgemmParams& p, int dtype);
```

Before: 147.9 steps/s.

## Fuse stem GN stats, resample into GN apply, add MFMA head conv, in-place loop

The stem conv_in kernel now emits GroupNorm partial sums, so the first GN no longer needs its own stats pass. It also reads the latent with a batch modulo, avoiding a CFG duplication copy. For up/down ResBlocks, gn_apply also writes the raw resampled skip tensor, replacing a separate resample launch. A dedicated MFMA kernel handles the low-Cout output head conv, and the sampler loop can run in place to skip copies. Each piece is behind an env flag that defaults on, so the change adds several new code paths to validate.

```diff
diff --git a/include/k22.h b/include/k22.h
--- a/include/k22.h
+++ b/include/k22.h
@@ -276,6 +276,12 @@
                  const float* film, long film_ld, float eps, float* coeff, void* stream);
 int k22_gn_apply(const void* x0, const void* x1, int C0, int C1, int B, int H, int W, const float* coeff, int act, int mode, int pad, void* out,
                  int dtype, void* stream);
+int k22_conv_in(const float* x, const float* img, const float* mask, const float* w, const float* bias, void* out, float* stats, int* rpi,
+                int B, int H, int W, int Cin, int Cout, int x_bmod, int img_premul, int dtype, void* stream);
+int k22_gn_apply_raw(const void* x0, int C0, int B, int H, int W, const float* coeff, int act, int mode, int pad, void* out, void* raw_out,
+                     int dtype, void* stream);
+int k22_resample(const void* x, void* y, int B, int H, int W, int C, int mode, int dtype, void* stream);
+int k22_conv_head(const void* x_padded, const void* Wp, const float* bias, float* out, int B, int H, int W, int Cin, int Cout, int dtype, void* stream);
 
 #ifdef __cplusplus
 }
diff --git a/kandinsky-2_amd/_lib.py b/kandinsky-2_amd/_lib.py
--- a/kandinsky-2_amd/_lib.py
+++ b/kandinsky-2_amd/_lib.py
@@ -172,6 +172,10 @@
     "k22_gn_stats": (_I, [_P, _P, _I, _I, _I, _I, _P, C.POINTER(_I), _I, _P]),
     "k22_gn_coeff": (_I, [_P, _I, _I, _P, _I, _I, _I, _I, _P, _P, _P, _L, _F, _P, _P]),
     "k22_gn_apply": (_I, [_P, _P, _I, _I, _I, _I, _I, _P, _I, _I, _I, _P, _I, _P]),
+    "k22_conv_in": (_I, [_P, _P, _P, _P, _P, _P, _P, C.POINTER(_I), _I, _I, _I, _I, _I, _I, _I, _I, _P]),
+    "k22_gn_apply_raw": (_I, [_P, _I, _I, _I, _I, _P, _I, _I, _I, _P, _P, _I, _P]),
+    "k22_resample": (_I, [_P, _P, _I, _I, _I, _I, _I, _I, _P]),
+    "k22_conv_head": (_I, [_P, _P, _P, _P, _I, _I, _I, _I, _I, _I, _P]),
 }
 
 _lib = None
diff --git a/kandinsky-2_amd/csrc/capi.hip b/kandinsky-2_amd/csrc/capi.hip
--- a/kandinsky-2_amd/csrc/capi.hip
+++ b/kandinsky-2_amd/csrc/capi.hip
@@ -82,6 +82,9 @@
   if (name && !strcmp(name, "stream_launches")) return stream_launch_count();
   if (name && !strcmp(name, "loop_captures")) return loop_capture_count();
   if (name && !strcmp(name, "loop_launches")) return loop_launch_count();
+  if (name && !strcmp(name, "gn_stats_launches")) return gn_stats_launch_count();
+  if (name && !strcmp(name, "resample_launches")) return resample_launch_count();
+  if (name && !strcmp(name, "loop_copies")) return loop_copy_count();
   return -1;
 }
 
@@ -551,6 +554,46 @@
   return launch_gn_apply(ap, k22_storage_dtype(dtype), reinterpret_cast<hipStream_t>(stream));
 }
 
+int k22_conv_in(const float* x, const float* img, const float* mask, const float* w, const float* bias, void* out, float* stats, int* rpi,
+                int B, int H, int W, int Cin, int Cout, int x_bmod, int img_premul, int dtype, void* stream) {
+  if (rpi) *rpi = 0;
+  if (!x || !w || !bias || !out || B < 1 || B > 65535 || H < 1 || H > 65535 || W < 1 || Cout < 1 || !(aux_dtype_ok(dtype) || k22_is_split(dtype)))
+    return k22_set_error(K22_EINVAL, "conv_in: bad argument");
+  if (Cin != 4 && Cin != 8 && Cin != 9) return k22_set_error(K22_EINVAL, "conv_in: in_channels must be 4, 8 or 9");
+  if (x_bmod < 1 || x_bmod > B) return k22_set_error(K22_EINVAL, "conv_in: x_bmod must be in 1..B");
+  if (Cin >= 8 && !img) return k22_set_error(K22_EINVAL, "conv_in: 8 / 9 input channels need img");
+  if (Cin == 9 && !mask) return k22_set_error(K22_EINVAL, "conv_in: 9 input channels need mask");
+  if (Cin == 8 && !img_premul) return k22_set_error(K22_EINVAL, "conv_in: 8 input channels take img as it is (img_premul)");
+  ConvInParams p = {};
+  p.x = x; p.img = Cin >= 8 ? img : nullptr; p.mask = Cin == 9 ? mask : nullptr; p.w = w; p.bias = bias; p.out = out;
+  p.B = B; p.H = H; p.W = W; p.Cin = Cin; p.Cout = Cout; p.img_premul = img_premul ? 1 : 0; p.x_bmod = x_bmod; p.stats = stats;
+  if (rpi) *rpi = conv_in_rpi(H, W);
+  return launch_conv_in(p, k22_storage_dtype(dtype), reinterpret_cast<hipStream_t>(stream));
+}
+int k22_gn_apply_raw(const void* x0, int C0, int B, int H, int W, const float* coeff, int act, int mode, int pad, void* out, void* raw_out,
+                     int dtype, void* stream) {
+  if (!x0 || !coeff || !out || !raw_out || C0 < 1 || B < 1 || H < 1 || W < 1 || (mode != 1 && mode != 2) || (mode == 1 && (H < 2 || W < 2)) ||
+      (pad != 0 && pad != 1) || (act != K22_ACT_NONE && act != K22_ACT_SILU) || !(aux_dtype_ok(dtype) || k22_is_split(dtype)))
+    return k22_set_error(K22_EINVAL, "gn_apply_raw: bad argument (mode 1 or 2 of a single tensor, raw_out required)");
+  GnApplyParams ap = {};
+  ap.x0 = x0; ap.C0 = C0; ap.B = B; ap.H = H; ap.W = W; ap.mode = mode; ap.pad = pad; ap.act = act;
+  ap.coeff = coeff; ap.out = out; ap.out_x3 = k22_is_split(dtype) ? 1 : 0; ap.raw_out = raw_out;
+  return launch_gn_apply(ap, k22_storage_dtype(dtype), reinterpret_cast<hipStream_t>(stream));
+}
+int k22_conv_head(const void* x_padded, const void* Wp, const float* bias, float* out, int B, int H, int W, int Cin, int Cout, int dtype, void* stream) {
+  if (!x_padded || !Wp || !bias || !out) return k22_set_error(K22_EINVAL, "conv_head: null argument");
+  ConvHeadParams p = {};
+  p.x = x_padded; p.Wp = Wp; p.bias = bias; p.out = out; p.B = B; p.H = H; p.W = W; p.Cin = Cin; p.Cout = Cout;
+  return launch_conv_head(p, dtype, reinterpret_cast<hipStream_t>(stream));
+}
+int k22_resample(const void* x, void* y, int B, int H, int W, int C, int mode, int dtype, void* stream) {
+  const int sd = k22_storage_dtype(dtype);
+  if (!x || !y || B < 1 || H < 1 || W < 1 || C < 1 || (mode != 1 && mode != 2) || (mode == 1 && (H < 2 || W < 2)) || !(aux_dtype_ok(dtype) || k22_is_split(dtype)) ||
+      C % (sd == K22_F32 ? 4 : 8))
+    return k22_set_error(K22_EINVAL, "resample: bad argument (mode 1 or 2, C a multiple of the 16-byte vector)");
+  return launch_resample(x, y, B, H, W, C, mode, sd, reinterpret_cast<hipStream_t>(stream));
+}
+
 }
 
 __global__ __launch_bounds__(256) void lds_sentinel_kernel(int words, int spins, unsigned* rec) {
diff --git a/kandinsky-2_amd/csrc/conv_head.hip b/kandinsky-2_amd/csrc/conv_head.hip
--- /dev/null
+++ b/kandinsky-2_amd/csrc/conv_head.hip
@@ -0,0 +1,131 @@
+#include "kernels.h"
+#include "elementwise.h"
+
+namespace {
+
+template <typename T> __device__ __forceinline__ f32x4_t head_mma(u32x4_t a, u32x4_t b, f32x4_t c);
+template <> __device__ __forceinline__ f32x4_t head_mma<bf16_t>(u32x4_t a, u32x4_t b, f32x4_t c) {
+  return __builtin_amdgcn_mfma_f32_16x16x32_bf16(__builtin_bit_cast(bf16x8_t, a), __builtin_bit_cast(bf16x8_t, b), c, 0, 0, 0);
+}
+template <> __device__ __forceinline__ f32x4_t head_mma<f16_t>(u32x4_t a, u32x4_t b, f32x4_t c) {
+  return __builtin_amdgcn_mfma_f32_16x16x32_f16(__builtin_bit_cast(f16x8_t, a), __builtin_bit_cast(f16x8_t, b), c, 0, 0, 0);
+}
+
+constexpr int HEAD_BM = 48;
+constexpr int HEAD_NW = 8;
+constexpr int HEAD_LDN = 17;
+
+template <typename T, bool VEC>
+__global__ __launch_bounds__(HEAD_NW * 64) void conv_head_kernel(ConvHeadParams p) {
+  constexpr int MT = HEAD_BM / 16;
+  __shared__ float red[HEAD_NW][HEAD_BM][HEAD_LDN];
+  const int tid = threadIdx.x, lane = tid & 63, wave = tid >> 6;
+  const int row = lane & 15, kq = lane >> 4;
+  const int HW = p.H * p.W, M = p.B * HW;
+  const int m0 = blockIdx.x * HEAD_BM;
+  const int Wp2 = p.W + 2;
+  const T* x = reinterpret_cast<const T*>(p.x);
+  const T* abase[MT];
+#pragma unroll
+  for (int i = 0; i < MT; ++i) {
+    const int m = min(m0 + 16 * i + row, M - 1);
+    const int b = m / HW, rem = m - b * HW, y = rem / p.W, xx = rem - y * p.W;
+    abase[i] = x + (((int64_t)b * (p.H + 2) + y) * Wp2 + xx) * p.Cin + 8 * kq;
+  }
+  const bool nvalid = row < p.Cout;
+  const T* wbase = reinterpret_cast<const T*>(p.Wp) + (int64_t)(nvalid ? row : 0) * 9 * p.Cin + 8 * kq;
+  f32x4_t acc[MT];
+#pragma unroll
+  for (int i = 0; i < MT; ++i) acc[i] = f32x4_t{0.f, 0.f, 0.f, 0.f};
+  const int spt = p.Cin / 32, KS = 9 * spt;
+  struct Frags { u32x4_t a[2][MT], b[2]; };
+  auto fetch = [&](int ks, Frags& f) {
+#pragma unroll
+    for (int h = 0; h < 2; ++h) {
+      const int k = ks + h * HEAD_NW;
+      if (k < KS) {
+        const int tap = k / spt, c0 = (k - tap * spt) * 32;
+        const int r = tap / 3, q = tap - 3 * r;
+        const int64_t aoff = ((int64_t)r * Wp2 + q) * p.Cin + c0;
+        f.b[h] = *reinterpret_cast<const u32x4_t*>(wbase + (int64_t)k * 32);
+#pragma unroll
+        for (int i = 0; i < MT; ++i) f.a[h][i] = *reinterpret_cast<const u32x4_t*>(abase[i] + aoff);
+      } else {
+        f.b[h] = u32x4_t{0u, 0u, 0u, 0u};
+#pragma unroll
+        for (int i = 0; i < MT; ++i) f.a[h][i] = u32x4_t{0u, 0u, 0u, 0u};
+      }
+      if (!nvalid) f.b[h] = u32x4_t{0u, 0u, 0u, 0u};
+    }
+  };
+  auto multiply = [&](const Frags& f) {
+#pragma unroll
+    for (int h = 0; h < 2; ++h)
+#pragma unroll
+      for (int i = 0; i < MT; ++i) acc[i] = head_mma<T>(f.a[h][i], f.b[h], acc[i]);
+  };
+  Frags f0, f1;
+  fetch(wave, f0);
+  for (int ks = wave; ks < KS; ks += 4 * HEAD_NW) {
+    fetch(ks + 2 * HEAD_NW, f1);
+    multiply(f0);
+    fetch(ks + 4 * HEAD_NW, f0);
+    multiply(f1);
+  }
+#pragma unroll
+  for (int i = 0; i < MT; ++i)
+#pragma unroll
+    for (int g = 0; g < 4; ++g) red[wave][16 * i + 4 * kq + g][row] = acc[i][g];
+  __syncthreads();
+  if constexpr (VEC) {
+    if (tid < (HEAD_BM / 4) * p.Cout) {
+      const int n = tid / (HEAD_BM / 4), px = (tid - n * (HEAD_BM / 4)) * 4, m = m0 + px;
+      if (m < M) {
+        const float bias = p.bias[n];
+        float v[4];
+#pragma unroll
+        for (int j = 0; j < 4; ++j) {
+          float s = red[0][px + j][n];
+#pragma unroll
+          for (int w = 1; w < HEAD_NW; ++w) s += red[w][px + j][n];
+          v[j] = s + bias;
+        }
+        const int b = m / HW, rem = m - b * HW;
+        *reinterpret_cast<float4*>(p.out + ((int64_t)b * p.Cout + n) * HW + rem) = make_float4(v[0], v[1], v[2], v[3]);
+      }
+    }
+  } else {
+    for (int idx = tid; idx < HEAD_BM * p.Cout; idx += HEAD_NW * 64) {
+      const int n = idx / HEAD_BM, px = idx - n * HEAD_BM, m = m0 + px;
+      if (m >= M) continue;
+      float s = red[0][px][n];
+#pragma unroll
+      for (int w = 1; w < HEAD_NW; ++w) s += red[w][px][n];
+      const int b = m / HW, rem = m - b * HW;
+      p.out[((int64_t)b * p.Cout + n) * HW + rem] = s + p.bias[n];
+    }
+  }
+}
+
+}
+
+bool conv_head_supported(int B, int H, int W, int Cin, int Cout, int dtype) {
+  return (dtype == K22_BF16 || dtype == K22_F16) && B >= 1 && H >= 1 && W >= 1 && Cout >= 1 && Cout <= 16 && Cin >= 32 && Cin % 32 == 0 &&
+         (int64_t)B * H * W <= 0x7fffffff - HEAD_BM && (int64_t)B * (H + 2) * (W + 2) * Cin <= ((int64_t)1 << 40);
+}
+
+int launch_conv_head(const ConvHeadParams& p, int dtype, hipStream_t s) {
+  if (!conv_head_supported(p.B, p.H, p.W, p.Cin, p.Cout, dtype)) return k22_set_error(K22_EINVAL, "conv_head: 16-bit operands, Cout <= 16, Cin % 32 == 0");
+  const int M = p.B * p.H * p.W;
+  const dim3 grid((M + HEAD_BM - 1) / HEAD_BM), block(HEAD_NW * 64);
+  const bool vec = p.W % 4 == 0 && (reinterpret_cast<uintptr_t>(p.out) & 15) == 0;
+  if (dtype == K22_BF16) {
+    if (vec) hipLaunchKernelGGL((conv_head_kernel<bf16_t, true>), grid, block, 0, s, p);
+    else hipLaunchKernelGGL((conv_head_kernel<bf16_t, false>), grid, block, 0, s, p);
+  } else {
+    if (vec) hipLaunchKernelGGL((conv_head_kernel<f16_t, true>), grid, block, 0, s, p);
+    else hipLaunchKernelGGL((conv_head_kernel<f16_t, false>), grid, block, 0, s, p);
+  }
+  K22_CHECK_LAUNCH();
+  return K22_OK;
+}
diff --git a/kandinsky-2_amd/csrc/elementwise.h b/kandinsky-2_amd/csrc/elementwise.h
--- a/kandinsky-2_amd/csrc/elementwise.h
+++ b/kandinsky-2_amd/csrc/elementwise.h
@@ -23,6 +23,7 @@
   const float* coeff;
   void* out;
   int out_x3;
+  void* raw_out;
 };
 struct ConvInParams {
   const float* x; const float* img; const float* mask;
@@ -30,7 +31,19 @@
   void* out;
   int B, H, W, Cin, Cout;
   int img_premul;
+  int x_bmod;
+  float* stats;
 };
+int conv_in_rpi(int H, int W);
+struct ConvHeadParams {
+  const void* x;
+  const void* Wp;
+  const float* bias;
+  float* out;
+  int B, H, W, Cin, Cout;
+};
+bool conv_head_supported(int B, int H, int W, int Cin, int Cout, int dtype);
+int launch_conv_head(const ConvHeadParams& p, int dtype, hipStream_t s);
 struct ConvDirectParams {
   const float* x; const float* w; const float* bias; float* y;
   int B, Cin, Cout, Hin, Win, stride, act;
@@ -108,6 +121,8 @@
 }
 int launch_gn_apply(const GnApplyParams& p, int dtype, hipStream_t s);
 int launch_resample(const void* x, void* y, int B, int H, int W, int C, int mode, int dtype, hipStream_t s);
+long gn_stats_launch_count();
+long resample_launch_count();
 int launch_conv_in(const ConvInParams& p, int dtype, hipStream_t s);
 int launch_timestep_embedding(const float* t, const float* freqs, float* out, int B, int half, hipStream_t s);
 int launch_linear_smallm(const LinearSmallParams& p, int wdtype, hipStream_t s);
diff --git a/kandinsky-2_amd/csrc/elementwise.hip b/kandinsky-2_amd/csrc/elementwise.hip
--- a/kandinsky-2_amd/csrc/elementwise.hip
+++ b/kandinsky-2_amd/csrc/elementwise.hip
@@ -1,5 +1,7 @@
 #include "kernels.h"
 #include "elementwise.h"
+#include "conv3_common.h"
+#include <atomic>
 
 __device__ __forceinline__ void load4(const bf16_t* p, float* f) {
   const uint2 r = *reinterpret_cast<const uint2*>(p);
@@ -162,7 +164,7 @@
   }
 }
 
-template <typename T>
+template <typename T, bool RAW>
 __global__ __launch_bounds__(256) void gn_apply_kernel(GnApplyParams p) {
   constexpr int EPV = Vec16<T>::N;
   const bool fast = p.out_x3 != 0;
@@ -206,10 +208,24 @@
         for (int q = 0; q < 4; ++q) acc += fast ? apply_act_sel<true>(v[q].get(k) * A[k] + Bc[k], p.act) : apply_act_sel<false>(v[q].get(k) * A[k] + Bc[k], p.act);
         r[k] = acc * 0.25f;
       }
+      if constexpr (RAW) {
+        float s[EPV];
+#pragma unroll
+        for (int k = 0; k < EPV; ++k) s[k] = 0.f;
+#pragma unroll
+        for (int q = 0; q < 4; ++q)
+#pragma unroll
+          for (int k = 0; k < EPV; ++k) s[k] += v[q].get(k);
+        Vec16<T> ro;
+#pragma unroll
+        for (int k = 0; k < EPV / 2; ++k) ro.set2(k, s[2 * k] * 0.25f, s[2 * k + 1] * 0.25f);
+        *reinterpret_cast<decltype(ro.raw)*>(reinterpret_cast<T*>(p.raw_out) + (((int64_t)b * Ho + yo) * Wo + xo) * C + c) = ro.raw;
+      }
     } else {
       const int yi = p.mode == 2 ? yo >> 1 : yo, xi = p.mode == 2 ? xo >> 1 : xo;
       Vec16<T> v;
       v.raw = *reinterpret_cast<const decltype(v.raw)*>(src + ((int64_t)(b * p.H + yi) * p.W + xi) * ld + cs);
+      if constexpr (RAW) *reinterpret_cast<decltype(v.raw)*>(reinterpret_cast<T*>(p.raw_out) + (((int64_t)b * Ho + yo) * Wo + xo) * C + c) = v.raw;
 #pragma unroll
       for (int k = 0; k < EPV; ++k) r[k] = fast ? apply_act_sel<true>(v.get(k) * A[k] + Bc[k], p.act) : apply_act_sel<false>(v.get(k) * A[k] + Bc[k], p.act);
     }
@@ -259,13 +275,19 @@
   }
 }
 
-constexpr int CONV_IN_PT = 8;
+#ifndef K22_CONV_IN_PT
+#define K22_CONV_IN_PT 32
+#endif
+constexpr int CONV_IN_PT = K22_CONV_IN_PT;
+int conv_in_rpi(int H, int W) { return H * ((W + CONV_IN_PT - 1) / CONV_IN_PT); }
 template <typename T, int CIN>
 __global__ __launch_bounds__(128) void conv_in_kernel(ConvInParams p) {
   constexpr int PT = CONV_IN_PT, PW = PT + 2;
   __shared__ float patch[CIN][3][PW];
   const int tid = threadIdx.x;
-  const int xt = blockIdx.x, y = blockIdx.y, b = blockIdx.z;
+  const int nch = (p.Cout + 127) / 128;
+  const int xt = blockIdx.x / nch, n = (blockIdx.x - xt * nch) * 128 + tid, y = blockIdx.y, b = blockIdx.z;
+  const int bx = b % p.x_bmod;
   const int x0 = xt * PT;
   const int hw = p.H * p.W;
   for (int i = tid; i < CIN * 3 * PW; i += 128) {
@@ -274,29 +296,42 @@
     float v = 0.f;
     if (yy >= 0 && yy < p.H && xs >= 0 && xs < p.W) {
       const int64_t o = (int64_t)yy * p.W + xs;
-      if (c < 4) v = p.x[((int64_t)b * 4 + c) * hw + o];
+      if (c < 4) v = p.x[((int64_t)bx * 4 + c) * hw + o];
       else if (c < 8) v = p.img[((int64_t)b * 4 + (c - 4)) * hw + o] * (p.img_premul ? 1.f : p.mask[(int64_t)b * hw + o]);
       else v = p.mask[(int64_t)b * hw + o];
     }
     patch[c][r][xx] = v;
   }
   __syncthreads();
-  T* out = reinterpret_cast<T*>(p.out);
-  for (int n = tid; n < p.Cout; n += 128) {
-    float w[CIN * 9];
-#pragma unroll
-    for (int k = 0; k < CIN * 9; ++k) w[k] = p.w[(int64_t)k * p.Cout + n];
-    const float bias = p.bias[n];
-    for (int px = 0; px < PT && x0 + px < p.W; ++px) {
+  if (n >= p.Cout) return;
+  T* out = reinterpret_cast<T*>(p.out) + ((int64_t)(b * p.H + y) * p.W + x0) * p.Cout + n;
+  float w[CIN * 9];
+#pragma unroll
+  for (int k = 0; k < CIN * 9; ++k) w[k] = p.w[(int64_t)k * p.Cout + n];
+  const float bias = p.bias[n];
+  const int npx = min(PT, p.W - x0);
+  float s = 0.f, q = 0.f;
+  for (int px0 = 0; px0 < npx; px0 += 8) {
+    float ts = 0.f, tq = 0.f;
+    const int pe = min(px0 + 8, npx);
+    for (int px = px0; px < pe; ++px) {
       float acc = bias;
 #pragma unroll
       for (int c = 0; c < CIN; ++c)
 #pragma unroll
         for (int r = 0; r < 3; ++r)
 #pragma unroll
-          for (int q = 0; q < 3; ++q) acc += w[c * 9 + r * 3 + q] * patch[c][r][px + q];
-      out[((int64_t)(b * p.H + y) * p.W + x0 + px) * p.Cout + n] = from_f32<T>(acc);
-    }
+          for (int t = 0; t < 3; ++t) acc += w[c * 9 + r * 3 + t] * patch[c][r][px + t];
+      out[(int64_t)px * p.Cout] = from_f32<T>(acc);
+      const float v = stored<T>(acc);
+      ts += v; tq += v * v;
+    }
+    s += ts; q += tq;
+  }
+  if (p.stats != nullptr) {
+    const int tiles = (p.W + PT - 1) / PT;
+    const int64_t row = ((int64_t)b * p.H + y) * tiles + xt;
+    *reinterpret_cast<float2*>(p.stats + (row * p.Cout + n) * 2) = make_float2(s, q);
   }
 }
 
@@ -483,6 +518,10 @@
   return ns < 1 ? 1 : ns;
 }
 
+static std::atomic<long> g_gn_stats_launches{0}, g_resample_launches{0};
+long gn_stats_launch_count() { return g_gn_stats_launches.load(); }
+long resample_launch_count() { return g_resample_launches.load(); }
+
 int launch_gn_stats(const GnStatsParams& p, int dtype, hipStream_t s) {
   const int C = p.C0 + p.C1;
   if (p.groups != 32 || C % 128 != 0 || p.C0 % 4 != 0) return k22_set_error(K22_EINVAL, "gn_stats: need 32 groups, C % 128 == 0");
@@ -493,6 +532,7 @@
   else if (dtype == K22_F16) hipLaunchKernelGGL(gn_stats_kernel<f16_t>, grid, dim3(256), 0, s, p);
   else hipLaunchKernelGGL(gn_stats_kernel<float>, grid, dim3(256), 0, s, p);
   K22_CHECK_LAUNCH();
+  g_gn_stats_launches.fetch_add(1, std::memory_order_relaxed);
   return K22_OK;
 }
 int launch_gn_coeff(const GnCoeffParams& p, int B, hipStream_t s) {
@@ -511,9 +551,17 @@
   const int Hp = Ho + 2 * p.pad, Wp = Wo + 2 * p.pad;
   if (Hp > 65535 || p.B > 65535) return k22_set_error(K22_EINVAL, "gn_apply: tensor too large");
   dim3 grid((Wp * (C / epv) + 255) / 256, Hp, p.B);
-  if (dtype == K22_BF16) hipLaunchKernelGGL(gn_apply_kernel<bf16_t>, grid, dim3(256), 0, s, p);
-  else if (dtype == K22_F16) hipLaunchKernelGGL(gn_apply_kernel<f16_t>, grid, dim3(256), 0, s, p);
-  else hipLaunchKernelGGL(gn_apply_kernel<float>, grid, dim3(256), 0, s, p);
+  if (p.raw_out) {
+    if ((p.mode != 1 && p.mode != 2) || p.C1 != 0 || p.x1) return k22_set_error(K22_EINVAL, "gn_apply: raw_out needs mode 1 or 2 of a single tensor");
+    if (dtype == K22_BF16) hipLaunchKernelGGL((gn_apply_kernel<bf16_t, true>), grid, dim3(256), 0, s, p);
+    else if (dtype == K22_F16) hipLaunchKernelGGL((gn_apply_kernel<f16_t, true>), grid, dim3(256), 0, s, p);
+    else hipLaunchKernelGGL((gn_apply_kernel<float, true>), grid, dim3(256), 0, s, p);
+    K22_CHECK_LAUNCH();
+    return K22_OK;
+  }
+  if (dtype == K22_BF16) hipLaunchKernelGGL((gn_apply_kernel<bf16_t, false>), grid, dim3(256), 0, s, p);
+  else if (dtype == K22_F16) hipLaunchKernelGGL((gn_apply_kernel<f16_t, false>), grid, dim3(256), 0, s, p);
+  else hipLaunchKernelGGL((gn_apply_kernel<float, false>), grid, dim3(256), 0, s, p);
   K22_CHECK_LAUNCH();
   return K22_OK;
 }
@@ -525,10 +573,14 @@
   else if (dtype == K22_F16) hipLaunchKernelGGL(resample_kernel<f16_t>, dim3(nb), dim3(256), 0, s, x, y, B, H, W, C, mode);
   else hipLaunchKernelGGL(resample_kernel<float>, dim3(nb), dim3(256), 0, s, x, y, B, H, W, C, mode);
   K22_CHECK_LAUNCH();
+  g_resample_launches.fetch_add(1, std::memory_order_relaxed);
   return K22_OK;
 }
 int launch_conv_in(const ConvInParams& p, int dtype, hipStream_t s) {
-  dim3 grid((p.W + CONV_IN_PT - 1) / CONV_IN_PT, p.H, p.B);
+  if (p.x_bmod < 1 || p.x_bmod > p.B || p.Cout < 1) return k22_set_error(K22_EINVAL, "conv_in: x_bmod must be in 1..B");
+  const int64_t gx = (int64_t)((p.W + CONV_IN_PT - 1) / CONV_IN_PT) * ((p.Cout + 127) / 128);
+  if (gx > 0x7fffffff || p.H > 65535 || p.B > 65535) return k22_set_error(K22_EINVAL, "conv_in: tensor too large");
+  dim3 grid((unsigned)gx, p.H, p.B);
   if (p.Cin == 4) {
     if (dtype == K22_BF16) hipLaunchKernelGGL((conv_in_kernel<bf16_t, 4>), grid, dim3(128), 0, s, p);
     else if (dtype == K22_F16) hipLaunchKernelGGL((conv_in_kernel<f16_t, 4>), grid, dim3(128), 0, s, p);
diff --git a/kandinsky-2_amd/csrc/engine.hip b/kandinsky-2_amd/csrc/engine.hip
--- a/kandinsky-2_amd/csrc/engine.hip
+++ b/kandinsky-2_amd/csrc/engine.hip
@@ -22,6 +22,8 @@
 static std::atomic<long> g_loop_captures{0}, g_loop_launches{0};
 long loop_capture_count() { return g_loop_captures.load(); }
 long loop_launch_count() { return g_loop_launches.load(); }
+static std::atomic<long> g_loop_copies{0};
+long loop_copy_count() { return g_loop_copies.load(); }
 void loop_count_capture() { g_loop_captures.fetch_add(1); }
 void loop_count_launch() { g_loop_launches.fetch_add(1); }
 enum : unsigned long long { K22_LOOP_KIND_P = 0, K22_LOOP_KIND_DDIM = 1, K22_LOOP_KIND_PLMS = 2 };
@@ -47,8 +49,10 @@
   Slot* s0 = nullptr; int C0 = 0;
   Slot* s1 = nullptr; int C1 = 0;
   int H = 0, W = 0;
-  const Tuned* p0 = nullptr; Slot* st0 = nullptr;
-  const Tuned* p1 = nullptr; Slot* st1 = nullptr;
+  const Tuned* p0 = nullptr; Slot* st0 = nullptr; int r0 = 0;
+  const Tuned* p1 = nullptr; Slot* st1 = nullptr; int r1 = 0;
+  int rpi0() const { return p0 ? p0->rpi : r0; }
+  int rpi1() const { return p1 ? p1->rpi : r1; }
   int C() const { return C0 + C1; }
 };
 
@@ -64,6 +68,11 @@
   OpList hint_ops;
   bool hint_set = false;
   int fuse_skip = 1;
+  int stem_stats = 1;
+  int loop_inplace = 1;
+  int fuse_resample = 1;
+  int head_conv = 1;
+  const float* xin_cur = nullptr;
   int fuse_gn = 0;
   struct GnLink { const Tuned* consumer = nullptr; };
   std::deque<GnLink> gn_links;
@@ -170,16 +179,26 @@
     }
     return K22_OK;
   }
+  static int loop_copy(void* dst, const void* src, size_t bytes, hipStream_t s) {
+    g_loop_copies.fetch_add(1);
+    return copy_d2d(dst, src, bytes, s);
+  }
   int loop_model(const LoopRows& lr, const float* cur, const float* timesteps, int call, hipStream_t s) {
-    const size_t half = (size_t)(B / 2) * 4 * H * W * sizeof(float);
-    if (int rc = copy_d2d(ptr(s_xin), cur, half, s)) return rc;
-    if (int rc = copy_d2d(ptr(s_xin) + half, cur, half, s)) return rc;
+    if (loop_inplace) {
+      xin_cur = cur;
+    } else {
+      const size_t half = (size_t)(B / 2) * 4 * H * W * sizeof(float);
+      if (int rc = loop_copy(ptr(s_xin), cur, half, s)) return rc;
+      if (int rc = loop_copy(ptr(s_xin) + half, cur, half, s)) return rc;
+    }
     if (lr.hoist) {
       film_cur = lr.film + (int64_t)call * B * film_total;
     } else {
       if (int rc = copy_d2d(ptr(s_t), timesteps + (size_t)call * B, (size_t)B * 4, s)) return rc;
     }
-    return exec(s);
+    const int rc = exec(s);
+    xin_cur = nullptr;
+    return rc;
   }
   template <typename F> int loop_run(const std::vector<unsigned long long>& key, const float* timesteps, const float* inpaint_image,
                                      const float* inpaint_mask, int use_graph, hipStream_t st, F body) {
@@ -219,7 +238,7 @@
   int run_ops(hipStream_t st) { return run_ops_range(st, 0, ops.size()); }
 
   void op_gn(OpList& L, const Act& in, const std::string& pfx, int64_t film_off,
-             int act, int mode, int pad, Slot* dst, const GnLink* link = nullptr) {
+             int act, int mode, int pad, Slot* dst, const GnLink* link = nullptr, Slot* raw_dst = nullptr) {
     const int Bn = B, C = in.C(), HW = in.H * in.W;
     const int nsplit = gn_nsplit(Bn, HW);
     const bool fused = in.st0 != nullptr && (in.s1 == nullptr || in.st1 != nullptr);
@@ -233,14 +252,15 @@
     const Act a = in;
     const int dt = sdt;
     const int x3 = k22_is_split(dtype) ? 1 : 0;
-    const double gn_bytes = (double)Bn * HW * C * esz * (fused ? 1.0 : 2.0) + (double)Bn * (Ho + 2 * pad) * (Wo + 2 * pad) * C * esz;
+    const double gn_bytes = (double)Bn * HW * C * esz * (fused ? 1.0 : 2.0) + (double)Bn * (Ho + 2 * pad) * (Wo + 2 * pad) * C * esz +
+                            (raw_dst ? (double)Bn * Ho * Wo * C * esz : 0.0);
     L.push_back(Op([=](hipStream_t st) {
       const void* x0 = ptr(a.s0);
       const void* x1 = a.s1 ? ptr(a.s1) : nullptr;
       GnCoeffParams cp = {};
       if (fused) {
-        cp.src[0].st = ptr<float>(a.st0); cp.src[0].rpi = a.p0->rpi; cp.src[0].C = a.C0;
-        if (a.s1) { cp.src[1].st = ptr<float>(a.st1); cp.src[1].rpi = a.p1->rpi; cp.src[1].C = a.C1; }
+        cp.src[0].st = ptr<float>(a.st0); cp.src[0].rpi = a.rpi0(); cp.src[0].C = a.C0;
+        if (a.s1) { cp.src[1].st = ptr<float>(a.st1); cp.src[1].rpi = a.rpi1(); cp.src[1].C = a.C1; }
         if (cp.src[0].rpi <= 0 || (a.s1 && cp.src[1].rpi <= 0)) return k22_set_error(K22_EINVAL, "unet: producer delivered no GroupNorm partial sums");
       } else {
         GnStatsParams sp;
@@ -257,6 +277,7 @@
       GnApplyParams ap = {};
       ap.x0 = x0; ap.x1 = x1; ap.C0 = a.C0; ap.C1 = a.C1; ap.B = Bn; ap.H = a.H; ap.W = a.W;
       ap.mode = mode; ap.pad = pad; ap.act = act; ap.coeff = ptr<float>(s_coeff); ap.out = ptr(dst); ap.out_x3 = x3;
+      ap.raw_out = raw_dst ? ptr(raw_dst) : nullptr;
       int rc = launch_gn_coeff(cp, Bn, st);
       if (rc) return rc;
       if (link != nullptr && link->consumer != nullptr && conv3_algo_fuses_gn(link->consumer->cfg.algo)) return K22_OK;
@@ -389,7 +410,9 @@
     const int Wo = updown == 1 ? in.W / 2 : (updown == 2 ? in.W * 2 : in.W);
     GnLink* l1 = nullptr;
     if (fuse_gn && updown == 0) { gn_links.emplace_back(); l1 = &gn_links.back(); }
-    op_gn(ops, in, pfx + ".in_layers.0", -1, K22_ACT_SILU, updown, 1, s_P1, l1);
+    const bool raw_skip = updown != 0 && fuse_resample && in.s1 == nullptr;
+    if (raw_skip) need(s_S, (size_t)B * Ho * Wo * Cin * esz);
+    op_gn(ops, in, pfx + ".in_layers.0", -1, K22_ACT_SILU, updown, 1, s_P1, l1, raw_skip ? s_S : nullptr);
     Tuned* t1 = op_conv(ops, CONV_IN, s_P1, Ho, Wo, Cin, Cout, pfx + ".in_layers.2", nullptr, s_U1, IG_OUT_ROWMAJOR, s_U1st, nullptr, std::string(),
                         l1 ? &in : nullptr, K22_ACT_SILU);
     if (l1) l1->consumer = t1;
@@ -405,8 +428,10 @@
     if (updown) {
       if (Cin != Cout || in.s1) { if (err.empty()) err = "updown ResBlock with channel change is not supported"; }
       need(s_S, (size_t)B * Ho * Wo * Cin * esz);
-      const Act a = in; const int Bn = B, dt = sdt;
-      ops.push_back([=](hipStream_t st) { return launch_resample(ptr(a.s0), ptr(s_S), Bn, a.H, a.W, Cin, updown, dt, st); });
+      if (!raw_skip) {
+        const Act a = in; const int Bn = B, dt = sdt;
+        ops.push_back([=](hipStream_t st) { return launch_resample(ptr(a.s0), ptr(s_S), Bn, a.H, a.W, Cin, updown, dt, st); });
+      }
       skip.s0 = s_S;
     } else if (Cin != Cout) {
       IgemmParams probe = igemm_conv3_problem(B, Ho, Wo, Cout, Cout);
@@ -564,14 +589,19 @@
       cp.B = B; cp.H = H; cp.W = W; cp.Cin = cfg.in_channels; cp.Cout = ch;
       const int dt = sdt; const bool inpaint = cfg.in_channels == 9, hinted = cfg.in_channels == 8;
       const int premul = (hinted || cfg.head_type == 1) ? 1 : 0;
+      Slot* sst = stem_stats ? new_slot((size_t)B * conv_in_rpi(H, W) * ch * 2 * sizeof(float)) : nullptr;
+      const int Bn = B;
       ops.push_back([=](hipStream_t st) {
         ConvInParams q = cp;
-        q.x = ptr<float>(s_xin); q.img = inpaint ? ptr<float>(s_img) : (hinted ? ptr<float>(s_hint) : nullptr);
+        q.x = xin_cur ? xin_cur : ptr<float>(s_xin); q.x_bmod = xin_cur ? Bn / 2 : Bn;
+        q.stats = sst ? ptr<float>(sst) : nullptr;
+        q.img = inpaint ? ptr<float>(s_img) : (hinted ? ptr<float>(s_hint) : nullptr);
         q.mask = inpaint ? ptr<float>(s_mask) : nullptr; q.img_premul = premul;
         q.out = ptr(d);
         return launch_conv_in(q, dt, st);
       });
       Act a; a.s0 = d; a.C0 = ch; a.H = H; a.W = W;
+      if (sst) { a.st0 = sst; a.r0 = conv_in_rpi(H, W); }
       hs.push_back(a);
     }
     Act h = hs.back();
@@ -611,6 +641,7 @@
         const Act skip = hs.back(); hs.pop_back();
         Act cat; cat.s0 = h.s0; cat.C0 = h.C0; cat.s1 = skip.s0; cat.C1 = skip.C0; cat.H = h.H; cat.W = h.W;
         cat.p0 = h.p0; cat.st0 = h.st0; cat.p1 = skip.p0; cat.st1 = skip.st0;
+        cat.r0 = h.r0; cat.r1 = skip.r0;
         if (skip.H != h.H || skip.W != h.W) return k22_set_error(K22_EINVAL, "unet: skip shape mismatch");
         const int co = mc * cfg.channel_mult[l];
         const std::string pfx = "output_blocks." + std::to_string(blk);
@@ -626,7 +657,19 @@
     }
     if (film_cursor != film_total) return k22_set_error(K22_EINVAL, "unet: internal FiLM width mismatch");
     op_gn(ops, h, "out.0", -1, K22_ACT_SILU, 0, 1, s_P1);
-    op_conv(ops, CONV_HEAD, s_P1, H, W, ch, cfg.out_channels, "out.2", nullptr, s_out, IG_OUT_NCHW_F32);
+    if (head_conv && conv_head_supported(B, H, W, ch, cfg.out_channels, conv_dt(CONV_HEAD, H))) {
+      ConvHeadParams hp = {};
+      hp.Wp = W_("out.2.weight"); hp.bias = Wf("out.2.bias");
+      hp.B = B; hp.H = H; hp.W = W; hp.Cin = ch; hp.Cout = cfg.out_channels;
+      const int dt = dtype;
+      ops.push_back(Op([=](hipStream_t st) {
+        ConvHeadParams q = hp;
+        q.x = ptr(s_P1); q.out = ptr<float>(s_out);
+        return launch_conv_head(q, dt, st);
+      }, OP_CONV3, 2.0 * B * H * W * (double)cfg.out_channels * 9.0 * ch, 0.0, 1));
+    } else {
+      op_conv(ops, CONV_HEAD, s_P1, H, W, ch, cfg.out_channels, "out.2", nullptr, s_out, IG_OUT_NCHW_F32);
+    }
 
     return finish_plan();
   }
@@ -748,6 +791,10 @@
   u->stream_frag = env_flag("K22_STREAM", 1);
   u->fuse_gn = env_flag("K22_FUSE_GN", 0);
   u->fuse_skip = env_flag("K22_FUSE_SKIP", 1);
+  u->stem_stats = env_flag("K22_STEM_STATS", 1);
+  u->loop_inplace = env_flag("K22_LOOP_INPLACE", 1);
+  u->fuse_resample = env_flag("K22_FUSE_RESAMPLE", 1);
+  u->head_conv = env_flag("K22_HEAD_CONV", 1);
   u->hoist_time = env_flag("K22_HOIST_TIME", 1);
   const char* xp = getenv("K22_X2_PLAN");
   u->x2_plan = xp ? (atoi(xp) & 3) : 0;
@@ -858,7 +905,7 @@
       if (rc) return rc;
       float* t_ = cur; cur = nxt; nxt = t_;
     }
-    if (cur != x) return copy_d2d(x, cur, (size_t)B * 4 * HW * sizeof(float), s);
+    if (cur != x) return K22UNet::loop_copy(x, cur, (size_t)B * 4 * HW * sizeof(float), s);
     return K22_OK;
   };
   std::vector<unsigned long long> key = {K22_LOOP_KIND_P, loop_key_ptr(x), loop_key_ptr(x_tmp), loop_key_ptr(timesteps), loop_key_ptr(noise_seq),
@@ -922,7 +969,7 @@
       }
       float* t_ = cur; cur = nxt; nxt = t_;
     }
-    if (cur != x) return copy_d2d(x, cur, lat * sizeof(float), s);
+    if (cur != x) return K22UNet::loop_copy(x, cur, lat * sizeof(float), s);
     return K22_OK;
   };
   const std::vector<unsigned long long> key = {kind == K22_LOOP_DDIM ? K22_LOOP_KIND_DDIM : K22_LOOP_KIND_PLMS, loop_key_ptr(x), loop_key_ptr(x_tmp),
diff --git a/kandinsky-2_amd/csrc/kernels.h b/kandinsky-2_amd/csrc/kernels.h
--- a/kandinsky-2_amd/csrc/kernels.h
+++ b/kandinsky-2_amd/csrc/kernels.h
@@ -157,6 +157,7 @@
 long stream_launch_count();
 long loop_capture_count();
 long loop_launch_count();
+long loop_copy_count();
 void loop_count_capture();
 void loop_count_launch();
 inline unsigned long long loop_key_ptr(const void* p) { return (unsigned long long)(uintptr_t)p; }
```

Result: no change. 149.3 steps/s, median of 6 (+1.0%).
